# beehover/dependence_free_rl

Hardware: AMD Instinct MI355X
Metric: env-steps/sec (whole node) PPO bin-packing 64-bin (higher is better)
Workload: dtype f32 via f16-pair (layer 2, dH1) / 3-part bf16 split (dW2) MFMA, f32 accumulate

## Files before the change

### dependence_free_rl_amd/csrc/policy_kernels.hip

```cpp
#include "spec8_e0_layout.h"
#include "xh_device.h"
#include "xh_kernels.h"
#include "xh_logit_table.h"
#include "xh_split.h"

#include <cstdlib>

#ifndef XH_DIAG_ABLATE
#define XH_DIAG_ABLATE 0
#endif
#define XH_ABL(a, k) (XH_DIAG_ABLATE && ((a).ablate & (k)))
#ifndef XH_DIAG_TRACE
#define XH_DIAG_TRACE 0
#endif
#if XH_DIAG_TRACE
#define XH_STAMP(a, gi, w, lane, slot)                                        \
  do {                                                                        \
    if ((a).trace && blockIdx.x < kTraceBlocks && (gi) < kTraceGroups &&      \
        (lane) == 0)                                                          \
      (a).trace[((blockIdx.x * kTraceGroups + (gi)) * 8 + (w)) * kTraceSlots + \
                (slot)] = clock64();                                          \
  } while (0)
#else
#define XH_STAMP(a, gi, w, lane, slot) \
  do {                                 \
  } while (0)
#endif
#define XH_STAMP4(a, gi, w, lane, slot) XH_STAMP(a, gi, w, lane, slot)
#if XH_DIAG_TRACE
#define XH_SPAN(a, which)                                                     \
  do {                                                                        \
    if ((a).trace && threadIdx.x == 0) {                                      \
      unsigned long long *sp = reinterpret_cast<unsigned long long *>(        \
          (a).trace + kTraceBlocks * kTraceGroups * 8 * kTraceSlots);         \
      const unsigned long long tnow = (unsigned long long)wall_clock64();     \
      if ((which) == 0)                                                       \
        atomicMin(sp, tnow);                                                  \
      else if ((which) == 3)                                                  \
        atomicMax(sp + 1, tnow);                                              \
      if (blockIdx.x < 512) sp[2 + 4 * blockIdx.x + (which)] = tnow;          \
      if ((which) == 0 && blockIdx.x < 512) {                                 \
        unsigned hw, xc;                                                      \
        asm volatile("s_getreg_b32 %0, hwreg(HW_REG_HW_ID)" : "=s"(hw));      \
        asm volatile("s_getreg_b32 %0, hwreg(HW_REG_XCC_ID)" : "=s"(xc));     \
        sp[2 + 2048 + 2 * blockIdx.x] = hw;                                   \
        sp[2 + 2048 + 2 * blockIdx.x + 1] = xc;                               \
      }                                                                       \
    }                                                                         \
  } while (0)
#else
#define XH_SPAN(a, which) \
  do {                    \
  } while (0)
#endif

namespace xh {
int diag_build() { return XH_DIAG_ABLATE || XH_DIAG_TRACE; }
}

namespace xh {

template <int B_, int D_, int H1_, int H2_>
struct PShape {
  static constexpr int B = B_, D = D_, H1 = H1_, H2 = H2_;
  static constexpr int F0 = 2 * D;
  static constexpr int S1 = (F0 + 1) / 2;
  static constexpr int NIT = H1 / 32, NOT = H2 / 32;
  static constexpr int G = B <= 64 ? 64 / B : 1;
  static constexpr int HG = B <= 64 ? 1 : B / 64;
  static constexpr int R = 64 * HG;
  static constexpr int BD = B * D;
  static constexpr int W2S = H1 + 4;
  static constexpr int HS = H1 + 1;
  static constexpr int AS = H2 + 1;
  static constexpr int FJ = NOT >= 4 ? 2 : 1;
  static constexpr int JW = (NOT * NIT + 3) / 4;
  static constexpr int JH = (2 * NIT + 3) / 4;
  static constexpr int TOCC = (H1 <= 64 && H2 <= 64 && D == 1) ? 2 : 1;
  static_assert(B == 8 || B == 16 || B == 32 || B == 64 || B == 128, "B");
  static_assert(NIT == 1 || NIT == 2 || NIT == 4, "H1 in {32,64,128}");
  static_assert(NOT == 1 || NOT == 2 || NOT == 4, "H2 in {32,64,128}");
  static_assert(D >= 1 && D <= 3, "D");
  static constexpr int r4(int x) { return (x + 3) & ~3; }
  static constexpr int L_W2 = 0;
  static constexpr int L_W1 = L_W2 + H2 * W2S;
  static constexpr int L_B1 = L_W1 + r4(H1 * F0);
  static constexpr int L_B2 = L_B1 + H1;
  static constexpr int L_W3 = L_B2 + H2;
  static constexpr int L_B3 = L_W3 + H2;
  static constexpr int L_Z = L_B3 + 4;
  static constexpr int L_ROLLOUT_END = L_Z + NOT * R;
  static constexpr int L_H1 = L_ROLLOUT_END;
  static constexpr int L_DA2 = L_H1 + r4(64 * HS);
  static constexpr int L_TRAIN_END = L_DA2 + r4(64 * AS);
  static constexpr int TS = 68;
  static constexpr int L_H1T = L_ROLLOUT_END;
  static constexpr int L_DAT = L_H1T + H1 * TS;
  static constexpr int L_B1F = L_DAT + H2 * TS;
  static constexpr int L_TRAIN8_END = L_B1F + 2 * H1;
  static constexpr int RED = H1 * F0 + H1 + 2 * H2 + 1;
  static_assert(4 * RED <= 64 * HS + 64 * AS, "scratch fits");
};

template <class S>
__device__ __forceinline__ void stage_params(const float *__restrict__ P,
                                             float *lds) {
  const PolicyLayout L{S::F0, S::H1, S::H2};
  const int tid = threadIdx.x;
  for (int i = tid; i < S::H2 * S::H1; i += blockDim.x) {
    const int o = i / S::H1, k = i - o * S::H1;
    lds[S::L_W2 + o * S::W2S + k] = P[L.oW2() + i];
  }
  for (int i = tid; i < S::H1 * S::F0; i += blockDim.x)
    lds[S::L_W1 + i] = P[L.oW1() + i];
  for (int i = tid; i < S::H1; i += blockDim.x) lds[S::L_B1 + i] = P[L.ob1() + i];
  for (int i = tid; i < S::H2; i += blockDim.x) {
    lds[S::L_B2 + i] = P[L.ob2() + i];
    lds[S::L_W3 + i] = P[L.ow3() + i];
  }
  if (tid == 0) lds[S::L_B3] = P[L.ob3()];
}

template <class S>
struct RowRaw {
  int bv[2][S::D];
  int iv[2][S::D];
};

template <class S>
__device__ __forceinline__ void fetch_rows(const Batch &b, int slot, int e0,
                                           RowRaw<S> &rr) {
  const int lr = threadIdx.x & 31;
#pragma unroll
  for (int rt = 0; rt < 2; ++rt) {
    const int r = rt * 32 + lr;
    const size_t env = (size_t)slot * b.N + e0 + r / S::B;
    const int8_t *bp = b.bins + env * S::BD + (r % S::B) * S::D;
    const int8_t *ip = b.items + env * 4;
#pragma unroll
    for (int d = 0; d < S::D; ++d) {
      rr.bv[rt][d] = bp[d];
      rr.iv[rt][d] = ip[d];
    }
  }
}

template <class S>
__device__ __forceinline__ float row_feature(const RowRaw<S> &rr, int rt,
                                             int f) {
  int v = 0;
#pragma unroll
  for (int d = 0; d < S::D; ++d) {
    if (f == d) v = rr.bv[rt][d];
    if (f == S::D + d) v = rr.iv[rt][d];
  }
  return f < S::F0 ? (float)v / (float)kCapacity : 0.0f;
}

__device__ __forceinline__ float4 lds4(const float *p) {
  return *reinterpret_cast<const float4 *>(p);
}

template <class S>
__device__ __forceinline__ void layer1(const RowRaw<S> &rr, const float *lds,
                                       f32x16 (&h1)[S::NIT][2]) {
  const int lane = threadIdx.x & 63, lr = lane & 31, h = lane >> 5;
  float xb[2][S::S1];
#pragma unroll
  for (int rt = 0; rt < 2; ++rt)
#pragma unroll
    for (int s = 0; s < S::S1; ++s) xb[rt][s] = row_feature<S>(rr, rt, 2 * s + h);
#pragma unroll
  for (int it = 0; it < S::NIT; ++it) {
    float wa[S::S1];
#pragma unroll
    for (int s = 0; s < S::S1; ++s) {
      const int k = 2 * s + h;
      wa[s] = k < S::F0 ? lds[S::L_W1 + (it * 32 + lr) * S::F0 + k] : 0.0f;
    }
    f32x16 acc0 = zero16(), acc1 = zero16();
#pragma unroll
    for (int s = 0; s < S::S1; ++s) {
      acc0 = mfma32(wa[s], xb[0][s], acc0);
      acc1 = mfma32(wa[s], xb[1][s], acc1);
    }
#pragma unroll
    for (int q = 0; q < 4; ++q) {
      const float4 bb = lds4(lds + S::L_B1 + it * 32 + 8 * q + 4 * h);
      const float bq[4] = {bb.x, bb.y, bb.z, bb.w};
#pragma unroll
      for (int u = 0; u < 4; ++u) {
        const float v0 = acc0[4 * q + u] + bq[u];
        const float v1 = acc1[4 * q + u] + bq[u];
        acc0[4 * q + u] = relu(v0);
        acc1[4 * q + u] = relu(v1);
      }
    }
    h1[it][0] = acc0;
    h1[it][1] = acc1;
  }
}

template <class S, int NR>
__device__ __forceinline__ void layer2(const float *lds,
                                       const f32x16 (&h1)[S::NIT][2], int o2t,
                                       int rt0, f32x16 (&acc)[NR]) {
  const int lane = threadIdx.x & 63, lr = lane & 31, h = lane >> 5;
  const float *wrow = lds + S::L_W2 + (o2t * 32 + lr) * S::W2S + 4 * h;
#pragma unroll
  for (int r = 0; r < NR; ++r) acc[r] = zero16();
#pragma unroll
  for (int it = 0; it < S::NIT; ++it) {
    f32x16 hb[NR];
#pragma unroll
    for (int r = 0; r < NR; ++r)
      hb[r] = NR == 2 ? h1[it][r] : (rt0 == 0 ? h1[it][0] : h1[it][1]);
#pragma unroll
    for (int q = 0; q < 4; ++q) {
      const float4 a4 = lds4(wrow + it * 32 + 8 * q);
      const float av[4] = {a4.x, a4.y, a4.z, a4.w};
#pragma unroll
      for (int u = 0; u < 4; ++u)
#pragma unroll
        for (int r = 0; r < NR; ++r) acc[r] = mfma32(av[u], hb[r][4 * q + u], acc[r]);
    }
  }
#pragma unroll
  for (int q = 0; q < 4; ++q) {
    const float4 bb = lds4(lds + S::L_B2 + o2t * 32 + 8 * q + 4 * h);
    const float bq[4] = {bb.x, bb.y, bb.z, bb.w};
#pragma unroll
    for (int u = 0; u < 4; ++u)
#pragma unroll
      for (int r = 0; r < NR; ++r) acc[r][4 * q + u] += bq[u];
  }
}

template <class S, bool kSwap = false>
__device__ __forceinline__ float logit_part(const float *lds, const f32x16 &pre,
                                            int o2t) {
  const int h = (threadIdx.x & 63) >> 5;
  float zp = 0.0f;
#pragma unroll
  for (int q = 0; q < 4; ++q) {
    const float4 ww = lds4(lds + S::L_W3 + o2t * 32 + 8 * q + 4 * h);
    const float wq[4] = {ww.x, ww.y, ww.z, ww.w};
#pragma unroll
    for (int u = 0; u < 4; ++u) {
      const float v = relu(pre[4 * q + u]);
      zp += v * wq[u];
    }
  }
  return zp + (kSwap ? half_swap(zp) : __shfl_xor(zp, 32, kWave));
}

template <class S>
__device__ __forceinline__ void sample_step_x(const RolloutArgs &a, int t, bool last,
                                              float z, int env, int seg0, int bin,
                                              const RowRaw<S> &cur, uint32_t &x,
                                              int (&nbv)[S::D], bool &first) {
  constexpr int B = S::B;
  const int lane = threadIdx.x & 63, h = lane >> 5;
  const int N = a.b.N;
  const float ex = expf(z);
  const float sum = seg_sum<B>(ex);
  const float p = ex / sum;
  if (last && a.logits_out) a.logits_out[(size_t)env * B + bin] = z;
  if (last && a.probs_out) a.probs_out[(size_t)env * B + bin] = p;
  if (a.qold_out) a.qold_out[((size_t)t * N + env) * B + bin] = p;

  int choice;
  if (a.forced) {
    choice = a.forced[(size_t)t * N + env];
    (void)canonical(x);
  } else {
    choice = sample_discrete<B>(p, lane, canonical(x));
  }
  const float pold = wave_shfl(p, seg0 + choice);

  int nb[S::D];
  int neg = 0;
#pragma unroll
  for (int d = 0; d < S::D; ++d) {
    const int bv = h ? cur.bv[1][d] : cur.bv[0][d];
    const int iv = h ? cur.iv[1][d] : cur.iv[0][d];
    nb[d] = bin == choice ? bv - iv : bv;
    neg |= nb[d] < 0;
  }
  const int done = __shfl(neg, seg0 + choice, kWave);
  first = canonical(x) < a.env.p_a;
  int8_t *ob = a.b.bins + ((size_t)(t + 1) * N + env) * S::BD + bin * S::D;
#pragma unroll
  for (int d = 0; d < S::D; ++d) {
    nbv[d] = done ? kCapacity : nb[d];
    ob[d] = (int8_t)nbv[d];
  }
  if (bin == 0) {
    int8_t *oi = a.b.items + ((size_t)(t + 1) * N + env) * 4;
#pragma unroll
    for (int d = 0; d < 4; ++d)
      oi[d] = d < S::D ? (int8_t)(first ? a.env.item_a[d] : a.env.item_b[d]) : 0;
    a.b.action[(size_t)t * N + env] = choice;
    a.b.pold[(size_t)t * N + env] = pold;
    a.b.done[(size_t)t * N + env] = (uint8_t)done;
  }
}

template <class S>
__device__ __forceinline__ void sample_step(const RolloutArgs &a, float z,
                                            int env, int seg0, int bin,
                                            const RowRaw<S> &cur) {
  uint32_t x = a.b.rng[env];
  int nbv[S::D];
  bool first;
  sample_step_x<S>(a, a.t, true, z, env, seg0, bin, cur, x, nbv, first);
  if (bin == 0) a.b.rng[env] = (a.t == a.b.T - 1) ? mstd_mulmod(x, a.jump_mul) : x;
}

template <class S>
__global__ __launch_bounds__(256, 2) void rollout_step_kernel(RolloutArgs a) {
  extern __shared__ __attribute__((aligned(16))) float lds[];
  stage_params<S>(a.params, lds);
  __syncthreads();
  const int lane = threadIdx.x & 63, w = threadIdx.x >> 6, lr = lane & 31;
  const int N = a.b.N, t = a.t;
  const int ngroups = N / S::G;
  const int o2t = w % S::NOT;
  const int rt0 = S::NOT >= 4 ? 0 : w / S::NOT;
  const bool fwd_active = (w / S::NOT) * S::FJ < 2;

  RowRaw<S> cur, nxt;
  if ((int)blockIdx.x < ngroups) fetch_rows<S>(a.b, t, blockIdx.x * S::G, cur);
  for (int g = blockIdx.x; g < ngroups; g += gridDim.x) {
    const int e0 = g * S::G;
    const int gn = g + gridDim.x;
    if (gn < ngroups) fetch_rows<S>(a.b, t, gn * S::G, nxt);
    {
      f32x16 h1[S::NIT][2];
      layer1<S>(cur, lds, h1);
      if (fwd_active) {
        f32x16 pre[S::FJ];
        layer2<S, S::FJ>(lds, h1, o2t, rt0, pre);
#pragma unroll
        for (int q = 0; q < S::FJ; ++q) {
          const float zp = logit_part<S>(lds, pre[q], o2t);
          if (lane < 32) lds[S::L_Z + o2t * 64 + (rt0 + q) * 32 + lr] = zp;
        }
      }
    }
    __syncthreads();
    if (w == 0) {
      constexpr int B = S::B;
      const int e = lane / B, bin = lane % B, env = e0 + e, seg0 = e * B;
      float zs = 0.0f;
#pragma unroll
      for (int o = 0; o < S::NOT; ++o) zs += lds[S::L_Z + o * 64 + lane];
      const float z = zs + lds[S::L_B3];
      sample_step<S>(a, z, env, seg0, bin, cur);
    }
    __syncthreads();
    cur = nxt;
  }
}

#ifndef XH_V_RPASS
#define XH_V_RPASS 1
#endif
#ifndef XH_V_RTILES64
#define XH_V_RTILES64 4
#endif
#ifndef XH_V_RTILES128
#define XH_V_RTILES128 2
#endif
constexpr int roll_waves(int tiles) { return XH_V_RPASS && tiles == 4 ? 12 : 8; }
constexpr int roll_occ(int waves) { return waves == 8 ? 4 : (waves == 12 ? 3 : 2); }
constexpr int kRollWaves64 = roll_waves(XH_V_RTILES64);
constexpr int kRollWaves128 = roll_waves(XH_V_RTILES128);
#ifndef XH_V_RSB
#define XH_V_RSB 1
#endif
template <class S, int OT>
__device__ __forceinline__ void wave_logits_rpass(const float *lds,
                                                  const RowRaw<S> &cur,
                                                  float (&zl)[2]) {
  const int lane = threadIdx.x & 63, lr = lane & 31, h = lane >> 5;
#pragma unroll
  for (int rt = 0; rt < 2; ++rt) {
    float xb[S::S1];
#pragma unroll
    for (int s = 0; s < S::S1; ++s) xb[s] = row_feature<S>(cur, rt, 2 * s + h);
    float z = 0.0f;
#pragma unroll 1
    for (int op = 0; op < 4 / OT; ++op) {
    f32x16 pre[OT];
#pragma unroll
    for (int o = 0; o < OT; ++o) pre[o] = zero16();
#pragma unroll 1
    for (int it = 0; it < 4; ++it) {
      f32x16 t1 = zero16();
#pragma unroll
      for (int s = 0; s < S::S1; ++s) {
        const int k = 2 * s + h;
        const float wa = k < S::F0 ? lds[S::L_W1 + (it * 32 + lr) * S::F0 + k] : 0.0f;
        t1 = mfma32(wa, xb[s], t1);
      }
#pragma unroll
      for (int q = 0; q < 4; ++q) {
        const float4 bb = lds4(lds + S::L_B1 + it * 32 + 8 * q + 4 * h);
        const float bq[4] = {bb.x, bb.y, bb.z, bb.w};
#pragma unroll
        for (int u = 0; u < 4; ++u) t1[4 * q + u] = relu(t1[4 * q + u] + bq[u]);
      }
#pragma unroll
      for (int oo = 0; oo < OT; ++oo) {
        const int o = op * OT + oo;
        const float *wrow = lds + S::L_W2 + (o * 32 + lr) * S::W2S + 4 * h;
#pragma unroll
        for (int q = 0; q < 4; ++q) {
          const float4 a4 = lds4(wrow + it * 32 + 8 * q);
          const float av[4] = {a4.x, a4.y, a4.z, a4.w};
#pragma unroll
          for (int u = 0; u < 4; ++u) pre[oo] = mfma32(av[u], t1[4 * q + u], pre[oo]);
        }
        if (XH_V_RSB) __builtin_amdgcn_sched_barrier(0);
      }
    }
#pragma unroll
    for (int oo = 0; oo < OT; ++oo) {
      const int o = op * OT + oo;
#pragma unroll
      for (int q = 0; q < 4; ++q) {
        const float4 bb = lds4(lds + S::L_B2 + o * 32 + 8 * q + 4 * h);
        const float bq[4] = {bb.x, bb.y, bb.z, bb.w};
#pragma unroll
        for (int u = 0; u < 4; ++u) pre[oo][4 * q + u] += bq[u];
      }
      z += logit_part<S>(lds, pre[oo], o);
    }
    }
    if (rt == 0)
      zl[0] = z;
    else
      zl[1] = z;
  }
}

template <class S>
__global__ __launch_bounds__(64 * kRollWaves64, roll_occ(kRollWaves64)) void rollout_wave_kernel(RolloutArgs a) {
  static_assert(S::B == 64 && S::NIT == 4 && S::NOT == 4, "wave rollout: B=64, [128,128]");
  extern __shared__ __attribute__((aligned(16))) float lds[];
  stage_params<S>(a.params, lds);
  __syncthreads();
  const int lane = threadIdx.x & 63, w = threadIdx.x >> 6, lr = lane & 31,
            h = lane >> 5;
  const int wpb = blockDim.x >> 6;
  for (int env = blockIdx.x * wpb + w; env < a.b.N; env += gridDim.x * wpb) {
    RowRaw<S> cur;
    fetch_rows<S>(a.b, a.t, env, cur);
    float xb[2][S::S1];
#pragma unroll
    for (int rt = 0; rt < 2; ++rt)
#pragma unroll
      for (int s = 0; s < S::S1; ++s) xb[rt][s] = row_feature<S>(cur, rt, 2 * s + h);
    float zl[2] = {0.0f, 0.0f};
    if (XH_V_RPASS) wave_logits_rpass<S, XH_V_RTILES64>(lds, cur, zl);
#pragma unroll 1
    for (int o2t = 0; o2t < (XH_V_RPASS ? 0 : 4); ++o2t) {
      const float *wrow = lds + S::L_W2 + (o2t * 32 + lr) * S::W2S + 4 * h;
      f32x16 pre[2];
      pre[0] = zero16();
      pre[1] = zero16();
#pragma unroll 1
      for (int it = 0; it < 4; ++it) {
        f32x16 t1[2];
        t1[0] = zero16();
        t1[1] = zero16();
#pragma unroll
        for (int s = 0; s < S::S1; ++s) {
          const int k = 2 * s + h;
          const float wa = k < S::F0 ? lds[S::L_W1 + (it * 32 + lr) * S::F0 + k] : 0.0f;
          t1[0] = mfma32(wa, xb[0][s], t1[0]);
          t1[1] = mfma32(wa, xb[1][s], t1[1]);
        }
#pragma unroll
        for (int q = 0; q < 4; ++q) {
          const float4 bb = lds4(lds + S::L_B1 + it * 32 + 8 * q + 4 * h);
          const float bq[4] = {bb.x, bb.y, bb.z, bb.w};
#pragma unroll
          for (int u = 0; u < 4; ++u) {
            t1[0][4 * q + u] = relu(t1[0][4 * q + u] + bq[u]);
            t1[1][4 * q + u] = relu(t1[1][4 * q + u] + bq[u]);
          }
        }
#pragma unroll
        for (int q = 0; q < 4; ++q) {
          const float4 a4 = lds4(wrow + it * 32 + 8 * q);
          const float av[4] = {a4.x, a4.y, a4.z, a4.w};
#pragma unroll
          for (int u = 0; u < 4; ++u) {
            pre[0] = mfma32(av[u], t1[0][4 * q + u], pre[0]);
            pre[1] = mfma32(av[u], t1[1][4 * q + u], pre[1]);
          }
        }
      }
#pragma unroll
      for (int q = 0; q < 4; ++q) {
        const float4 bb = lds4(lds + S::L_B2 + o2t * 32 + 8 * q + 4 * h);
        const float bq[4] = {bb.x, bb.y, bb.z, bb.w};
#pragma unroll
        for (int u = 0; u < 4; ++u) {
          pre[0][4 * q + u] += bq[u];
          pre[1][4 * q + u] += bq[u];
        }
      }
      zl[0] += logit_part<S>(lds, pre[0], o2t);
      zl[1] += logit_part<S>(lds, pre[1], o2t);
    }
    const float z = (h ? zl[1] : zl[0]) + lds[S::L_B3];
    sample_step<S>(a, z, env, 0, lane, cur);
  }
}

template <class S>
struct RollSplitLds {
  static constexpr int W2 = 0;
  static constexpr int F = 2 * S::H2 * kImgRow;
  static constexpr int W1 = 0, B1 = S::H1 * S::F0, B2 = B1 + S::H1, W3 = B2 + S::H2,
                       B3 = W3 + S::H2, SH = B3 + 1, SC = B3 + 4, B1F = SC + 2 * 16;
  static constexpr int S1F = (S::D + 1) / 2;
  static constexpr size_t bytes = F + sizeof(float) * (B1F + 2 * S::H1);
};

template <class S>
__device__ __forceinline__ void stage_split_rollout(const float *__restrict__ P,
                                                    const EnvDesc &env, char *lds) {
  using L = RollSplitLds<S>;
  float *lf = reinterpret_cast<float *>(lds + L::F);
  const PolicyLayout PL{S::F0, S::H1, S::H2};
  float mw = 0.0f, mh = 0.0f;
  for (int e = threadIdx.x; e < S::H2 * S::H1; e += blockDim.x)
    mw = fmaxf(mw, fabsf(P[PL.oW2() + e]));
  for (int i = threadIdx.x; i < S::H1; i += blockDim.x) {
    float v = fabsf(P[PL.ob1() + i]);
    for (int k = 0; k < S::F0; ++k) v += fabsf(P[PL.oW1() + i * S::F0 + k]);
    mh = fmaxf(mh, v);
  }
#pragma unroll
  for (int o = 1; o < 64; o <<= 1) {
    mw = fmaxf(mw, __shfl_xor(mw, o, kWave));
    mh = fmaxf(mh, __shfl_xor(mh, o, kWave));
  }
  const int nw = blockDim.x >> 6, wv = threadIdx.x >> 6;
  if ((threadIdx.x & 63) == 0) {
    lf[L::SC + wv] = mw;
    lf[L::SC + 16 + wv] = mh;
  }
  __syncthreads();
  float MW = 0.0f, MH = 0.0f;
  for (int v = 0; v < nw; ++v) {
    MW = fmaxf(MW, lf[L::SC + v]);
    MH = fmaxf(MH, lf[L::SC + 16 + v]);
  }
  const float SW = f16_scale_for(MW), SH = f16_scale_for(MH), S2 = SW * SH;
  for (int e = threadIdx.x; e < S::H2 * S::H1; e += blockDim.x) {
    const int o = e / S::H1, i = e % S::H1;
    const int c = (i & ~12) | ((i & 4) << 1) | ((i & 8) >> 1);
    _Float16 x0, x1;
    split2h(P[PL.oW2() + e] * SW, x0, x1);
    const int off = img_off(o, c >> 3) + 2 * (c & 7);
    *reinterpret_cast<_Float16 *>(lds + L::W2 + off) = x0;
    *reinterpret_cast<_Float16 *>(lds + L::W2 + S::H2 * kImgRow + off) = x1;
  }
  for (int i = threadIdx.x; i < S::H1 * S::F0; i += blockDim.x)
    lf[L::W1 + i] = P[PL.oW1() + i] * SH;
  for (int i = threadIdx.x; i < S::H1; i += blockDim.x) {
    lf[L::B1 + i] = P[PL.ob1() + i] * SH;
    lf[L::B2 + i] = P[PL.ob2() + i] * S2;
    lf[L::W3 + i] = P[PL.ow3() + i] * (1.0f / S2);
    float ba = P[PL.ob1() + i], bb = ba;
#pragma unroll
    for (int d = 0; d < S::D; ++d) {
      const float wv = P[PL.oW1() + i * S::F0 + S::D + d];
      ba += wv * ((float)env.item_a[d] / (float)kCapacity);
      bb += wv * ((float)env.item_b[d] / (float)kCapacity);
    }
    lf[L::B1F + i] = ba * SH;
    lf[L::B1F + S::H1 + i] = bb * SH;
  }
  if (threadIdx.x == 0) {
    lf[L::B3] = P[PL.ob3()];
    lf[L::SH] = SH;
  }
}

template <class S, bool E0 = false>
__device__ __forceinline__ void wave_logits_split(const char *lds,
                                                  const RowRaw<S> &cur,
                                                  const float *const (&b1r)[2],
                                                  float (&zl)[2],
                                                  unsigned *mbits = nullptr) {
  using L = RollSplitLds<S>;
  const float *lf = reinterpret_cast<const float *>(lds + L::F);
  const int lane = threadIdx.x & 63, lr = lane & 31, h = lane >> 5;
  const char *w2i[2] = {lds + L::W2, lds + L::W2 + S::H2 * kImgRow};
#pragma unroll
  for (int rt = 0; rt < 2; ++rt) {
    float xb[L::S1F];
#pragma unroll
    for (int s1 = 0; s1 < L::S1F; ++s1) {
      const int f = 2 * s1 + h;
      xb[s1] = f < S::D ? row_feature<S>(cur, rt, f) : 0.0f;
    }
    f32x16s pre[S::NOT];
#pragma unroll
    for (int ot = 0; ot < S::NOT; ++ot)
#pragma unroll
      for (int q = 0; q < 4; ++q) {
        const float4 bb = *reinterpret_cast<const float4 *>(lf + L::B2 + ot * 32 + 8 * q + 4 * h);
        pre[ot][4 * q + 0] = bb.x;
        pre[ot][4 * q + 1] = bb.y;
        pre[ot][4 * q + 2] = bb.z;
        pre[ot][4 * q + 3] = bb.w;
      }
#pragma unroll
    for (int it = 0; it < S::NIT; ++it) {
      f32x16 t1;
#pragma unroll
      for (int q = 0; q < 4; ++q) {
        const float4 bb = *reinterpret_cast<const float4 *>(b1r[rt] + it * 32 + 8 * q + 4 * h);
        t1[4 * q + 0] = bb.x;
        t1[4 * q + 1] = bb.y;
        t1[4 * q + 2] = bb.z;
        t1[4 * q + 3] = bb.w;
      }
#pragma unroll
      for (int s1 = 0; s1 < L::S1F; ++s1) {
        const int k = 2 * s1 + h;
        const float wa = k < S::D ? lf[L::W1 + (it * 32 + lr) * S::F0 + k] : 0.0f;
        t1 = mfma32(wa, xb[s1], t1);
      }
      f16x8 bfr[2][2];
      {
        typedef unsigned u32x4_t __attribute__((ext_vector_type(4)));
        u32x4_t hb[2], lb[2];
#pragma unroll
        for (int jj = 0; jj < 8; ++jj) {
          unsigned h2, l2;
          split2h_x2(relu(t1[2 * jj]), relu(t1[2 * jj + 1]), h2, l2);
          hb[jj >> 2][jj & 3] = h2;
          lb[jj >> 2][jj & 3] = l2;
        }
#pragma unroll
        for (int s = 0; s < 2; ++s) {
          bfr[s][0] = __builtin_bit_cast(f16x8, hb[s]);
          bfr[s][1] = __builtin_bit_cast(f16x8, lb[s]);
        }
      }
#pragma unroll
      for (int ot = 0; ot < S::NOT; ++ot) {
        const int rb = row_base(ot * 32 + lr, h);
#pragma unroll
        for (int s = 0; s < 2; ++s) {
          f16x8 af[2];
#pragma unroll
          for (int p = 0; p < 2; ++p)
            af[p] = __builtin_bit_cast(f16x8, ld_row(w2i[p], rb, 2 * it + s));
          pre[ot] = mfma_f16(af[1], bfr[s][0], pre[ot]);
          pre[ot] = mfma_f16(af[0], bfr[s][1], pre[ot]);
          pre[ot] = mfma_f16(af[0], bfr[s][0], pre[ot]);
        }
        __builtin_amdgcn_sched_barrier(0);
      }
    }
    float z = 0.0f;
#pragma unroll
    for (int ot = 0; ot < S::NOT; ++ot) {
      float zp = 0.0f;
#pragma unroll
      for (int q = 0; q < 4; ++q) {
        const float4 ww = *reinterpret_cast<const float4 *>(lf + L::W3 + ot * 32 + 8 * q + 4 * h);
        const float wq[4] = {ww.x, ww.y, ww.z, ww.w};
#pragma unroll
        for (int u = 0; u < 4; ++u) zp = fmaf(relu(pre[ot][4 * q + u]), wq[u], zp);
      }
      z += zp + __shfl_xor(zp, 32, kWave);
    }
    zl[rt] = z;
    if constexpr (E0) {
#pragma unroll
      for (int ot = 0; ot < S::NOT; ++ot) {
        unsigned wd = rt == 0 ? 0u : mbits[ot];
#pragma unroll
        for (int e = 0; e < 16; ++e) {
          int m;
          asm("v_med3_i32 %0, %1, 0, 1" : "=v"(m) : "v"(__float_as_int(pre[ot][e])));
          wd |= (unsigned)m << sp8::e0_bit(rt, e);
        }
        mbits[ot] = wd;
      }
    }
  }
}

template <class S>
constexpr int roll_split_waves() { return S::B == 64 ? kRollWaves64 : 4; }
template <class S>
constexpr int roll_split_occ() { return S::B == 64 ? roll_occ(kRollWaves64) : 2; }

template <class S>
__device__ __forceinline__ void build_logit_table(const char *lds, float *out) {
  static_assert(S::B == 64 && S::D == 2 && S::G == 1 && lt::kCap == kCapacity,
                "the logit table: 64 bins, 2-D");
  const float *lfr = reinterpret_cast<const float *>(lds + RollSplitLds<S>::F);
  const float *const b1r[2] = {lfr + RollSplitLds<S>::B1F,
                               lfr + RollSplitLds<S>::B1F + S::H1};
  const int lane = threadIdx.x & 63, w = threadIdx.x >> 6, lr = lane & 31;
  const int nw = blockDim.x >> 6;
#pragma unroll 1
  for (int c = w; c < lt::kCalls; c += nw) {
    const int sn = lt::enum_state(c, lr);
    const int s = sn < lt::kStates ? sn : lt::kStates - 1;
    int b0, b1;
    lt::state_bins(s, b0, b1);
    RowRaw<S> cur;
#pragma unroll
    for (int rt = 0; rt < 2; ++rt) {
      cur.bv[rt][0] = b0;
      cur.bv[rt][1] = b1;
      cur.iv[rt][0] = cur.iv[rt][1] = 0;
    }
    float zl[2];
    wave_logits_split<S>(lds, cur, b1r, zl);
    if (lane < 32 && sn < lt::kStates) {
      out[lt::entry(0, b0, b1)] = zl[0];
      out[lt::entry(1, b0, b1)] = zl[1];
    }
  }
}

template <class S, bool TAB>
constexpr size_t roll_split_lds() {
  return RollSplitLds<S>::bytes + (TAB ? sizeof(float) * lt::kEntries : 0);
}

template <class S, bool E0 = false, bool TAB = false>
__global__ __launch_bounds__(64 * roll_split_waves<S>(), roll_split_occ<S>()) void rollout_split_kernel(RolloutArgs a) {
  static_assert((S::B == 64 && S::NIT == 4 && S::NOT == 4) ||
                    (S::B == 32 && S::NIT == 2 && S::NOT == 2),
                "split rollout: B=64 [128,128] or B=32 [64,64]");
  static_assert(!E0 || (S::B == 64 && S::G == 1 && S::H2 == sp8::kE0Outs),
                "the epoch-0 records: one env of 64 bins per wave");
  static_assert(!TAB || !E0, "the table carries no relu masks");
  extern __shared__ __attribute__((aligned(16))) float ldsf[];
  char *lds = reinterpret_cast<char *>(ldsf);
  stage_split_rollout<S>(a.params, a.env, lds);
  __syncthreads();
  const float *lfr = reinterpret_cast<const float *>(lds + RollSplitLds<S>::F);
  const float b3 = lfr[RollSplitLds<S>::B3];
  const float *tab = reinterpret_cast<const float *>(lds + RollSplitLds<S>::bytes);
  if constexpr (TAB) {
    build_logit_table<S>(lds, reinterpret_cast<float *>(lds + RollSplitLds<S>::bytes));
    __syncthreads();
  }
  const float *b1fa = lfr + RollSplitLds<S>::B1F, *b1fb = b1fa + S::H1;
  const int lane = threadIdx.x & 63, w = threadIdx.x >> 6, h = lane >> 5, lr = lane & 31;
  const int wpb = blockDim.x >> 6;
  const int ngroups = a.b.N / S::G;
  const int t_last = a.t + (a.nsteps > 1 ? a.nsteps : 1) - 1;
  const int eoff = S::G == 2 ? h : 0, seg0 = S::G == 2 ? 32 * h : 0;
  const int bin = S::G == 2 ? lr : lane;
  const int per = (ngroups + (int)gridDim.x - 1) / (int)gridDim.x;
  const int g_end = min(ngroups, ((int)blockIdx.x + 1) * per);
  for (int g = (int)blockIdx.x * per + w; g < g_end; g += wpb) {
    const int e0 = g * S::G, env = e0 + eoff;
    RowRaw<S> cur;
    fetch_rows<S>(a.b, a.src_slot > 0 ? a.src_slot : a.t, e0, cur);
    if (a.src_slot > 0) {
      int8_t *ob = a.b.bins + (size_t)env * S::BD + bin * S::D;
#pragma unroll
      for (int d = 0; d < S::D; ++d) ob[d] = (int8_t)(h ? cur.bv[1][d] : cur.bv[0][d]);
      if (bin == 0) {
        int8_t *oi = a.b.items + (size_t)env * 4;
#pragma unroll
        for (int d = 0; d < 4; ++d)
          oi[d] = d < S::D ? (int8_t)(h ? cur.iv[1][d] : cur.iv[0][d]) : 0;
      }
    }
    uint32_t x = a.b.rng[env];
    for (int t = a.t; t <= t_last; ++t) {
      const float *b1r[2];
      bool iar[2];
#pragma unroll
      for (int rt = 0; rt < 2; ++rt) {
        bool ia = true;
#pragma unroll
        for (int d = 0; d < S::D; ++d) ia &= cur.iv[rt][d] == a.env.item_a[d];
        iar[rt] = ia;
        b1r[rt] = ia ? b1fa : b1fb;
      }
      float zl[2];
      if constexpr (TAB) {
        const int e = lt::entry((h ? iar[1] : iar[0]) ? 0 : 1,
                                h ? cur.bv[1][0] : cur.bv[0][0],
                                h ? cur.bv[1][1] : cur.bv[0][1]);
        zl[0] = zl[1] = tab[min((unsigned)e, (unsigned)lt::kEntries - 1u)];
      } else if constexpr (E0) {
        unsigned mbits[4];
        wave_logits_split<S, true>(lds, cur, b1r, zl, mbits);
        uint32_t *rec = a.e0_mask + ((size_t)t * a.b.N + env) * sp8::kE0Words;
#pragma unroll
        for (int ot = 0; ot < 4; ++ot) rec[sp8::e0_word(ot, lane)] = mbits[ot];
      } else {
        wave_logits_split<S>(lds, cur, b1r, zl);
      }
      const float z = (h ? zl[1] : zl[0]) + b3;
      int nbv[S::D];
      bool first;
      sample_step_x<S>(a, t, t == t_last, z, env, seg0, bin, cur, x, nbv, first);
      if (t < t_last) {
#pragma unroll
        for (int d = 0; d < S::D; ++d) {
          const int own = nbv[d], oth = __shfl_xor(own, 32, kWave);
          const int ito = first ? a.env.item_a[d] : a.env.item_b[d];
          const int itp = S::G == 2 ? __shfl_xor(ito, 32, kWave) : ito;
          cur.bv[0][d] = h ? oth : own;
          cur.bv[1][d] = h ? own : oth;
          cur.iv[0][d] = h ? itp : ito;
          cur.iv[1][d] = h ? ito : itp;
        }
      }
    }
    if (bin == 0) a.b.rng[env] = (t_last == a.b.T - 1) ? mstd_mulmod(x, a.jump_mul) : x;
  }
}

template <class S>
__device__ __forceinline__ void sample_step128_x(const RolloutArgs &a, int t, bool last,
                                                 int env, const float (&z)[2],
                                                 uint32_t &x, int (&nbv)[2][S::D],
                                                 const int (&iv)[S::D], bool &first) {
  const int lane = threadIdx.x & 63;
  const int N = a.b.N;
  float p[2];
  float se = 0.0f;
#pragma unroll
  for (int k = 0; k < 2; ++k) {
    p[k] = expf(z[k]);
    se += p[k];
  }
  se = seg_sum<64>(se);
  p[0] = p[0] / se;
  p[1] = p[1] / se;
  if (last && a.logits_out) {
    a.logits_out[(size_t)env * 128 + lane] = z[0];
    a.logits_out[(size_t)env * 128 + 64 + lane] = z[1];
  }
  if (last && a.probs_out) {
    a.probs_out[(size_t)env * 128 + lane] = p[0];
    a.probs_out[(size_t)env * 128 + 64 + lane] = p[1];
  }
  if (a.qold_out) {
    a.qold_out[((size_t)t * N + env) * 128 + lane] = p[0];
    a.qold_out[((size_t)t * N + env) * 128 + 64 + lane] = p[1];
  }
  int choice;
  if (a.forced) {
    choice = a.forced[(size_t)t * N + env];
    (void)canonical(x);
  } else {
    const double pd0 = (double)p[0], pd1 = (double)p[1];
    const double sd = seg_sum_d<64>(pd0 + pd1);
    const double c0 = seg_scan_d<64>(pd0 / sd, lane);
    const double tot0 = wave_shfl_d(c0, 63);
    double c1 = tot0 + seg_scan_d<64>(pd1 / sd, lane);
    if (lane == 63) c1 = 1.0;
    const double u = canonical(x);
    choice = __popcll(__ballot(c0 < u)) + __popcll(__ballot(c1 < u));
    const float gap = (float)fmin(fabs(c0 - u), fabs(c1 - u));
    if (seg_min<64>(gap) < 1e-9f) {
      double s2 = 0.0;
      for (int k = 0; k < 128; ++k)
        s2 += (double)wave_shfl(p[k >> 6], k & 63);
      double acc = 0.0;
      int c2 = 127;
      for (int k = 0; k < 128; ++k) {
        const double qk = (double)wave_shfl(p[k >> 6], k & 63) / s2;
        acc = k == 0 ? qk : acc + qk;
        const double cpk = k == 127 ? 1.0 : acc;
        if (!(cpk < u) && k < c2) c2 = k;
      }
      choice = c2;
    }
  }
  const float pold = choice < 64 ? wave_shfl(p[0], choice)
                                 : wave_shfl(p[1], choice - 64);
  int nb[2][S::D];
  int neg[2] = {0, 0};
#pragma unroll
  for (int k = 0; k < 2; ++k) {
    const int bin = k * 64 + lane;
#pragma unroll
    for (int d = 0; d < S::D; ++d) {
      nb[k][d] = bin == choice ? nbv[k][d] - iv[d] : nbv[k][d];
      neg[k] |= nb[k][d] < 0;
    }
  }
  const int done = __shfl(choice < 64 ? neg[0] : neg[1], choice & 63, kWave);
  first = canonical(x) < a.env.p_a;
  const size_t o = (size_t)(t + 1) * N + env;
#pragma unroll
  for (int k = 0; k < 2; ++k) {
    int8_t *ob = a.b.bins + o * S::BD + (k * 64 + lane) * S::D;
#pragma unroll
    for (int d = 0; d < S::D; ++d) {
      nbv[k][d] = done ? kCapacity : nb[k][d];
      ob[d] = (int8_t)nbv[k][d];
    }
  }
  if (lane == 0) {
    int8_t *oi = a.b.items + o * 4;
#pragma unroll
    for (int d = 0; d < 4; ++d)
      oi[d] = d < S::D ? (int8_t)(first ? a.env.item_a[d] : a.env.item_b[d]) : 0;
    a.b.action[(size_t)t * N + env] = choice;
    a.b.pold[(size_t)t * N + env] = pold;
    a.b.done[(size_t)t * N + env] = (uint8_t)done;
  }
}

template <class S>
__device__ __forceinline__ void sample_step128(const RolloutArgs &a, int env,
                                               const float (&z)[2]) {
  const int lane = threadIdx.x & 63;
  uint32_t x = a.b.rng[env];
  const size_t e = (size_t)a.t * a.b.N + env;
  int nbv[2][S::D], iv[S::D];
#pragma unroll
  for (int k = 0; k < 2; ++k)
#pragma unroll
    for (int d = 0; d < S::D; ++d) nbv[k][d] = a.b.bins[e * S::BD + (k * 64 + lane) * S::D + d];
#pragma unroll
  for (int d = 0; d < S::D; ++d) iv[d] = a.b.items[e * 4 + d];
  bool first;
  sample_step128_x<S>(a, a.t, true, env, z, x, nbv, iv, first);
  if (lane == 0) a.b.rng[env] = (a.t == a.b.T - 1) ? mstd_mulmod(x, a.jump_mul) : x;
}

template <class S>
__global__ __launch_bounds__(256, 2) void rollout_step128_kernel(RolloutArgs a) {
  static_assert(S::B == 128 && S::HG == 2, "128-bin rollout");
  extern __shared__ __attribute__((aligned(16))) float lds[];
  stage_params<S>(a.params, lds);
  __syncthreads();
  constexpr int R = S::R;
  const int lane = threadIdx.x & 63, w = threadIdx.x >> 6, lr = lane & 31;
  const int N = a.b.N, t = a.t;
  const int o2t = w % S::NOT;
  const int rt0 = S::NOT >= 4 ? 0 : w / S::NOT;
  const bool fwd_active = (w / S::NOT) * S::FJ < 2;
  for (int env = blockIdx.x; env < N; env += gridDim.x) {
#pragma unroll
    for (int hg = 0; hg < 2; ++hg) {
      RowRaw<S> rr;
#pragma unroll
      for (int k = 0; k < 2; ++k) {
        const int bin = hg * 64 + k * 32 + lr;
        const size_t e = (size_t)t * N + env;
        const int8_t *bp = a.b.bins + e * S::BD + bin * S::D;
        const int8_t *ip = a.b.items + e * 4;
#pragma unroll
        for (int d = 0; d < S::D; ++d) {
          rr.bv[k][d] = bp[d];
          rr.iv[k][d] = ip[d];
        }
      }
      f32x16 h1[S::NIT][2];
      layer1<S>(rr, lds, h1);
      if (fwd_active) {
        f32x16 pre[S::FJ];
        layer2<S, S::FJ>(lds, h1, o2t, rt0, pre);
#pragma unroll
        for (int q = 0; q < S::FJ; ++q) {
          const float zp = logit_part<S>(lds, pre[q], o2t);
          if (lane < 32) lds[S::L_Z + o2t * R + hg * 64 + (rt0 + q) * 32 + lr] = zp;
        }
      }
    }
    __syncthreads();
    if (w == 0) {
      float z[2];
#pragma unroll
      for (int k = 0; k < 2; ++k) {
        float zs = 0.0f;
#pragma unroll
        for (int o = 0; o < S::NOT; ++o) zs += lds[S::L_Z + o * R + k * 64 + lane];
        z[k] = zs + lds[S::L_B3];
      }
      sample_step128<S>(a, env, z);
    }
    __syncthreads();
  }
}

template <class S>
__global__ __launch_bounds__(64 * kRollWaves128, roll_occ(kRollWaves128)) void rollout_wave128_kernel(RolloutArgs a) {
  static_assert(S::B == 128 && S::NIT == 4 && S::NOT == 4,
                "wave rollout: B=128, [128,128]");
  extern __shared__ __attribute__((aligned(16))) float lds[];
  stage_params<S>(a.params, lds);
  __syncthreads();
  const int lane = threadIdx.x & 63, w = threadIdx.x >> 6, lr = lane & 31,
            h = lane >> 5;
  const int wpb = blockDim.x >> 6;
  const int N = a.b.N, t = a.t;
  for (int env = blockIdx.x * wpb + w; env < N; env += gridDim.x * wpb) {
    float z0 = 0.0f, z1 = 0.0f;
#pragma unroll 1
    for (int hg = 0; hg < 2; ++hg) {
      RowRaw<S> cur;
      const size_t e = (size_t)t * N + env;
#pragma unroll
      for (int rt = 0; rt < 2; ++rt) {
        const int bin = hg * 64 + rt * 32 + lr;
        const int8_t *bp = a.b.bins + e * S::BD + bin * S::D;
        const int8_t *ip = a.b.items + e * 4;
#pragma unroll
        for (int d = 0; d < S::D; ++d) {
          cur.bv[rt][d] = bp[d];
          cur.iv[rt][d] = ip[d];
        }
      }
      float xb[2][S::S1];
#pragma unroll
      for (int rt = 0; rt < 2; ++rt)
#pragma unroll
        for (int s = 0; s < S::S1; ++s) xb[rt][s] = row_feature<S>(cur, rt, 2 * s + h);
      float zl[2] = {0.0f, 0.0f};
      if (XH_V_RPASS) wave_logits_rpass<S, XH_V_RTILES128>(lds, cur, zl);
#pragma unroll 1
      for (int o2t = 0; o2t < (XH_V_RPASS ? 0 : 4); ++o2t) {
        const float *wrow = lds + S::L_W2 + (o2t * 32 + lr) * S::W2S + 4 * h;
        f32x16 pre[2];
        pre[0] = zero16();
        pre[1] = zero16();
#pragma unroll 1
        for (int it = 0; it < 4; ++it) {
          f32x16 t1[2];
          t1[0] = zero16();
          t1[1] = zero16();
#pragma unroll
          for (int s = 0; s < S::S1; ++s) {
            const int k = 2 * s + h;
            const float wa = k < S::F0 ? lds[S::L_W1 + (it * 32 + lr) * S::F0 + k] : 0.0f;
            t1[0] = mfma32(wa, xb[0][s], t1[0]);
            t1[1] = mfma32(wa, xb[1][s], t1[1]);
          }
#pragma unroll
          for (int q = 0; q < 4; ++q) {
            const float4 bb = lds4(lds + S::L_B1 + it * 32 + 8 * q + 4 * h);
            const float bq[4] = {bb.x, bb.y, bb.z, bb.w};
#pragma unroll
            for (int u = 0; u < 4; ++u) {
              t1[0][4 * q + u] = relu(t1[0][4 * q + u] + bq[u]);
              t1[1][4 * q + u] = relu(t1[1][4 * q + u] + bq[u]);
            }
          }
#pragma unroll
          for (int q = 0; q < 4; ++q) {
            const float4 a4 = lds4(wrow + it * 32 + 8 * q);
            const float av[4] = {a4.x, a4.y, a4.z, a4.w};
#pragma unroll
            for (int u = 0; u < 4; ++u) {
              pre[0] = mfma32(av[u], t1[0][4 * q + u], pre[0]);
              pre[1] = mfma32(av[u], t1[1][4 * q + u], pre[1]);
            }
          }
        }
#pragma unroll
        for (int q = 0; q < 4; ++q) {
          const float4 bb = lds4(lds + S::L_B2 + o2t * 32 + 8 * q + 4 * h);
          const float bq[4] = {bb.x, bb.y, bb.z, bb.w};
#pragma unroll
          for (int u = 0; u < 4; ++u) {
            pre[0][4 * q + u] += bq[u];
            pre[1][4 * q + u] += bq[u];
          }
        }
        zl[0] += logit_part<S>(lds, pre[0], o2t);
        zl[1] += logit_part<S>(lds, pre[1], o2t);
      }
      const float zh = (h ? zl[1] : zl[0]) + lds[S::L_B3];
      if (hg == 0)
        z0 = zh;
      else
        z1 = zh;
    }
    const float z[2] = {z0, z1};
    sample_step128<S>(a, env, z);
  }
}

constexpr int kRollWavesS128 = 12;
template <class S>
__global__ __launch_bounds__(64 * kRollWavesS128, 3) void rollout_split128_kernel(RolloutArgs a) {
  static_assert(S::B == 128 && S::NIT == 4 && S::NOT == 4,
                "split rollout: B=128, [128,128]");
  extern __shared__ __attribute__((aligned(16))) float ldsf[];
  char *lds = reinterpret_cast<char *>(ldsf);
  stage_split_rollout<S>(a.params, a.env, lds);
  __syncthreads();
  const float *lfr = reinterpret_cast<const float *>(lds + RollSplitLds<S>::F);
  const float b3 = lfr[RollSplitLds<S>::B3];
  const float *b1fa = lfr + RollSplitLds<S>::B1F, *b1fb = b1fa + S::H1;
  const int lane = threadIdx.x & 63, w = threadIdx.x >> 6, h = lane >> 5;
  const int wpb = blockDim.x >> 6;
  const int N = a.b.N;
  const int t_last = a.t + (a.nsteps > 1 ? a.nsteps : 1) - 1;
  const int per = (N + (int)gridDim.x - 1) / (int)gridDim.x;
  const int env_end = min(N, ((int)blockIdx.x + 1) * per);
  for (int env = (int)blockIdx.x * per + w; env < env_end; env += wpb) {
    int own[2][S::D], it[S::D];
    {
      const size_t e = (size_t)(a.src_slot > 0 ? a.src_slot : a.t) * N + env;
#pragma unroll
      for (int k = 0; k < 2; ++k)
#pragma unroll
        for (int d = 0; d < S::D; ++d) own[k][d] = a.b.bins[e * S::BD + (k * 64 + lane) * S::D + d];
#pragma unroll
      for (int d = 0; d < S::D; ++d) it[d] = a.b.items[e * 4 + d];
      if (a.src_slot > 0) {
#pragma unroll
        for (int k = 0; k < 2; ++k)
#pragma unroll
          for (int d = 0; d < S::D; ++d)
            a.b.bins[(size_t)env * S::BD + (k * 64 + lane) * S::D + d] = (int8_t)own[k][d];
        if (lane == 0)
#pragma unroll
          for (int d = 0; d < 4; ++d) a.b.items[(size_t)env * 4 + d] = d < S::D ? (int8_t)it[d] : 0;
      }
    }
    uint32_t x = a.b.rng[env];
    for (int t = a.t; t <= t_last; ++t) {
      bool ia = true;
#pragma unroll
      for (int d = 0; d < S::D; ++d) ia &= it[d] == a.env.item_a[d];
      const float *b1r[2] = {ia ? b1fa : b1fb, ia ? b1fa : b1fb};
      float z[2];
#pragma unroll 1
      for (int hg = 0; hg < 2; ++hg) {
        RowRaw<S> cur;
#pragma unroll
        for (int d = 0; d < S::D; ++d) {
          const int v = hg ? own[1][d] : own[0][d];
          const int o = __shfl_xor(v, 32, kWave);
          cur.bv[0][d] = h ? o : v;
          cur.bv[1][d] = h ? v : o;
          cur.iv[0][d] = it[d];
          cur.iv[1][d] = it[d];
        }
        float zl[2];
        wave_logits_split<S>(lds, cur, b1r, zl);
        const float zh = (h ? zl[1] : zl[0]) + b3;
        if (hg == 0)
          z[0] = zh;
        else
          z[1] = zh;
      }
      bool first;
      sample_step128_x<S>(a, t, t == t_last, env, z, x, own, it, first);
#pragma unroll
      for (int d = 0; d < S::D; ++d) it[d] = first ? a.env.item_a[d] : a.env.item_b[d];
    }
    if (lane == 0) a.b.rng[env] = (t_last == a.b.T - 1) ? mstd_mulmod(x, a.jump_mul) : x;
  }
}


template <class S>
__global__ __launch_bounds__(256, 1) void eval_argmax_kernel(EvalArgs a) {
  static_assert(S::HG == 1, "groups of whole envs");
  extern __shared__ __attribute__((aligned(16))) float lds[];
  stage_params<S>(a.params, lds);
  constexpr int B = S::B, G = S::G, D = S::D;
  int *sbins = reinterpret_cast<int *>(lds + S::L_ROLLOUT_END);
  int *sitem = sbins + G * S::BD;
  uint32_t *srng = reinterpret_cast<uint32_t *>(sitem + G * 4);
  int *sleft = reinterpret_cast<int *>(srng + G);
  int *sflag = sleft + G;
  const int lane = threadIdx.x & 63, w = threadIdx.x >> 6, lr = lane & 31;
  const int o2t = w % S::NOT;
  const int rt0 = S::NOT >= 4 ? 0 : w / S::NOT;
  const bool fwd_active = (w / S::NOT) * S::FJ < 2;
  const int ngroups = a.n_envs / G;
  for (int g = blockIdx.x; g < ngroups; g += gridDim.x) {
    __syncthreads();
    if (w == 0) {
      const int e = lane / B, bin = lane % B, env = g * G + e;
      uint32_t x = mstd_jump(a.x0, (uint64_t)env * a.stream_stride);
      bool first = false;
      if (!a.init_items) first = canonical(x) < a.env.p_a;
      for (int d = 0; d < D; ++d) sbins[e * S::BD + bin * D + d] = kCapacity;
      if (bin == 0) {
        for (int d = 0; d < 4; ++d)
          sitem[e * 4 + d] =
              d >= D ? 0
              : a.init_items ? a.init_items[env * D + d]
              : (first ? a.env.item_a[d] : a.env.item_b[d]);
        srng[e] = x;
        sleft[e] = a.episodes;
        a.total[env] = 0.0;
        a.steps[env] = 0;
      }
    }
    __syncthreads();
    double reward = 0.0;
    long nsteps = 0;
    for (long it = 0; it < a.max_steps; ++it) {
      RowRaw<S> rr;
#pragma unroll
      for (int rt = 0; rt < 2; ++rt) {
        const int r = rt * 32 + lr, e = r / B, bin = r % B;
#pragma unroll
        for (int d = 0; d < D; ++d) {
          rr.bv[rt][d] = sbins[e * S::BD + bin * D + d];
          rr.iv[rt][d] = sitem[e * 4 + d];
        }
      }
      {
        f32x16 h1[S::NIT][2];
        layer1<S>(rr, lds, h1);
        if (fwd_active) {
          f32x16 pre[S::FJ];
          layer2<S, S::FJ>(lds, h1, o2t, rt0, pre);
#pragma unroll
          for (int q = 0; q < S::FJ; ++q) {
            const float zp = logit_part<S>(lds, pre[q], o2t);
            if (lane < 32) lds[S::L_Z + o2t * 64 + (rt0 + q) * 32 + lr] = zp;
          }
        }
      }
      __syncthreads();
      if (w == 0) {
        const int e = lane / B, bin = lane % B, seg0 = e * B;
        float zs = 0.0f;
#pragma unroll
        for (int o = 0; o < S::NOT; ++o) zs += lds[S::L_Z + o * 64 + lane];
        float v = zs + lds[S::L_B3];
        if (a.argmax_probs) {
          const float ex = expf(v);
          v = ex / seg_sum<B>(ex);
        }
        const int choice = seg_argmax_first<B>(v, bin);
        const bool active = sleft[e] > 0;
        int nb[D];
        int neg = 0;
#pragma unroll
        for (int d = 0; d < D; ++d) {
          const int b0 = sbins[e * S::BD + bin * D + d];
          nb[d] = bin == choice ? b0 - sitem[e * 4 + d] : b0;
          neg |= nb[d] < 0;
        }
        const int done = __shfl(neg, seg0 + choice, kWave);
        if (active) {
          uint32_t x = srng[e];
          const bool first = canonical(x) < a.env.p_a;
#pragma unroll
          for (int d = 0; d < D; ++d)
            sbins[e * S::BD + bin * D + d] = done ? kCapacity : nb[d];
          __builtin_amdgcn_wave_barrier();
          if (bin == 0) {
            for (int d = 0; d < D; ++d)
              sitem[e * 4 + d] = first ? a.env.item_a[d] : a.env.item_b[d];
            srng[e] = x;
            if (done) sleft[e] -= 1;
            reward += done ? 0.0 : 1.0;
            if (a.trace && g == 0 && e == 0 && nsteps < a.trace_cap)
              a.trace[nsteps] = choice;
            ++nsteps;
          }
        }
        const int any = __any(sleft[e] > 0);
        if (lane == 0) *sflag = any;
      }
      __syncthreads();
      if (*sflag == 0) break;
    }
    if (w == 0 && lane % B == 0) {
      const int env = g * G + lane / B;
      a.total[env] = reward;
      a.steps[env] = nsteps;
      a.rng_out[env] = srng[lane / B];
      for (int d = 0; d < D; ++d)
        a.final_items[env * D + d] = sitem[(lane / B) * 4 + d];
    }
  }
}

#ifndef XH_V4_UNROLL
#define XH_V4_UNROLL 3
#endif
#ifndef XH_V4_L3
#define XH_V4_L3 1
#endif


template <class S, bool KL>
__global__ __launch_bounds__(256, S::TOCC) void policy_train_kernel(PolicyTrainArgs a) {
  extern __shared__ __attribute__((aligned(16))) float lds[];
  XH_SPAN(a, 0);
  XH_STAMP4(a, kTraceGroups - 1, threadIdx.x >> 6, threadIdx.x & 63, 0);
  stage_params<S>(a.params, lds);
  __syncthreads();
  XH_STAMP4(a, kTraceGroups - 1, threadIdx.x >> 6, threadIdx.x & 63, 1);
  XH_SPAN(a, 1);
  constexpr int B = S::B, NIT = S::NIT, NOT = S::NOT;
  const int lane = threadIdx.x & 63, w = threadIdx.x >> 6, lr = lane & 31,
            h = lane >> 5;
  const int N = a.b.N, T = a.b.T;
  const int gpt = N / S::G;
  const int gmain = T * gpt;
  const int n_end = KL ? *a.n_end : 0;
  const int ngroups = KL ? gmain + gpt + (n_end + S::G - 1) / S::G : gmain;
  const float beta = KL ? *a.beta : 0.0f;
  double kl_acc = 0.0;
  float *H1img = lds + S::L_H1;
  float *DAimg = lds + S::L_DA2;

  const int o2t = w % NOT;
  const int rt0 = NOT >= 4 ? 0 : w / NOT;
  const bool fwd_active = (w / NOT) * S::FJ < 2;
  const int it_own = w % NIT;
  const int hrt0 = NIT >= 4 ? 0 : w / NIT;
  constexpr int HSTEP = 4 / NIT;

  f32x16 accW2[S::JW];
#pragma unroll
  for (int q = 0; q < S::JW; ++q) accW2[q] = zero16();
  float accW1[16][S::F0], accB1[16], accW3[16], accB2[16], accB3 = 0.0f;
#pragma unroll
  for (int j = 0; j < 16; ++j) {
    accB1[j] = accW3[j] = accB2[j] = 0.0f;
#pragma unroll
    for (int f = 0; f < S::F0; ++f) accW1[j][f] = 0.0f;
  }

  RowRaw<S> cur, nxt;
  int c_cur = 0, c_nxt = 0, v_cur = 1, v_nxt = 1;
  float po_cur = 1.0f, po_nxt = 1.0f, A_cur = 0.0f, A_nxt = 0.0f;
  float q_cur = 1.0f, q_nxt = 1.0f;
  auto fetch = [&](int g, RowRaw<S> &rr, int &c, float &po, float &A, float &q,
                   int &valid) {
    if constexpr (!KL) {
      const int t = g / gpt, e0 = (g - t * gpt) * S::G;
      fetch_rows<S>(a.b, t, e0, rr);
      const size_t ti = (size_t)t * N + e0 + lane / B;
      c = a.b.action[ti];
      po = a.b.pold[ti];
      A = a.adv[ti];
    } else {
#pragma unroll
      for (int rt = 0; rt < 2; ++rt) {
        const int r = rt * 32 + lr, el = r / B, bin = r % B;
        int t, e, kind, ok = 1;
        if (g < gmain) {
          t = g / gpt;
          e = (g - t * gpt) * S::G + el;
          kind = 0;
        } else if (g < gmain + gpt) {
          t = T;
          e = (g - gmain) * S::G + el;
          kind = 1;
          ok = a.b.done[(size_t)(T - 1) * N + e] == 0;
        } else {
          const int j = (g - gmain - gpt) * S::G + el;
          kind = 2;
          ok = j < n_end;
          const int te = ok ? a.end_list[j] : 0;
          t = te / N;
          e = te - t * N;
        }
        const size_t env = (size_t)t * N + e;
        const int8_t *bp = a.b.bins + env * S::BD + bin * S::D;
        const int8_t *ip = a.b.items + env * 4;
        const bool sub = kind == 2 && a.b.action[env] == bin;
#pragma unroll
        for (int d = 0; d < S::D; ++d) {
          rr.iv[rt][d] = ip[d];
          rr.bv[rt][d] = bp[d] - (sub ? ip[d] : 0);
        }
        if (rt == h) {
          c = kind == 0 ? a.b.action[env] : 0;
          A = kind == 0 ? a.adv[env] : 0.0f;
          po = 1.0f;
          const size_t qrow = kind == 1 ? (size_t)(T - 1) * N + e : env;
          q = a.qold[qrow * B + bin];
          valid = ok;
        }
      }
    }
  };
  if ((int)blockIdx.x < ngroups)
    fetch(blockIdx.x, cur, c_cur, po_cur, A_cur, q_cur, v_cur);

  for (int g = blockIdx.x; g < ngroups; g += gridDim.x) {
    const int gi = (g - (int)blockIdx.x) / (int)gridDim.x;
    (void)gi;
    XH_STAMP4(a, gi, w, lane, 0);
    const int gn = g + gridDim.x;
    if (gn < ngroups) fetch(gn, nxt, c_nxt, po_nxt, A_nxt, q_nxt, v_nxt);
    f32x16 pre[S::FJ];
    f32x16 h1own[2];
    {
      f32x16 h1[NIT][2];
      layer1<S>(cur, lds, h1);
      if (w < NIT) {
#pragma unroll
        for (int it = 0; it < NIT; ++it)
          if (it == w) {
#pragma unroll
            for (int rt = 0; rt < 2; ++rt)
#pragma unroll
              for (int j = 0; j < 16; ++j)
                H1img[(rt * 32 + lr) * S::HS + it * 32 + acc_row(j, h)] =
                    h1[it][rt][j];
          }
      }
#pragma unroll
      for (int it = 0; it < NIT; ++it)
        if (it == it_own) {
          h1own[0] = h1[it][0];
          h1own[1] = h1[it][1];
        }
      if (fwd_active) {
        if (!XH_ABL(a, 4)) {
          layer2<S, S::FJ>(lds, h1, o2t, rt0, pre);
        } else {
#pragma unroll
          for (int q = 0; q < S::FJ; ++q) pre[q] = h1[0][q & 1];
        }
#pragma unroll
        for (int q = 0; q < S::FJ; ++q) {
          const float zp = logit_part<S>(lds, pre[q], o2t);
          if (lane < 32) lds[S::L_Z + o2t * 64 + (rt0 + q) * 32 + lr] = zp;
        }
      }
    }
    XH_STAMP4(a, gi, w, lane, 1);
    __syncthreads();
    XH_STAMP4(a, gi, w, lane, 2);

    constexpr bool kOne = S::JW == 1 && S::JH == 1 && !KL;
    constexpr int kU4 = kOne ? XH_V4_UNROLL : 0;
    constexpr bool kL34 = kOne && XH_V4_L3;
    float4 w3v[4];
    if (kL34) {
#pragma unroll
      for (int qq = 0; qq < 4; ++qq)
        w3v[qq] = lds4(lds + S::L_W3 + o2t * 32 + 8 * qq + 4 * h);
    }

    float gz;
    {
      const int bin = lane % B, seg0 = (lane / B) * B;
      float zs = 0.0f;
#pragma unroll
      for (int o = 0; o < NOT; ++o) zs += lds[S::L_Z + o * 64 + lane];
      const float z = zs + lds[S::L_B3];
      const float ex = expf(z);
      const float p = ex / seg_sum<B>(ex);
      const int c = c_cur;
      const float A = A_cur;
      if constexpr (KL) {
        float gp = p * A + beta * (p - q_cur);
        if (bin == c) gp -= A;
        const float sg = seg_sum<B>(p * gp);
        gz = v_cur ? p * (gp - sg) : 0.0f;
        if (w == 0 && v_cur)
          kl_acc += (double)q_cur * log((double)q_cur / (double)p);
      } else if (XH_ABL(a, 8)) {
        gz = z * 1e-3f;
      } else if (a.algo == kPPO) {
        const float pc = wave_shfl(p, seg0 + c);
        const float ratio = pc / po_cur;
        float clipped = ratio;
        if (ratio > 1.0f + a.clip_eps)
          clipped = 1.0f + a.clip_eps;
        else if (ratio < 1.0f - a.clip_eps)
          clipped = 1.0f - a.clip_eps;
        const float ig = fminf(clipped * A, ratio * A) * -1.0f;
        const float gc = ig / pc;
        const float lin = bin == c ? p : 0.0f;
        gz = (lin - p * pc) * gc;
      } else {
        gz = p * A;
        if (bin == c) gz -= A;
      }
      if (w == 0) accB3 += gz;
    }
    XH_STAMP4(a, gi, w, lane, 3);

    if (fwd_active) {
#pragma unroll
      for (int q = 0; q < S::FJ; ++q) {
        const int rt = rt0 + q;
        const float gr = wave_shfl(gz, rt * 32 + lr);
#pragma unroll
        for (int qq = 0; qq < 4; ++qq) {
          const float4 ww =
              kL34 ? w3v[qq] : lds4(lds + S::L_W3 + o2t * 32 + 8 * qq + 4 * h);
          const float wq[4] = {ww.x, ww.y, ww.z, ww.w};
#pragma unroll
          for (int u = 0; u < 4; ++u) {
            const int j = 4 * qq + u;
            const float v = pre[q][j];
            const float h2 = relu(v);
            accW3[j] += gr * h2;
            const float d = v > 0.0f ? gr * wq[u] : 0.0f;
            accB2[j] += d;
            DAimg[(rt * 32 + lr) * S::AS + o2t * 32 + acc_row(j, h)] = d;
          }
        }
      }
    }
    XH_STAMP4(a, gi, w, lane, 4);
    __syncthreads();
    XH_STAMP4(a, gi, w, lane, 5);

    auto dw2_step = [&](int s) {
      const int r = 2 * s + h;
      const float av = DAimg[r * S::AS + o2t * 32 + lr];
#pragma unroll
      for (int q = 0; q < S::JW; ++q) {
        const int it = NOT >= 4 ? q : w / NOT + q * (4 / NOT);
        if (NOT >= 4 || it < NIT)
          accW2[q] = mfma32(av, H1img[r * S::HS + it * 32 + lr], accW2[q]);
      }
    };
    if constexpr (kU4 & 1) {
#pragma unroll
      for (int s = 0; s < 32; ++s) dw2_step(s);
    } else {
#pragma unroll 4
      for (int s = 0; s < (XH_ABL(a, 1) ? 0 : 32); ++s) dw2_step(s);
    }
    XH_STAMP4(a, gi, w, lane, 6);

    {
      f32x16 dh[S::JH];
#pragma unroll
      for (int q = 0; q < S::JH; ++q) dh[q] = zero16();
      auto dh1_step = [&](int s) {
        const int k = 2 * s + h;
        const float av = lds[S::L_W2 + k * S::W2S + it_own * 32 + lr];
#pragma unroll
        for (int q = 0; q < S::JH; ++q) {
          const int rt = NIT >= 4 ? q : hrt0 + q * HSTEP;
          if (NIT >= 4 || rt < 2)
            dh[q] = mfma32(av, DAimg[(rt * 32 + lr) * S::AS + k], dh[q]);
        }
      };
      if constexpr (kU4 & 2) {
#pragma unroll
        for (int s = 0; s < S::H2 / 2; ++s) dh1_step(s);
      } else {
#pragma unroll 4
        for (int s = 0; s < (XH_ABL(a, 2) ? 0 : S::H2 / 2); ++s) dh1_step(s);
      }
#pragma unroll
      for (int q = 0; q < S::JH; ++q) {
        const int rt = NIT >= 4 ? q : hrt0 + q * HSTEP;
        if (NIT >= 4 || rt < 2) {
          float xf[S::F0];
#pragma unroll
          for (int f = 0; f < S::F0; ++f)
            xf[f] = rt == 0 ? row_feature<S>(cur, 0, f) : row_feature<S>(cur, 1, f);
          const f32x16 hv = (rt == 0) ? h1own[0] : h1own[1];
#pragma unroll
          for (int j = 0; j < 16; ++j) {
            const float d = hv[j] > 0.0f ? dh[q][j] : 0.0f;
            accB1[j] += d;
#pragma unroll
            for (int f = 0; f < S::F0; ++f) accW1[j][f] += d * xf[f];
          }
        }
      }
    }
    XH_STAMP4(a, gi, w, lane, 7);
    __syncthreads();
    cur = nxt;
    c_cur = c_nxt;
    po_cur = po_nxt;
    A_cur = A_nxt;
    q_cur = q_nxt;
    v_cur = v_nxt;
  }
  XH_STAMP4(a, kTraceGroups - 1, w, lane, 2);
  XH_SPAN(a, 2);
  if constexpr (KL) {
    if (w == 0) {
#pragma unroll
      for (int o = 1; o < 64; o <<= 1) kl_acc += __shfl_xor(kl_acc, o, kWave);
      if (lane == 0) a.kl_part[blockIdx.x] = kl_acc;
    }
  }

  const PolicyLayout L{S::F0, S::H1, S::H2};
  float *slab = a.slab + (size_t)blockIdx.x * a.slab_stride;
#pragma unroll
  for (int q = 0; q < S::JW; ++q) {
    const int it = w / NOT + q * (4 / NOT);
    if (it < NIT) {
#pragma unroll
      for (int j = 0; j < 16; ++j) {
        const int o2 = o2t * 32 + acc_row(j, h);
        slab[L.oW2() + o2 * S::H1 + it * 32 + lr] = accW2[q][j];
      }
    }
  }
  float *scr = lds + S::L_H1;
  for (int i = threadIdx.x; i < 4 * S::RED; i += blockDim.x) scr[i] = 0.0f;
  __syncthreads();
  float *my = scr + w * S::RED;
  const bool h_active = hrt0 < 2;
#pragma unroll
  for (int j = 0; j < 16; ++j) {
    const float vb1 = half_sum32(accB1[j]), vw3 = half_sum32(accW3[j]),
                vb2 = half_sum32(accB2[j]);
    float vw1[S::F0];
#pragma unroll
    for (int f = 0; f < S::F0; ++f) vw1[f] = half_sum32(accW1[j][f]);
    if (lr == 31) {
      const int i = it_own * 32 + acc_row(j, h);
      const int o2 = o2t * 32 + acc_row(j, h);
      if (h_active) {
#pragma unroll
        for (int f = 0; f < S::F0; ++f) my[i * S::F0 + f] = vw1[f];
        my[S::H1 * S::F0 + i] = vb1;
      }
      if (fwd_active) {
        my[S::H1 * S::F0 + S::H1 + o2] = vw3;
        my[S::H1 * S::F0 + S::H1 + S::H2 + o2] = vb2;
      }
    }
  }
  {
    float v = accB3;
#pragma unroll
    for (int o = 1; o < 64; o <<= 1) v += __shfl_xor(v, o, kWave);
    if (w == 0 && lane == 0) my[S::RED - 1] = v;
  }
  __syncthreads();
  for (int i = threadIdx.x; i < S::RED; i += blockDim.x) {
    const float v = ((scr[i] + scr[S::RED + i]) + scr[2 * S::RED + i]) +
                    scr[3 * S::RED + i];
    int dst;
    if (i < S::H1 * S::F0)
      dst = L.oW1() + i;
    else if (i < S::H1 * S::F0 + S::H1)
      dst = L.ob1() + (i - S::H1 * S::F0);
    else if (i < S::H1 * S::F0 + S::H1 + S::H2)
      dst = L.ow3() + (i - S::H1 * S::F0 - S::H1);
    else if (i < S::RED - 1)
      dst = L.ob2() + (i - S::H1 * S::F0 - S::H1 - S::H2);
    else
      dst = L.ob3();
    slab[dst] = v;
  }
  XH_STAMP4(a, kTraceGroups - 1, w, lane, 3);
  XH_SPAN(a, 3);
}

#ifndef XH_V_DH1
#define XH_V_DH1 1
#endif
#ifndef XH_V_DH1W
#define XH_V_DH1W 16
#endif
#ifndef XH_V_W2U
#define XH_V_W2U 8
#endif
#ifndef XH_V_L3
#define XH_V_L3 1
#endif
#ifndef XH_V_L3W
#define XH_V_L3W 1
#endif
#ifndef XH_V_FOLDW
#define XH_V_FOLDW 1
#endif
#ifndef XH_V_FOLD
#define XH_V_FOLD 1
#endif

template <class S>
__global__ __launch_bounds__(512, 2) void policy_train8_kernel(PolicyTrainArgs a) {
  static_assert(S::NIT == 4 && S::NOT == 4, "8-wave kernel is for 128x128");
  static_assert(8 * S::RED <= (S::H1 + S::H2) * S::TS, "scratch fits");
  extern __shared__ __attribute__((aligned(16))) float lds[];
  stage_params<S>(a.params, lds);
  constexpr bool kFold = XH_V_FOLD && S::G == 1 && (S::HG > 1 ? XH_V_FOLDW : 1);
  constexpr int kS1 = kFold ? (S::D + 1) / 2 : S::S1;
  if (kFold) {
    __syncthreads();
    for (int i = threadIdx.x; i < 2 * S::H1; i += blockDim.x) {
      const int e = i / S::H1, u = i - e * S::H1;
      const int *it = e == 0 ? a.env.item_a : a.env.item_b;
      float v = lds[S::L_B1 + u];
#pragma unroll
      for (int d = 0; d < S::D; ++d)
        v += lds[S::L_W1 + u * S::F0 + S::D + d] * ((float)it[d] / (float)kCapacity);
      lds[S::L_B1F + i] = v;
    }
  }
  __syncthreads();
  constexpr int B = S::B, HG = S::HG, R = S::R;
  const int lane = threadIdx.x & 63, w = threadIdx.x >> 6, lr = lane & 31,
            h = lane >> 5;
  const int q = w & 3, rt = w >> 2;
  const int N = a.b.N, T = a.b.T;
  const int gpt = N / S::G;
  const int ngroups = T * gpt;
  float *H1T = lds + S::L_H1T;
  float *DAT = lds + S::L_DAT;

  f32x16 accW2[2];
  accW2[0] = zero16();
  accW2[1] = zero16();
  constexpr bool kB2Late = S::HG > 1;
  constexpr bool kMW1 = S::HG > 1;
  typedef float f32x4 __attribute__((ext_vector_type(4)));
  f32x4 accW1m = {0.0f, 0.0f, 0.0f, 0.0f};
  float b2s = 0.0f;
  float accW1[16][S::D], sA[16], sB[16], accW3[16], accB2[16], accB3 = 0.0f;
#pragma unroll
  for (int j = 0; j < 16; ++j) {
    sA[j] = sB[j] = accW3[j] = accB2[j] = 0.0f;
#pragma unroll
    for (int f = 0; f < S::D; ++f) accW1[j][f] = 0.0f;
  }

  int bv_c[S::D], iv_c[S::D], bv_n[S::D], iv_n[S::D];
  auto fetch_row = [&](int g, int hg, int (&bv)[S::D], int (&iv)[S::D]) {
    const int t = g / gpt, e0 = (g - t * gpt) * S::G;
    const int r = hg * 64 + rt * 32 + lr;
    const size_t env = (size_t)t * N + e0 + r / B;
    const int8_t *bp = a.b.bins + env * S::BD + (r % B) * S::D;
    const int8_t *ip = a.b.items + env * 4;
#pragma unroll
    for (int d = 0; d < S::D; ++d) {
      bv[d] = bp[d];
      iv[d] = ip[d];
    }
  };
  auto feat = [&](int f) {
    int v = 0;
#pragma unroll
    for (int d = 0; d < S::D; ++d) {
      if (f == d) v = bv_c[d];
      if (f == S::D + d) v = iv_c[d];
    }
    return f < S::F0 ? (float)v / (float)kCapacity : 0.0f;
  };
  auto fold_feat = [&](int f) { return (kFold && f >= S::D) ? 0.0f : feat(f); };
  bool item_b_grp = false;
  auto forward = [&](bool write_h1) {
    f32x16 pre;
#pragma unroll
    for (int qq = 0; qq < 4; ++qq) {
      const float4 bb = lds4(lds + S::L_B2 + q * 32 + 8 * qq + 4 * h);
      pre[4 * qq + 0] = bb.x;
      pre[4 * qq + 1] = bb.y;
      pre[4 * qq + 2] = bb.z;
      pre[4 * qq + 3] = bb.w;
    }
    float xb[S::S1];
#pragma unroll
    for (int s = 0; s < S::S1; ++s) xb[s] = fold_feat(2 * s + h);
    const float *wrow = lds + S::L_W2 + (q * 32 + lr) * S::W2S + 4 * h;
    auto l1 = [&](int it) {
      f32x16 t;
      const float *bsrc = kFold ? lds + S::L_B1F + (item_b_grp ? S::H1 : 0)
                                : lds + S::L_B1;
#pragma unroll
      for (int qq = 0; qq < 4; ++qq) {
        const float4 bb = lds4(bsrc + it * 32 + 8 * qq + 4 * h);
        t[4 * qq + 0] = bb.x;
        t[4 * qq + 1] = bb.y;
        t[4 * qq + 2] = bb.z;
        t[4 * qq + 3] = bb.w;
      }
#pragma unroll
      for (int s = 0; s < kS1; ++s) {
        const int k = 2 * s + h;
        const float wa = k < S::F0 ? lds[S::L_W1 + (it * 32 + lr) * S::F0 + k] : 0.0f;
        t = mfma32(wa, xb[s], t);
      }
      return t;
    };
#pragma unroll
    for (int it = 0; it < 4; ++it) {
      f32x16 t1 = l1(it);
#pragma unroll
      for (int j = 0; j < 16; ++j) t1[j] = relu(t1[j]);
      if (write_h1 && it == q) {
#pragma unroll
        for (int j = 0; j < 16; ++j)
          H1T[(it * 32 + acc_row(j, h)) * S::TS + rt * 32 + lr] = t1[j];
      }
      if (XH_ABL(a, 4)) continue;
#pragma unroll
      for (int qq = 0; qq < 4; ++qq) {
        const float4 a4 = lds4(wrow + it * 32 + 8 * qq);
        pre = mfma32(a4.x, t1[4 * qq + 0], pre);
        pre = mfma32(a4.y, t1[4 * qq + 1], pre);
        pre = mfma32(a4.z, t1[4 * qq + 2], pre);
        pre = mfma32(a4.w, t1[4 * qq + 3], pre);
      }
    }
    return pre;
  };
  auto write_h1_tile = [&]() {
    float xb[S::S1];
#pragma unroll
    for (int s = 0; s < S::S1; ++s) xb[s] = fold_feat(2 * s + h);
    f32x16 t1;
    const float *bsrc = kFold ? lds + S::L_B1F + (item_b_grp ? S::H1 : 0)
                              : lds + S::L_B1;
#pragma unroll
    for (int qq = 0; qq < 4; ++qq) {
      const float4 bb = lds4(bsrc + q * 32 + 8 * qq + 4 * h);
      t1[4 * qq + 0] = bb.x;
      t1[4 * qq + 1] = bb.y;
      t1[4 * qq + 2] = bb.z;
      t1[4 * qq + 3] = bb.w;
    }
#pragma unroll
    for (int s = 0; s < kS1; ++s) {
      const int k = 2 * s + h;
      const float wa = k < S::F0 ? lds[S::L_W1 + (q * 32 + lr) * S::F0 + k] : 0.0f;
      t1 = mfma32(wa, xb[s], t1);
    }
#pragma unroll
    for (int j = 0; j < 16; ++j)
      H1T[(q * 32 + acc_row(j, h)) * S::TS + rt * 32 + lr] = relu(t1[j]);
  };

  if (HG == 1 && (int)blockIdx.x < ngroups) fetch_row(blockIdx.x, 0, bv_c, iv_c);
  constexpr int kDH1 = HG == 1 ? XH_V_DH1 : 0;
  constexpr bool kL3 = HG == 1 ? XH_V_L3 : XH_V_L3W;

  for (int g = blockIdx.x; g < ngroups; g += gridDim.x) {
    const int gi = (g - (int)blockIdx.x) / (int)gridDim.x;
    (void)gi;
    XH_STAMP(a, gi, w, lane, 0);
    const int gn = g + gridDim.x;
    if (HG == 1 && gn < ngroups) fetch_row(gn, 0, bv_n, iv_n);
    int c_cur;
    float po_cur, A_cur;
    {
      const int t = g / gpt, e0 = (g - t * gpt) * S::G;
      const size_t ti = (size_t)t * N + e0 + lane / (B <= 64 ? B : 64);
      c_cur = a.b.action[ti];
      po_cur = a.b.pold[ti];
      A_cur = a.adv[ti];
    }

    if (kFold && HG == 1) {
      bool is_a = true;
#pragma unroll
      for (int d = 0; d < S::D; ++d) is_a &= iv_c[d] == a.env.item_a[d];
      item_b_grp = !is_a;
    }
    f32x16 pre, pre0 = zero16();
#pragma unroll
    for (int hg = 0; hg < HG; ++hg) {
      if (HG > 1) {
        fetch_row(g, hg, bv_c, iv_c);
        if (kFold && hg == 0) {
          bool is_a = true;
#pragma unroll
          for (int d = 0; d < S::D; ++d) is_a &= iv_c[d] == a.env.item_a[d];
          item_b_grp = !is_a;
        }
      }
      pre = forward(hg == HG - 1);
      if (HG > 1 && hg == 0) pre0 = pre;
      const float zp = logit_part<S, true>(lds, pre, q);
      if (lane < 32) lds[S::L_Z + q * R + hg * 64 + rt * 32 + lr] = zp;
    }
    XH_STAMP(a, gi, w, lane, 1);
    __syncthreads();
    XH_STAMP(a, gi, w, lane, 2);
    float4 w3v[4];
    if (kL3) {
#pragma unroll
      for (int qq = 0; qq < 4; ++qq)
        w3v[qq] = lds4(lds + S::L_W3 + q * 32 + 8 * qq + 4 * h);
    }

    float gzk[HG];
    {
      constexpr int SEG = B <= 64 ? B : 64;
      float z[HG], ex[HG], p[HG];
      float se = 0.0f;
#pragma unroll
      for (int k = 0; k < HG; ++k) {
        const int r = k * 64 + lane;
        const float zs = ((lds[S::L_Z + r] + lds[S::L_Z + R + r]) +
                          lds[S::L_Z + 2 * R + r]) + lds[S::L_Z + 3 * R + r];
        z[k] = zs + lds[S::L_B3];
        ex[k] = __expf(z[k]);
        se += ex[k];
      }
      se = seg_sum<SEG>(se);
      const float rse = __builtin_amdgcn_rcpf(se);
#pragma unroll
      for (int k = 0; k < HG; ++k) p[k] = ex[k] * rse;
      const int c = c_cur;
      const float A = A_cur;
      const int seg0 = (lane / SEG) * SEG;
      float pc = 0.0f;
      if constexpr (B == 64) {
        const int cu = __builtin_amdgcn_readfirstlane(c);
        pc = __int_as_float(__builtin_amdgcn_readlane(__float_as_int(p[0]), cu));
      } else {
#pragma unroll
        for (int k = 0; k < HG; ++k) {
          const float v = wave_shfl(p[k], seg0 + (c % SEG));
          if (HG == 1 || c / 64 == k) pc = v;
        }
      }
#pragma unroll
      for (int k = 0; k < HG; ++k) {
        const int bin = (k * 64 + lane) % B;
        float gz;
        if (XH_ABL(a, 8)) {
          gz = z[k] * 1e-3f;
        } else if (a.algo == kPPO) {
          const float ratio = pc * __builtin_amdgcn_rcpf(po_cur);
          float clipped = ratio;
          if (ratio > 1.0f + a.clip_eps)
            clipped = 1.0f + a.clip_eps;
          else if (ratio < 1.0f - a.clip_eps)
            clipped = 1.0f - a.clip_eps;
          const float ig = fminf(clipped * A, ratio * A) * -1.0f;
          const float gc = ig * __builtin_amdgcn_rcpf(pc);
          const float lin = bin == c ? p[k] : 0.0f;
          gz = (lin - p[k] * pc) * gc;
        } else {
          gz = p[k] * A;
          if (bin == c) gz -= A;
        }
        gzk[k] = gz;
        if (w == 0) accB3 += gz;
      }
    }
    XH_STAMP(a, gi, w, lane, 3);

#pragma unroll
    for (int hb = 0; hb < HG; ++hb) {
      const int hg = HG - 1 - hb;
      if (hb > 0) {
        __syncthreads();
        fetch_row(g, hg, bv_c, iv_c);
        write_h1_tile();
        pre = pre0;
      }
      {
        const float sw = half_swap(gzk[hg]);
        const float gr = h == rt ? gzk[hg] : sw;
#pragma unroll
        for (int qq = 0; qq < 4; ++qq) {
          const float4 ww =
              kL3 ? w3v[qq] : lds4(lds + S::L_W3 + q * 32 + 8 * qq + 4 * h);
          const float wq[4] = {ww.x, ww.y, ww.z, ww.w};
#pragma unroll
          for (int u = 0; u < 4; ++u) {
            const int j = 4 * qq + u;
            const float v = pre[j];
            accW3[j] += gr * relu(v);
            const float d = v > 0.0f ? gr * wq[u] : 0.0f;
            if (!kB2Late) accB2[j] += d;
            DAT[(q * 32 + acc_row(j, h)) * S::TS + rt * 32 + lr] = d;
          }
        }
      }
      XH_STAMP(a, gi, w, lane, 4);
      __syncthreads();
      XH_STAMP(a, gi, w, lane, 5);

      f32x16 dh = zero16();
      auto dh1_step = [&](int s) {
        const int k = (kDH1 & 2) ? s + (S::H2 / 2) * h : 2 * s + h;
        dh = mfma32(lds[S::L_W2 + k * S::W2S + q * 32 + lr],
                    DAT[k * S::TS + rt * 32 + lr], dh);
      };
      if constexpr (kDH1 & 1) {
#pragma unroll
        for (int s = 0; s < S::H2 / 2; ++s) {
          if (XH_ABL(a, 16)) break;
          dh1_step(s);
        }
      } else {
        constexpr int kU = XH_V_DH1W;
#pragma unroll kU
        for (int s = 0; s < S::H2 / 2; ++s) {
          if (XH_ABL(a, 16)) break;
          dh1_step(s);
        }
      }
      XH_STAMP(a, gi, w, lane, 6);
      float xf[S::D];
#pragma unroll
      for (int f = 0; f < S::D; ++f) xf[f] = feat(f);
      bool item_is_a = true;
#pragma unroll
      for (int d = 0; d < S::D; ++d) item_is_a &= iv_c[d] == a.env.item_a[d];
      const float fa = item_is_a ? 1.0f : 0.0f, fb = 1.0f - fa;
      const float *hcol = H1T + (q * 32) * S::TS + rt * 32 + lr;
      constexpr int kUnrollW2 = S::HG > 1 ? XH_V_W2U : 8;
      const float *pa = DAT + (q * 32 + lr) * S::TS + 32 * h;
      const float *pb0 = H1T + ((2 * rt) * 32 + lr) * S::TS + 32 * h;
      const float *pb1 = H1T + ((2 * rt + 1) * 32 + lr) * S::TS + 32 * h;
#pragma unroll kUnrollW2
      for (int s4 = 0; s4 < 8; ++s4) {
        if (XH_ABL(a, 32)) break;
        const float4 av = lds4(pa + 4 * s4);
        const float4 b0 = lds4(pb0 + 4 * s4);
        const float4 b1 = lds4(pb1 + 4 * s4);
        if (kB2Late && (s4 >> 2) == rt) b2s += (av.x + av.y) + (av.z + av.w);
        accW2[0] = mfma32(av.x, b0.x, accW2[0]);
        accW2[1] = mfma32(av.x, b1.x, accW2[1]);
        accW2[0] = mfma32(av.y, b0.y, accW2[0]);
        accW2[1] = mfma32(av.y, b1.y, accW2[1]);
        accW2[0] = mfma32(av.z, b0.z, accW2[0]);
        accW2[1] = mfma32(av.z, b1.z, accW2[1]);
        accW2[0] = mfma32(av.w, b0.w, accW2[0]);
        accW2[1] = mfma32(av.w, b1.w, accW2[1]);
#pragma unroll
        for (int jj = 0; jj < 2; ++jj) {
          const int j = 2 * s4 + jj;
          const float d = hcol[acc_row(j, h) * S::TS] > 0.0f ? dh[j] : 0.0f;
          if constexpr (kMW1) {
            dh[j] = d;
          } else {
            sA[j] = fmaf(d, fa, sA[j]);
            sB[j] = fmaf(d, fb, sB[j]);
#pragma unroll
            for (int f = 0; f < S::D; ++f) accW1[j][f] += d * xf[f];
          }
        }
      }
      XH_STAMP(a, gi, w, lane, 7);
      if constexpr (kMW1) {
        __syncthreads();
        float *A1T = H1T;
        float *XT = DAT;
#pragma unroll
        for (int j = 0; j < 16; ++j)
          A1T[(q * 32 + acc_row(j, h)) * S::TS + rt * 32 + lr] = dh[j];
        if (q == 0) {
#pragma unroll
          for (int f = 0; f < S::F0; ++f) XT[f * S::TS + rt * 32 + lr] = feat(f);
          XT[S::F0 * S::TS + rt * 32 + lr] = 1.0f;
        }
        __syncthreads();
        const int fi = lane & 15, kq = lane >> 4;
        const float *xa = XT + fi * S::TS + kq;
        const float *ab = A1T + (w * 16 + fi) * S::TS + kq;
#pragma unroll
        for (int s = 0; s < 16; ++s) {
          const float av = fi <= S::F0 ? xa[4 * s] : 0.0f;
          accW1m = __builtin_amdgcn_mfma_f32_16x16x4f32(av, ab[4 * s], accW1m,
                                                       0, 0, 0);
        }
      }
    }
    __syncthreads();
    if (HG == 1) {
#pragma unroll
      for (int d = 0; d < S::D; ++d) {
        bv_c[d] = bv_n[d];
        iv_c[d] = iv_n[d];
      }
    }
  }

  const PolicyLayout L{S::F0, S::H1, S::H2};
  float *slab = a.slab + (size_t)blockIdx.x * a.slab_stride;
#pragma unroll
  for (int k = 0; k < 2; ++k) {
    const int it = 2 * rt + k;
#pragma unroll
    for (int j = 0; j < 16; ++j) {
      const int o2 = q * 32 + acc_row(j, h);
      slab[L.oW2() + o2 * S::H1 + it * 32 + lr] = accW2[k][j];
    }
  }
  float *scr = lds + S::L_H1T;
  for (int i = threadIdx.x; i < 8 * S::RED; i += blockDim.x) scr[i] = 0.0f;
  __syncthreads();
  float *my = scr + w * S::RED;
#pragma unroll
  for (int j = 0; j < 16; ++j) {
    const float va = half_sum32(sA[j]), vb = half_sum32(sB[j]),
                vw3 = half_sum32(accW3[j]), vb2 = half_sum32(accB2[j]);
    float vw1[S::D];
#pragma unroll
    for (int f = 0; f < S::D; ++f) vw1[f] = half_sum32(accW1[j][f]);
    if (lr == 31) {
      const int i = q * 32 + acc_row(j, h);
      if constexpr (!kMW1) {
#pragma unroll
        for (int f = 0; f < S::D; ++f) my[i * S::F0 + f] = vw1[f];
#pragma unroll
        for (int d = 0; d < S::D; ++d)
          my[i * S::F0 + S::D + d] =
              va * ((float)a.env.item_a[d] / (float)kCapacity) +
              vb * ((float)a.env.item_b[d] / (float)kCapacity);
        my[S::H1 * S::F0 + i] = va + vb;
      }
      my[S::H1 * S::F0 + S::H1 + i] = vw3;
      if (!kB2Late) my[S::H1 * S::F0 + S::H1 + S::H2 + i] = vb2;
    }
  }
  if (kB2Late) {
    const float v = b2s + __shfl_xor(b2s, 32, kWave);
    if (h == 0) my[S::H1 * S::F0 + S::H1 + S::H2 + q * 32 + lr] = v;
  }
  {
    float v = accB3;
#pragma unroll
    for (int o = 1; o < 64; o <<= 1) v += __shfl_xor(v, o, kWave);
    if (lane == 0) my[S::RED - 1] = w == 0 ? v : 0.0f;
  }
  __syncthreads();
  if constexpr (kMW1) {
    const int fi = lane & 15, kq = lane >> 4, i = w * 16 + fi;
#pragma unroll
    for (int r = 0; r < 4; ++r) {
      const int f = 4 * kq + r;
      if (f < S::F0)
        slab[L.oW1() + i * S::F0 + f] = accW1m[r];
      else if (f == S::F0)
        slab[L.ob1() + i] = accW1m[r];
    }
  }
  for (int i = threadIdx.x; i < S::RED; i += blockDim.x) {
    if (kMW1 && i < S::H1 * S::F0 + S::H1) continue;
    float v = 0.0f;
#pragma unroll
    for (int k = 0; k < 8; ++k) v += scr[k * S::RED + i];
    int dst;
    if (i < S::H1 * S::F0)
      dst = L.oW1() + i;
    else if (i < S::H1 * S::F0 + S::H1)
      dst = L.ob1() + (i - S::H1 * S::F0);
    else if (i < S::H1 * S::F0 + S::H1 + S::H2)
      dst = L.ow3() + (i - S::H1 * S::F0 - S::H1);
    else if (i < S::RED - 1)
      dst = L.ob2() + (i - S::H1 * S::F0 - S::H1 - S::H2);
    else
      dst = L.ob3();
    slab[dst] = v;
  }
}

#define XH_POLICY_SHAPES(X) \
  X(8, 2, 128, 64)          \
  X(8, 2, 64, 32)           \
  X(16, 2, 64, 64)          \
  X(32, 1, 64, 64)          \
  X(64, 2, 128, 128)        \
  X(128, 3, 128, 128)

#ifndef XH_TRAIN4
#define XH_TRAIN4 0
#endif

template <class S>
constexpr size_t rollout_lds() {
  return sizeof(float) * S::L_ROLLOUT_END;
}
template <class S>
constexpr size_t train_lds() {
  return sizeof(float) *
         (S::L_TRAIN_END > S::L_TRAIN8_END ? S::L_TRAIN_END : S::L_TRAIN8_END);
}

static bool rollout4() {
  const char *e = std::getenv("XH_ROLLOUT_KERNEL");
  return e && std::atoi(e) == 4;
}
static bool rollout_split() {
  const char *e = std::getenv("XH_ROLLOUT_KERNEL");
  return !(e && (e[0] == 'f' || std::atoi(e) == 4));
}

bool policy_shape_supported(int B, int D, int H1, int H2) {
#define X(XB, XD, XH1, XH2) \
  if (B == XB && D == XD && H1 == XH1 && H2 == XH2) return true;
  XH_POLICY_SHAPES(X)
#undef X
  return false;
}

static int cu_count() {
  static int n = 0;
  if (!n) {
    int dev = 0;
    (void)hipGetDevice(&dev);
    if (hipDeviceGetAttribute(&n, hipDeviceAttributeMultiprocessorCount, dev) !=
            hipSuccess ||
        n <= 0)
      n = 256;
  }
  return n;
}

int rollout_grid(int B, int D, int H1, int H2) {
  (void)B; (void)D; (void)H1; (void)H2;
  return 2 * cu_count();
}
int policy_train_grid(int B, int D, int H1, int H2, int kl) {
  if (train_spec4_default(B, D, H1, H2, kl)) return cu_count();
#define X(XB, XD, XH1, XH2)                                     \
  if (B == XB && D == XD && H1 == XH1 && H2 == XH2) {          \
    using S = PShape<XB, XD, XH1, XH2>;                         \
    (void)kl;                                                   \
    return (S::NIT == 4 && S::NOT == 4) ? cu_count()            \
                                        : S::TOCC * cu_count(); \
  }
  XH_POLICY_SHAPES(X)
#undef X
  return cu_count();
}

static bool rollout_fetch_shifts(const RolloutArgs &a, int H1, int H2) {
  if (!rollout_split() || a.wide) return false;
  const int B = a.env.B;
  return (B == 64 && H1 == 128 && H2 == 128) || (B == 32 && H1 == 64 && H2 == 64) ||
         (B == 128 && H1 == 128 && H2 == 128);
}

static bool rollout_table() {
  const char *e = std::getenv("XH_ROLLOUT_TABLE");
  return !(e && *e && std::atoi(e) == 0);
}

static hipError_t launch_rollout_one(const RolloutArgs &a, int H1, int H2,
                                     int grid, hipStream_t s, KernelInfo *info,
                                     bool &multi) {
  const int B = a.env.B, D = a.env.D;
  multi = false;
  info->math = kMathF32Mfma;
#define X(XB, XD, XH1, XH2)                                                  \
  if (B == XB && D == XD && H1 == XH1 && H2 == XH2) {                        \
    using S = PShape<XB, XD, XH1, XH2>;                                      \
    static bool attr = false;                                                \
    if (!attr) {                                                             \
      if constexpr (S::HG == 1)                                              \
        (void)hipFuncSetAttribute((const void *)rollout_step_kernel<S>,      \
                                  hipFuncAttributeMaxDynamicSharedMemorySize,\
                                  (int)rollout_lds<S>());                    \
      else                                                                   \
        (void)hipFuncSetAttribute((const void *)rollout_step128_kernel<S>,   \
                                  hipFuncAttributeMaxDynamicSharedMemorySize,\
                                  (int)rollout_lds<S>());                    \
      attr = true;                                                           \
    }                                                                        \
    const int ng = a.b.N / S::G;                                             \
    if constexpr (S::B == 128 && S::NIT == 4 && S::NOT == 4) {               \
      if (rollout_split() && !a.wide) {                                      \
        static bool sattr = false;                                           \
        if (!sattr) {                                                        \
          (void)hipFuncSetAttribute((const void *)rollout_split128_kernel<S>,\
                                    hipFuncAttributeMaxDynamicSharedMemorySize,\
                                    (int)RollSplitLds<S>::bytes);            \
          sattr = true;                                                      \
        }                                                                    \
        constexpr int kRW = kRollWavesS128;                                  \
        const int wg = (a.b.N + kRW - 1) / kRW;                              \
        const int wgr = cu_count();                                          \
        info->name = "rollout_split128_kernel";                              \
        info->math = kMathSplitRollout;                                      \
        multi = true;                                                        \
        hipLaunchKernelGGL(rollout_split128_kernel<S>,                       \
                           dim3(wgr < wg ? wgr : wg), dim3(64 * kRW),        \
                           RollSplitLds<S>::bytes, s, a);                    \
        return hipGetLastError();                                            \
      }                                                                      \
    }                                                                        \
    if constexpr (S::B == 128 && S::NIT == 4 && S::NOT == 4) {               \
      if (!rollout4()) {                                                     \
        static bool wattr = false;                                           \
        if (!wattr) {                                                        \
          (void)hipFuncSetAttribute((const void *)rollout_wave128_kernel<S>, \
                                    hipFuncAttributeMaxDynamicSharedMemorySize,\
                                    (int)rollout_lds<S>());                  \
          wattr = true;                                                      \
        }                                                                    \
        constexpr int kRW = kRollWaves128;                                   \
        const int wg = (a.b.N + kRW - 1) / kRW;                              \
        const int wgr = kRW == 8 ? grid : cu_count();                        \
        info->name = "rollout_wave128_kernel";                               \
        hipLaunchKernelGGL(rollout_wave128_kernel<S>,                        \
                           dim3(wgr < wg ? wgr : wg), dim3(64 * kRW),        \
                           rollout_lds<S>(), s, a);                          \
        return hipGetLastError();                                            \
      }                                                                      \
    }                                                                        \
    if constexpr ((S::B == 64 && S::NIT == 4 && S::NOT == 4) ||             \
                  (S::B == 32 && S::NIT == 2 && S::NOT == 2)) {              \
      if (rollout_split() && !a.wide) {                                      \
        static bool sattr = false;                                           \
        if (!sattr) {                                                        \
          (void)hipFuncSetAttribute((const void *)rollout_split_kernel<S>,   \
                                    hipFuncAttributeMaxDynamicSharedMemorySize,\
                                    (int)RollSplitLds<S>::bytes);               \
          sattr = true;                                                      \
        }                                                                    \
        constexpr int kRW = roll_split_waves<S>();                           \
        const int wg = (ng + kRW - 1) / kRW;                                 \
         \
         \
        const int wgr = S::B == 64 ? (kRW == 8 ? grid : cu_count()) : wg;    \
        info->name = "rollout_split_kernel";                                 \
        info->math = kMathSplitRollout;                                      \
        multi = true;                                                        \
        if constexpr (S::B == 64) {                                          \
          if (a.e0_mask) {                                                   \
            static bool eattr = false;                                       \
            if (!eattr) {                                                    \
              (void)hipFuncSetAttribute(                                     \
                  (const void *)rollout_split_kernel<S, true>,               \
                  hipFuncAttributeMaxDynamicSharedMemorySize,                \
                  (int)RollSplitLds<S>::bytes);                              \
              eattr = true;                                                  \
            }                                                                \
            hipLaunchKernelGGL((rollout_split_kernel<S, true>),              \
                               dim3(wgr < wg ? wgr : wg), dim3(64 * kRW),    \
                               RollSplitLds<S>::bytes, s, a);                \
            return hipGetLastError();                                        \
          }                                                                  \
          if constexpr (S::D == 2) {                                         \
             \
             \
            if (rollout_table() && !a.wide_seen) {                           \
              static bool tattr = false;                                     \
              if (!tattr) {                                                  \
                (void)hipFuncSetAttribute(                                   \
                    (const void *)rollout_split_kernel<S, false, true>,      \
                    hipFuncAttributeMaxDynamicSharedMemorySize,              \
                    (int)roll_split_lds<S, true>());                         \
                tattr = true;                                                \
              }                                                              \
              info->logit_table = true;                                      \
              hipLaunchKernelGGL((rollout_split_kernel<S, false, true>),     \
                                 dim3(wgr < wg ? wgr : wg), dim3(64 * kRW),  \
                                 (roll_split_lds<S, true>()), s, a);         \
              return hipGetLastError();                                      \
            }                                                                \
          }                                                                  \
        }                                                                    \
        hipLaunchKernelGGL(rollout_split_kernel<S>,                          \
                           dim3(wgr < wg ? wgr : wg), dim3(64 * kRW),        \
                           RollSplitLds<S>::bytes, s, a);                       \
        return hipGetLastError();                                            \
      }                                                                      \
    }                                                                        \
    if constexpr (S::B == 64 && S::NIT == 4 && S::NOT == 4) {                \
      if (!rollout4()) {                                                     \
        static bool wattr = false;                                           \
        if (!wattr) {                                                        \
          (void)hipFuncSetAttribute((const void *)rollout_wave_kernel<S>,    \
                                    hipFuncAttributeMaxDynamicSharedMemorySize,\
                                    (int)rollout_lds<S>());                  \
          wattr = true;                                                      \
        }                                                                    \
        constexpr int kRW = kRollWaves64;                                    \
        const int wg = (ng + kRW - 1) / kRW;                                 \
        const int wgr = kRW == 8 ? grid : cu_count();                        \
        info->name = "rollout_wave_kernel";                                  \
        hipLaunchKernelGGL(rollout_wave_kernel<S>,                           \
                           dim3(wgr < wg ? wgr : wg), dim3(64 * kRW),        \
                           rollout_lds<S>(), s, a);                          \
        return hipGetLastError();                                            \
      }                                                                      \
    }                                                                        \
    info->name = S::HG == 1 ? "rollout_step_kernel" : "rollout_step128_kernel";\
    if constexpr (S::HG == 1)                                                \
      hipLaunchKernelGGL(rollout_step_kernel<S>, dim3(grid < ng ? grid : ng),\
                         dim3(256), rollout_lds<S>(), s, a);                 \
    else                                                                     \
      hipLaunchKernelGGL(rollout_step128_kernel<S>,                          \
                         dim3(grid < ng ? grid : ng), dim3(256),             \
                         rollout_lds<S>(), s, a);                            \
    return hipGetLastError();                                                \
  }
  XH_POLICY_SHAPES(X)
#undef X
  return hipErrorInvalidValue;
}

hipError_t launch_rollout_step(const RolloutArgs &a, int H1, int H2, int grid,
                               hipStream_t s, KernelInfo *info) {
  KernelInfo dummy;
  if (!info) info = &dummy;
  info->logit_table = false;
  const int n = a.nsteps > 1 ? a.nsteps : 1;
  bool multi = false;
  if (a.src_slot > 0 && !rollout_fetch_shifts(a, H1, H2)) {
    const size_t N = (size_t)a.b.N, BD = (size_t)a.env.B * a.env.D;
    hipError_t e = hipMemcpyAsync(a.b.bins, a.b.bins + (size_t)a.src_slot * N * BD,
                                  N * BD, hipMemcpyDeviceToDevice, s);
    if (e == hipSuccess)
      e = hipMemcpyAsync(a.b.items, a.b.items + (size_t)a.src_slot * N * 4, N * 4,
                         hipMemcpyDeviceToDevice, s);
    if (e != hipSuccess) return e;
    RolloutArgs a0 = a;
    a0.src_slot = -1;
    return launch_rollout_step(a0, H1, H2, grid, s, info);
  }
  if (a.e0_p && !a.qold_out) {
    RolloutArgs ap = a;
    ap.qold_out = a.e0_p;
    ap.e0_p = nullptr;
    return launch_rollout_step(ap, H1, H2, grid, s, info);
  }
  hipError_t e = launch_rollout_one(a, H1, H2, grid, s, info, multi);
  for (int k = 1; e == hipSuccess && !multi && k < n; ++k) {
    RolloutArgs ak = a;
    ak.t = a.t + k;
    ak.nsteps = n - k;
    ak.wide = 0;
    ak.src_slot = -1;
    e = launch_rollout_one(ak, H1, H2, grid, s, info, multi);
  }
  return e;
}

hipError_t launch_eval_argmax(const EvalArgs &a, int H1, int H2,
                              hipStream_t s) {
  const int B = a.env.B, D = a.env.D;
#define X(XB, XD, XH1, XH2)                                                  \
  if (B == XB && D == XD && H1 == XH1 && H2 == XH2) {                        \
    using S = PShape<XB, XD, XH1, XH2>;                                      \
    if constexpr (S::HG == 1) {                                              \
      constexpr size_t bytes =                                               \
          rollout_lds<S>() + sizeof(int) * (S::G * (S::BD + 4 + 2) + 4);     \
      static bool attr = false;                                              \
      if (!attr) {                                                           \
        (void)hipFuncSetAttribute((const void *)eval_argmax_kernel<S>,       \
                                  hipFuncAttributeMaxDynamicSharedMemorySize,\
                                  (int)bytes);                               \
        attr = true;                                                         \
      }                                                                      \
      const int ng = a.n_envs / S::G;                                        \
      hipLaunchKernelGGL(eval_argmax_kernel<S>,                              \
                         dim3(ng < 1024 ? ng : 1024), dim3(256), bytes, s, a);\
      return hipGetLastError();                                              \
    }                                                                        \
  }
  XH_POLICY_SHAPES(X)
#undef X
  return hipErrorInvalidValue;
}

hipError_t launch_policy_train(const PolicyTrainArgs &a, int H1, int H2,
                               int grid, hipStream_t s, KernelInfo *info) {
  const int B = a.env.B, D = a.env.D;
  KernelInfo dummy;
  if (!info) info = &dummy;
  info->math = kMathF32Mfma;
  if (policy_train_split_supported(a, H1, H2) && train_split_enabled() &&
      !a.wide)
    return launch_policy_train_split(a, grid, s, info);
#define X(XB, XD, XH1, XH2)                                                  \
  if (B == XB && D == XD && H1 == XH1 && H2 == XH2) {                        \
    using S = PShape<XB, XD, XH1, XH2>;                                      \
    static bool attr = false;                                                \
    if (!attr) {                                                             \
      if constexpr (S::HG == 1) {                                            \
        (void)hipFuncSetAttribute((const void *)policy_train_kernel<S, false>,\
                                  hipFuncAttributeMaxDynamicSharedMemorySize,\
                                  (int)train_lds<S>());                      \
        (void)hipFuncSetAttribute((const void *)policy_train_kernel<S, true>,\
                                  hipFuncAttributeMaxDynamicSharedMemorySize,\
                                  (int)train_lds<S>());                      \
      }                                                                      \
      if constexpr (S::NIT == 4 && S::NOT == 4)                              \
        (void)hipFuncSetAttribute((const void *)policy_train8_kernel<S>,     \
                                  hipFuncAttributeMaxDynamicSharedMemorySize,\
                                  (int)train_lds<S>());                      \
      attr = true;                                                           \
    }                                                                        \
    if (a.algo == kKLPPO) {                                                  \
      info->name = "policy_train_kernel<kl>";                                \
      if constexpr (S::HG == 1)                                              \
        hipLaunchKernelGGL((policy_train_kernel<S, true>), dim3(grid),       \
                           dim3(256), train_lds<S>(), s, a);                 \
      else                                                                   \
        return hipErrorInvalidValue;                                         \
      return hipGetLastError();                                              \
    }                                                                        \
    info->name = (S::NIT == 4 && S::NOT == 4 && (!XH_TRAIN4 || S::HG > 1))   \
                     ? "policy_train8_kernel" : "policy_train_kernel";       \
    if constexpr (S::NIT == 4 && S::NOT == 4 && (!XH_TRAIN4 || S::HG > 1))  \
      hipLaunchKernelGGL(policy_train8_kernel<S>, dim3(grid), dim3(512),     \
                         train_lds<S>(), s, a);                              \
    else if constexpr (S::HG == 1)                                           \
      hipLaunchKernelGGL((policy_train_kernel<S, false>), dim3(grid),        \
                         dim3(256), train_lds<S>(), s, a);                   \
    return hipGetLastError();                                                \
  }
  XH_POLICY_SHAPES(X)
#undef X
  return hipErrorInvalidValue;
}

template <int B>
__device__ __forceinline__ void diag_record(const DiagArgs &a, size_t row,
                                            double hterm, double kterm,
                                            float pa, bool writer) {
#pragma clang fp contract(off)
  const double hs = seg_sum_d<(B < 64 ? B : 64)>(hterm);
  const double ks = seg_sum_d<(B < 64 ? B : 64)>(kterm);
  if (writer) {
    a.p_new[row] = pa;
    a.ent[row] = -hs;
    a.kl[row] = a.q ? ks : __builtin_nan("");
  }
}

__device__ __forceinline__ void diag_bin_terms(float p, const float *q,
                                               double &hterm, double &kterm) {
#pragma clang fp contract(off)
  const double pd = (double)p, lp = log(pd);
  hterm += p == 0.0f ? 0.0 : pd * lp;
  if (q) {
    const float qf = *q;
    const double qd = (double)qf;
    kterm += qf == 0.0f ? 0.0 : qd * (log(qd) - lp);
  }
}

template <class S>
__device__ __forceinline__ void diag_step(const DiagArgs &a, int t, float z,
                                          int env, int seg0, int bin) {
  constexpr int B = S::B;
  const float ex = expf(z);
  const float sum = seg_sum<B>(ex);
  const float p = ex / sum;
  const size_t row = (size_t)t * a.b.N + env;
  const float pa = wave_shfl(p, seg0 + a.b.action[row]);
  double hterm = 0.0, kterm = 0.0;
  diag_bin_terms(p, a.q ? a.q + row * B + bin : nullptr, hterm, kterm);
  diag_record<B>(a, row, hterm, kterm, pa, bin == 0);
}

template <class S>
__device__ __forceinline__ void diag_step128(const DiagArgs &a, int t, int env,
                                             const float (&z)[2]) {
  const int lane = threadIdx.x & 63;
  float p[2];
  float se = 0.0f;
#pragma unroll
  for (int k = 0; k < 2; ++k) {
    p[k] = expf(z[k]);
    se += p[k];
  }
  se = seg_sum<64>(se);
  p[0] = p[0] / se;
  p[1] = p[1] / se;
  const size_t row = (size_t)t * a.b.N + env;
  const int act = a.b.action[row];
  const float pa = act < 64 ? wave_shfl(p[0], act) : wave_shfl(p[1], act - 64);
  double hterm = 0.0, kterm = 0.0;
#pragma unroll
  for (int k = 0; k < 2; ++k)
    diag_bin_terms(p[k], a.q ? a.q + row * 128 + k * 64 + lane : nullptr, hterm,
                   kterm);
  diag_record<128>(a, row, hterm, kterm, pa, lane == 0);
}

template <class S>
__global__ __launch_bounds__(256, 2) void policy_diag_kernel(DiagArgs a) {
  extern __shared__ __attribute__((aligned(16))) float lds[];
  stage_params<S>(a.params, lds);
  __syncthreads();
  const int lane = threadIdx.x & 63, w = threadIdx.x >> 6, lr = lane & 31;
  const int N = a.b.N;
  const int o2t = w % S::NOT;
  const int rt0 = S::NOT >= 4 ? 0 : w / S::NOT;
  const bool fwd_active = (w / S::NOT) * S::FJ < 2;
  if constexpr (S::HG == 1) {
    const int ngroups = N / S::G;
    const int njobs = a.b.T * ngroups;
    RowRaw<S> cur, nxt;
    if ((int)blockIdx.x < njobs)
      fetch_rows<S>(a.b, blockIdx.x / ngroups, (blockIdx.x % ngroups) * S::G, cur);
    for (int j = blockIdx.x; j < njobs; j += gridDim.x) {
      const int t = j / ngroups, e0 = (j - t * ngroups) * S::G;
      const int jn = j + gridDim.x;
      if (jn < njobs) fetch_rows<S>(a.b, jn / ngroups, (jn % ngroups) * S::G, nxt);
      {
        f32x16 h1[S::NIT][2];
        layer1<S>(cur, lds, h1);
        if (fwd_active) {
          f32x16 pre[S::FJ];
          layer2<S, S::FJ>(lds, h1, o2t, rt0, pre);
#pragma unroll
          for (int q = 0; q < S::FJ; ++q) {
            const float zp = logit_part<S>(lds, pre[q], o2t);
            if (lane < 32) lds[S::L_Z + o2t * 64 + (rt0 + q) * 32 + lr] = zp;
          }
        }
      }
      __syncthreads();
      if (w == 0) {
        constexpr int B = S::B;
        const int e = lane / B, bin = lane % B, env = e0 + e, seg0 = e * B;
        float zs = 0.0f;
#pragma unroll
        for (int o = 0; o < S::NOT; ++o) zs += lds[S::L_Z + o * 64 + lane];
        const float z = zs + lds[S::L_B3];
        diag_step<S>(a, t, z, env, seg0, bin);
      }
      __syncthreads();
      cur = nxt;
    }
  } else {
    static_assert(S::B == 128 && S::HG == 2, "128-bin form");
    constexpr int R = S::R;
    const int njobs = a.b.T * N;
    for (int j = blockIdx.x; j < njobs; j += gridDim.x) {
      const int t = j / N, env = j - t * N;
#pragma unroll
      for (int hg = 0; hg < 2; ++hg) {
        RowRaw<S> rr;
#pragma unroll
        for (int k = 0; k < 2; ++k) {
          const int bin = hg * 64 + k * 32 + lr;
          const size_t e = (size_t)t * N + env;
          const int8_t *bp = a.b.bins + e * S::BD + bin * S::D;
          const int8_t *ip = a.b.items + e * 4;
#pragma unroll
          for (int d = 0; d < S::D; ++d) {
            rr.bv[k][d] = bp[d];
            rr.iv[k][d] = ip[d];
          }
        }
        f32x16 h1[S::NIT][2];
        layer1<S>(rr, lds, h1);
        if (fwd_active) {
          f32x16 pre[S::FJ];
          layer2<S, S::FJ>(lds, h1, o2t, rt0, pre);
#pragma unroll
          for (int q = 0; q < S::FJ; ++q) {
            const float zp = logit_part<S>(lds, pre[q], o2t);
            if (lane < 32) lds[S::L_Z + o2t * R + hg * 64 + (rt0 + q) * 32 + lr] = zp;
          }
        }
      }
      __syncthreads();
      if (w == 0) {
        float z[2];
#pragma unroll
        for (int k = 0; k < 2; ++k) {
          float zs = 0.0f;
#pragma unroll
          for (int o = 0; o < S::NOT; ++o) zs += lds[S::L_Z + o * R + k * 64 + lane];
          z[k] = zs + lds[S::L_B3];
        }
        diag_step128<S>(a, t, env, z);
      }
      __syncthreads();
    }
  }
}

template <class S>
__global__ __launch_bounds__(64 * roll_split_waves<S>(), roll_split_occ<S>()) void policy_diag_split_kernel(DiagArgs a) {
  static_assert((S::B == 64 && S::NIT == 4 && S::NOT == 4) ||
                    (S::B == 32 && S::NIT == 2 && S::NOT == 2),
                "split form: B=64 [128,128] or B=32 [64,64]");
  extern __shared__ __attribute__((aligned(16))) float ldsf[];
  char *lds = reinterpret_cast<char *>(ldsf);
  stage_split_rollout<S>(a.params, a.env, lds);
  __syncthreads();
  const float *lfr = reinterpret_cast<const float *>(lds + RollSplitLds<S>::F);
  const float b3 = lfr[RollSplitLds<S>::B3];
  const float *b1fa = lfr + RollSplitLds<S>::B1F, *b1fb = b1fa + S::H1;
  const int lane = threadIdx.x & 63, w = threadIdx.x >> 6, h = lane >> 5, lr = lane & 31;
  const int wpb = blockDim.x >> 6;
  const int ngroups = a.b.N / S::G;
  const int eoff = S::G == 2 ? h : 0, seg0 = S::G == 2 ? 32 * h : 0;
  const int bin = S::G == 2 ? lr : lane;
  const int per = (ngroups + (int)gridDim.x - 1) / (int)gridDim.x;
  const int g_end = min(ngroups, ((int)blockIdx.x + 1) * per);
  for (int g = (int)blockIdx.x * per + w; g < g_end; g += wpb) {
    const int e0 = g * S::G, env = e0 + eoff;
    for (int t = 0; t < a.b.T; ++t) {
      RowRaw<S> cur;
      fetch_rows<S>(a.b, t, e0, cur);
      const float *b1r[2];
#pragma unroll
      for (int rt = 0; rt < 2; ++rt) {
        bool ia = true;
#pragma unroll
        for (int d = 0; d < S::D; ++d) ia &= cur.iv[rt][d] == a.env.item_a[d];
        b1r[rt] = ia ? b1fa : b1fb;
      }
      float zl[2];
      wave_logits_split<S>(lds, cur, b1r, zl);
      const float z = (h ? zl[1] : zl[0]) + b3;
      diag_step<S>(a, t, z, env, seg0, bin);
    }
  }
}

hipError_t launch_policy_diag(const DiagArgs &a, int H1, int H2, int wide,
                              int grid, hipStream_t s, KernelInfo *info) {
  const int B = a.env.B, D = a.env.D;
  KernelInfo dummy;
  if (!info) info = &dummy;
  info->math = kMathF32Mfma;
#define X(XB, XD, XH1, XH2)                                                  \
  if (B == XB && D == XD && H1 == XH1 && H2 == XH2) {                        \
    using S = PShape<XB, XD, XH1, XH2>;                                      \
    const int ng = a.b.N / S::G;                                             \
    if constexpr ((S::B == 64 && S::NIT == 4 && S::NOT == 4) ||             \
                  (S::B == 32 && S::NIT == 2 && S::NOT == 2)) {              \
      if (rollout_split() && !wide) {                                        \
        static bool sattr = false;                                           \
        if (!sattr) {                                                        \
          (void)hipFuncSetAttribute(                                         \
              (const void *)policy_diag_split_kernel<S>,                     \
              hipFuncAttributeMaxDynamicSharedMemorySize,                    \
              (int)RollSplitLds<S>::bytes);                                  \
          sattr = true;                                                      \
        }                                                                    \
        constexpr int kRW = roll_split_waves<S>();                           \
        const int wg = (ng + kRW - 1) / kRW;                                 \
        const int wgr = S::B == 64 ? (kRW == 8 ? grid : cu_count()) : wg;    \
        info->name = "policy_diag_split_kernel";                             \
        info->math = kMathSplitRollout;                                      \
        hipLaunchKernelGGL(policy_diag_split_kernel<S>,                      \
                           dim3(wgr < wg ? wgr : wg), dim3(64 * kRW),        \
                           RollSplitLds<S>::bytes, s, a);                    \
        return hipGetLastError();                                            \
      }                                                                      \
    }                                                                        \
    static bool attr = false;                                                \
    if (!attr) {                                                             \
      (void)hipFuncSetAttribute((const void *)policy_diag_kernel<S>,         \
                                hipFuncAttributeMaxDynamicSharedMemorySize,  \
                                (int)rollout_lds<S>());                      \
      attr = true;                                                           \
    }                                                                        \
    const long jobs = (long)a.b.T * ng;                                      \
    info->name = "policy_diag_kernel";                                       \
    hipLaunchKernelGGL(policy_diag_kernel<S>,                                \
                       dim3((unsigned)(grid < jobs ? grid : jobs)),          \
                       dim3(256), rollout_lds<S>(), s, a);                   \
    return hipGetLastError();                                                \
  }
  XH_POLICY_SHAPES(X)
#undef X
  return hipErrorInvalidValue;
}

}
```

### dependence_free_rl_amd/csrc/trainer_diag.cpp

```cpp
#include <hip/hip_runtime.h>

#include <cmath>
#include <cstdio>
#include <cstdlib>
#include <cstring>
#include <string>

#include "../../include/xylo_hip.h"
#include "spec8_pack_layout.h"
#include "spec8_table_layout.h"
#include "xh_host.h"
#include "xh_kernels.h"
#include "xh_trainer.h"

namespace xh {
namespace host {

void stats_free(xh_trainer *t) {
  auto &st = t->stats;
  if (st.ring.dev) (void)hipFree(st.ring.dev);
  if (st.part) (void)hipFree(st.part);
  if (st.norms) (void)hipFree(st.norms);
  if (st.ep_len) (void)hipFree(st.ep_len);
  st = xh_trainer::stats_state{};
}

int stats_rollout(xh_trainer *t) {
  auto &st = t->stats;
  hipStream_t s = t->ctx->stream;
  const int N = (int)t->N(), T = (int)t->T();
  double *row = ring_row(st.ring, st.ring.rows);
  CHK(timed(t, "stats", [&]() {
    return xh::launch_episode_stats(t->done, t->pold, N, T, st.ep_len, st.part,
                                    s);
  }));
  CHK(timed(t, "stats", [&]() {
    return xh::launch_episode_row(st.part, xh::gae_grid(N),
                                  (double)st.ring.rows,
                                  (double)T * t->cfg.num_envs_global,
                                  (double)T * N, row, s);
  }));
  CHK(allreduce_d(t, row + XH_STAT_EPISODES, xh::kStatEpisodeSummed));
  ++st.ring.rows;
  st.open = true;
  return XH_OK;
}

int stats_learn(xh_trainer *t) {
  auto &st = t->stats;
  if (!st.open) return XH_OK;
  hipStream_t s = t->ctx->stream;
  const int N = (int)t->N(), T = (int)t->T();
  double *row = ring_row(st.ring, st.ring.rows - 1);
  CHK(timed(t, "stats", [&]() {
    return xh::launch_learner_stats(t->v_state0, t->targets, t->adv, N, T,
                                    st.part, s);
  }));
  CHK(timed(t, "stats", [&]() {
    return xh::launch_grad_norms(
        t->pgrads, t->pgrads + (size_t)(t->cfg.epochs - 1) * t->np, t->np,
        t->vgrad, t->nv, st.norms, s);
  }));
  CHK(timed(t, "stats", [&]() {
    return xh::launch_learner_row(
        st.part, xh::gae_grid(N), st.norms,
        t->kl_log ? t->kl_log + 3 * (size_t)(t->cfg.epochs - 1) : nullptr,
        t->clip[XH_POLICY].log, t->cfg.epochs, t->clip[XH_VALUE].log, row, s);
  }));
  CHK(allreduce_d(t, row + XH_STAT_VERR_SUM, xh::kStatLearnerSums));
  st.open = false;
  return XH_OK;
}

void upd_free(xh_trainer *t) {
  if (t->upd.ring.dev) (void)hipFree(t->upd.ring.dev);
  t->upd = xh_trainer::upd_state{};
}

int upd_learn(xh_trainer *t, bool e0_at_entry) {
  auto &u = t->upd;
  const long learn = u.learns++;
  if (learn % u.every) return XH_OK;
  hipStream_t s = t->ctx->stream;
  const int N = (int)t->N(), T = (int)t->T();
  xh::DiagArgs a{};
  a.env = t->env;
  a.b = t->batch();
  a.params = t->pp;
  a.q = t->qold ? t->qold : (e0_at_entry && t->e0_p ? t->e0_p : nullptr);
  u.kl_source = t->qold ? "qold" : (a.q ? "e0_p" : nullptr);
  a.p_new = u.p_new;
  a.ent = u.ent;
  a.kl = u.kl;
  const int wide = batch_wide(t);
  double *row = ring_row(u.ring, u.ring.rows);
  CHK(timed(t, "probe", [&]() {
    return xh::launch_policy_diag(a, t->cfg.policy_h1, t->cfg.policy_h2, wide,
                                  t->rgrid, s, &u.info);
  }));
  CHK(timed(t, "probe", [&]() {
    return xh::launch_update_diag_sum(u.p_new, t->pold, t->adv, u.ent, u.kl, N,
                                      T, t->cfg.clip_eps, u.part, s);
  }));
  CHK(timed(t, "probe", [&]() {
    return xh::launch_update_diag_row(u.part, xh::gae_grid(N), (double)learn,
                                      (double)T * t->cfg.num_envs_global, row,
                                      s);
  }));
  CHK(allreduce_d(t, row + XH_UPD_LOGR_SUM, xh::kUpdSums));
  ++u.ring.rows;
  return XH_OK;
}

void clip_free(xh_trainer *t, int which) {
  auto &c = t->clip[which];
  if (c.part) (void)hipFree(c.part);
  c = xh_trainer::clip_state{};
}

namespace {

constexpr int kMaxStatsRows = 1 << 20;
constexpr int kMaxUpdRows = 1 << 20;

int upd_ready(const xh_trainer *t, const char *who, bool probed) {
  if (!t->upd.ring.history)
    return fail(XH_ERR_STATE, "%s: the diagnostics are off "
                "(xh_trainer_set_update_diag)", who);
  if (probed && !t->upd.ring.rows)
    return fail(XH_ERR_STATE, "%s: no probed learn() since "
                "xh_trainer_set_update_diag", who);
  return XH_OK;
}

int clip_log_rows(const xh_trainer *t, int which) {
  return which == XH_POLICY && t->cfg.algo != XH_PG ? t->cfg.epochs : 1;
}

constexpr double kBf16DensePeakTflops = 2500.0;
constexpr double kF32MfmaPeakTflops = 157.3;

std::string kernel_json(const xh::KernelInfo &k) {
  char buf[640];
  if (!k.name) return "{\"kernel\": null}";
  const double prod = k.math == xh::kMathSplitTrain      ? 4.0
                      : k.math == xh::kMathSplitRollout  ? 3.0
                      : k.math == xh::kMathSplitTrainF16 ||
                                k.math == xh::kMathSplitTrainF16Pair
                          ? 8.0 / 3.0
                          : 0.0;
  const bool bf16 = k.math == xh::kMathSplitTrain;
  const char *math = prod == 0.0                         ? "f32_mfma"
                     : bf16                              ? "bf16_split"
                     : k.math == xh::kMathSplitRollout   ? "f16_pair"
                                                         : "f16_pair_bf16_split";
  char products[32] = "null";
  if (prod > 0) std::snprintf(products, sizeof products, "%.6g", prod);
  int n = std::snprintf(buf, sizeof buf,
                        "{\"kernel\": \"%s\", \"math\": \"%s\", "
                        "\"bf16_products_per_f32_product\": %s, "
                        "\"products_per_f32_product\": %s, \"peak_tflops\": %.6g",
                        k.name, math, bf16 ? products : "null", products,
                        prod > 0 ? kBf16DensePeakTflops / prod
                                 : kF32MfmaPeakTflops);
  if (k.math == xh::kMathSplitTrainF16Pair) {
    const double issued = 7.0 / 3.0;
    std::snprintf(buf + n, sizeof buf - n,
                  ", \"dw2_math\": \"f16_pair_per_feature_scale\", "
                  "\"issued_math\": \"f16_pair_train\", "
                  "\"issued_products_per_f32_product\": %.6g, "
                  "\"issued_peak_tflops\": %.6g",
                  issued, kBf16DensePeakTflops / issued);
  }
  return std::string(buf) + "}";
}

std::string env_json(const char *name) {
  const char *v = std::getenv(name);
  if (!v) return std::string("\"") + name + "\": null";
  std::string out = std::string("\"") + name + "\": \"";
  for (const char *p = v; *p; ++p)
    if (*p != '"' && *p != '\\' && (unsigned char)*p >= 32) out += *p;
  return out + "\"";
}

}
}
}

using namespace xh::host;

extern "C" {

int xh_trainer_set_stats(xh_trainer *t, int history_rows) {
  return guard([&]() -> int {
    if (!t) return fail(XH_ERR_INVALID, "null trainer");
    if (t->cfg.algo == XH_PG)
      return fail(XH_ERR_INVALID, "set_stats: not for XH_PG trainers (REINFORCE "
                  "plays whole episodes: XH_BUF_LEN)");
    if (history_rows < 0 || history_rows > kMaxStatsRows)
      return fail(XH_ERR_INVALID, "set_stats: history_rows %d not in [0, %d]",
                  history_rows, kMaxStatsRows);
    HIPCHK(hipSetDevice(t->ctx->device));
    hipStream_t s = t->ctx->stream;
    HIPCHK(hipStreamSynchronize(s));
    stats_free(t);
    if (history_rows == 0) return XH_OK;
    auto &st = t->stats;
    const size_t ring = (size_t)history_rows * XH_STAT_COUNT * 8,
                 part = (size_t)xh::gae_grid((int)t->N()) *
                        xh::kStatLearnerSums * 8;
    hipError_t e = hipMalloc((void **)&st.ring.dev, ring);
    if (e == hipSuccess) e = hipMalloc((void **)&st.part, part);
    if (e == hipSuccess) e = hipMalloc((void **)&st.norms, 3 * 8);
    if (e == hipSuccess) e = hipMalloc((void **)&st.ep_len, t->N() * 4);
    if (e == hipSuccess) e = hipMemsetAsync(st.ring.dev, 0xFF, ring, s);
    if (e == hipSuccess) e = hipMemsetAsync(st.ep_len, 0, t->N() * 4, s);
    if (e == hipSuccess) e = hipStreamSynchronize(s);
    if (e != hipSuccess) {
      stats_free(t);
      return fail(XH_ERR_HIP, "set_stats(%d): %s", history_rows,
                  hipGetErrorString(e));
    }
    st.ring.history = history_rows;
    return XH_OK;
  });
}

int xh_trainer_stats_count(xh_trainer *t, long *total_rows) {
  return guard([&]() -> int {
    if (!t || !total_rows) return fail(XH_ERR_INVALID, "null arg");
    if (!t->stats.ring.history)
      return fail(XH_ERR_STATE, "stats_count: statistics are off "
                  "(xh_trainer_set_stats)");
    *total_rows = t->stats.ring.rows;
    return XH_OK;
  });
}

int xh_trainer_get_stats(xh_trainer *t, long first, int count, double *out) {
  return guard([&]() -> int {
    if (!t || (count > 0 && !out)) return fail(XH_ERR_INVALID, "null arg");
    if (!t->stats.ring.history)
      return fail(XH_ERR_STATE, "get_stats: statistics are off "
                  "(xh_trainer_set_stats)");
    return ring_read(t->stats.ring, t->ctx, first, count, out, "get_stats");
  });
}

int xh_trainer_set_update_diag(xh_trainer *t, int history_rows, int every) {
  return guard([&]() -> int {
    if (!t) return fail(XH_ERR_INVALID, "null trainer");
    if (t->cfg.algo == XH_PG)
      return fail(XH_ERR_INVALID, "set_update_diag: not for XH_PG trainers "
                  "(REINFORCE has no old policy to compare with)");
    if (history_rows < 0 || history_rows > kMaxUpdRows)
      return fail(XH_ERR_INVALID, "set_update_diag: history_rows %d not in "
                  "[0, %d]", history_rows, kMaxUpdRows);
    if (history_rows > 0 && every < 1)
      return fail(XH_ERR_INVALID, "set_update_diag: every %d (>= 1)", every);
    HIPCHK(hipSetDevice(t->ctx->device));
    hipStream_t s = t->ctx->stream;
    HIPCHK(hipStreamSynchronize(s));
    upd_free(t);
    if (history_rows == 0) return XH_OK;
    auto &u = t->upd;
    const size_t rows = t->T() * t->N();
    const size_t ring = (size_t)history_rows * XH_UPD_COUNT,
                 part = (size_t)xh::gae_grid((int)t->N()) * xh::kUpdSums;
    const size_t bytes = (ring + part + 2 * rows) * 8 + rows * 4;
    hipError_t e = hipMalloc((void **)&u.ring.dev, bytes);
    if (e == hipSuccess) e = hipMemsetAsync(u.ring.dev, 0xFF, bytes, s);
    if (e == hipSuccess) e = hipStreamSynchronize(s);
    if (e != hipSuccess) {
      upd_free(t);
      return fail(XH_ERR_HIP, "set_update_diag(%d, %d): %s", history_rows, every,
                  hipGetErrorString(e));
    }
    u.part = u.ring.dev + ring;
    u.ent = u.part + part;
    u.kl = u.ent + rows;
    u.p_new = reinterpret_cast<float *>(u.kl + rows);
    u.ring.history = history_rows;
    u.every = every;
    return XH_OK;
  });
}

int xh_trainer_update_diag_count(xh_trainer *t, long *total_rows) {
  return guard([&]() -> int {
    if (!t || !total_rows) return fail(XH_ERR_INVALID, "null arg");
    CHK(upd_ready(t, "update_diag_count", false));
    *total_rows = t->upd.ring.rows;
    return XH_OK;
  });
}

int xh_trainer_get_update_diag(xh_trainer *t, long first, int count, double *out) {
  return guard([&]() -> int {
    if (!t || (count > 0 && !out)) return fail(XH_ERR_INVALID, "null arg");
    CHK(upd_ready(t, "get_update_diag", true));
    return ring_read(t->upd.ring, t->ctx, first, count, out, "get_update_diag");
  });
}

int xh_trainer_get_update_diag_rows(xh_trainer *t, float *p_new, double *entropy,
                                    double *kl, size_t n) {
  return guard([&]() -> int {
    if (!t) return fail(XH_ERR_INVALID, "null trainer");
    const auto &u = t->upd;
    CHK(upd_ready(t, "get_update_diag_rows", true));
    const size_t rows = t->T() * t->N();
    if (n != rows)
      return fail(XH_ERR_INVALID, "get_update_diag_rows: n %zu, the batch has "
                  "%zu transitions", n, rows);
    HIPCHK(hipSetDevice(t->ctx->device));
    hipStream_t s = t->ctx->stream;
    HIPCHK(hipStreamSynchronize(s));
    if (p_new) HIPCHK(copy_to_host(p_new, u.p_new, rows * 4, s));
    if (entropy) HIPCHK(copy_to_host(entropy, u.ent, rows * 8, s));
    if (kl) HIPCHK(copy_to_host(kl, u.kl, rows * 8, s));
    return XH_OK;
  });
}

int xh_trainer_update_diag_info(xh_trainer *t, char *buf, size_t cap) {
  return guard([&]() -> int {
    if (!t || !buf || cap == 0) return fail(XH_ERR_INVALID, "null arg");
    const auto &u = t->upd;
    CHK(upd_ready(t, "update_diag_info", false));
    auto quoted = [](const char *v) {
      return v ? "\"" + std::string(v) + "\"" : std::string("null");
    };
    const std::string js =
        "{\"kernel\": " + quoted(u.info.name) + ", \"math\": " +
        quoted(u.info.math == xh::kMathSplitRollout ? "f16_pair" : "f32_mfma") +
        ", \"kl_source\": " + quoted(u.kl_source) + ", \"history_rows\": " +
        std::to_string(u.ring.history) + ", \"every\": " +
        std::to_string(u.every) + "}";
    if (js.size() + 1 > cap)
      return fail(XH_ERR_INVALID, "update_diag_info: %zu bytes needed",
                  js.size() + 1);
    std::memcpy(buf, js.c_str(), js.size() + 1);
    return XH_OK;
  });
}

int xh_trainer_set_grad_clip(xh_trainer *t, int which, float max_norm) {
  return guard([&]() -> int {
    if (!t) return fail(XH_ERR_INVALID, "null trainer");
    if (which != XH_POLICY && which != XH_VALUE)
      return fail(XH_ERR_INVALID, "grad clip: which %d", which);
    if (which == XH_VALUE && t->cfg.algo == XH_PG)
      return fail(XH_ERR_INVALID, "grad clip: REINFORCE has no value net");
    if (!(max_norm >= 0.0f) || std::isinf(max_norm))
      return fail(XH_ERR_INVALID, "grad clip: max_norm %g (a finite norm > 0, "
                  "or 0 for off)", (double)max_norm);
    HIPCHK(hipSetDevice(t->ctx->device));
    hipStream_t s = t->ctx->stream;
    HIPCHK(hipStreamSynchronize(s));
    auto &c = t->clip[which];
    if (max_norm == 0.0f) {
      clip_free(t, which);
      return XH_OK;
    }
    if (!c.part) {
      const size_t bytes =
          ((size_t)xh::kClipMaxParts + 2 * (size_t)clip_log_rows(t, which)) * 8;
      hipError_t e = hipMalloc((void **)&c.part, bytes);
      if (e == hipSuccess) e = hipMemsetAsync(c.part, 0, bytes, s);
      if (e == hipSuccess) e = hipStreamSynchronize(s);
      if (e != hipSuccess) {
        clip_free(t, which);
        return fail(XH_ERR_HIP, "grad clip: %s", hipGetErrorString(e));
      }
      c.log = c.part + xh::kClipMaxParts;
    }
    c.max_norm = max_norm;
    c.learned = false;
    return XH_OK;
  });
}

int xh_trainer_get_grad_clip_log(xh_trainer *t, int which, double *out,
                                 int cap_rows, int *rows) {
  return guard([&]() -> int {
    if (!t || !out || !rows) return fail(XH_ERR_INVALID, "null arg");
    if (which != XH_POLICY && which != XH_VALUE)
      return fail(XH_ERR_INVALID, "grad clip log: which %d", which);
    const auto &c = t->clip[which];
    if (!c.part)
      return fail(XH_ERR_STATE, "grad clip log: clipping is off for net %d "
                  "(xh_trainer_set_grad_clip)", which);
    if (!c.learned)
      return fail(XH_ERR_STATE, "grad clip log: no learn() since "
                  "xh_trainer_set_grad_clip");
    const int n = clip_log_rows(t, which);
    if (cap_rows < n)
      return fail(XH_ERR_INVALID, "grad clip log: room for %d rows, the log has "
                  "%d", cap_rows, n);
    HIPCHK(hipSetDevice(t->ctx->device));
    HIPCHK(copy_to_host(out, c.log, (size_t)n * 16, t->ctx->stream));
    *rows = n;
    return XH_OK;
  });
}

int xh_trainer_set_timing(xh_trainer *t, int on) {
  if (!t) return fail(XH_ERR_INVALID, "null trainer");
  if (on < 0 || on > XH_TIMING_TRAIN)
    return fail(XH_ERR_INVALID, "set_timing: mode %d (0, 1 or XH_TIMING_TRAIN)", on);
  t->timing = on;
  return XH_OK;
}

int xh_trainer_reset_timing(xh_trainer *t) {
  return guard([&]() -> int {
    if (!t) return fail(XH_ERR_INVALID, "null trainer");
    HIPCHK(hipStreamSynchronize(t->ctx->stream));
    for (auto &ev : t->events) {
      t->event_pool.push_back(ev.start);
      t->event_pool.push_back(ev.stop);
    }
    t->events.clear();
    return XH_OK;
  });
}

int xh_trainer_kernel_info(xh_trainer *t, char *buf, size_t cap) {
  return guard([&]() -> int {
    if (!t || !buf || cap == 0) return fail(XH_ERR_INVALID, "null arg");
    std::string roll = kernel_json(t->last_rollout);
    roll.insert(roll.size() - 1, std::string(", \"logit_table\": ") +
                                     (t->last_rollout.logit_table ? "true" : "false"));
    const std::string js = "{\"rollout_step\": " + roll +
                           ", \"policy_train\": " + kernel_json(t->last_train) +
                           ", \"value\": \"" +
                           std::string(t->cfg.algo != XH_PG
                                           ? xh::value_kernel_name(value_mlp(t, 0, nullptr))
                                           : "gemm") +
                           "\", \"train_grid\": " + std::to_string(t->pslab_n) +
                           ", \"train_grid_cap\": " +
                           std::to_string(t->cfg.train_grid_cap) +
                           ", \"overrides\": {" + env_json("XH_TRAIN_KERNEL") +
                           ", " + env_json("XH_ROLLOUT_KERNEL") + ", " +
                           env_json("XH_VALUE_KERNEL") + "}}";
    if (js.size() + 1 > cap)
      return fail(XH_ERR_INVALID, "kernel_info: %zu bytes needed", js.size() + 1);
    std::memcpy(buf, js.c_str(), js.size() + 1);
    return XH_OK;
  });
}

int xh_trainer_pack_stats(xh_trainer *t, long *packed, long *unpacked, long *groups) {
  return guard([&]() -> int {
    if (!t || !packed || !unpacked || !groups) return fail(XH_ERR_INVALID, "null arg");
    *packed = *unpacked = *groups = 0;
    if (!t->pk_hdr || !t->pk_learned) return XH_OK;
    int h[xh::sp8::kPkHdrInts];
    HIPCHK(hipMemcpyAsync(h, t->pk_hdr, sizeof(h), hipMemcpyDeviceToHost, t->ctx->stream));
    HIPCHK(hipStreamSynchronize(t->ctx->stream));
    *packed = (long)h[xh::sp8::kPkNA] + h[xh::sp8::kPkNB];
    *unpacked = (long)h[xh::sp8::kPkUA] + h[xh::sp8::kPkUB];
    *groups = h[xh::sp8::kPkGroups];
    return XH_OK;
  });
}

int xh_trainer_pack_read(xh_trainer *t, int *hdr, void *records, size_t cap) {
  return guard([&]() -> int {
    if (!t || !hdr) return fail(XH_ERR_INVALID, "null arg");
    if (!t->pk || !t->pk_hdr || !t->pk_learned)
      return fail(XH_ERR_STATE, "pack_read: the last learn() did not run packed");
    HIPCHK(hipMemcpyAsync(hdr, t->pk_hdr, xh::sp8::kPkHdrInts * sizeof(int),
                          hipMemcpyDeviceToHost, t->ctx->stream));
    HIPCHK(hipStreamSynchronize(t->ctx->stream));
    if (!records) return XH_OK;
    const size_t groups = (size_t)hdr[xh::sp8::kPkGroups];
    const size_t bytes = groups * xh::sp8::kPkGroupBytes;
    if (hdr[xh::sp8::kPkGroups] < 0 ||
        groups > xh::sp8::pk_max_groups((size_t)(t->T() * t->N())))
      return fail(XH_ERR_STATE, "pack_read: a header of %d groups", hdr[xh::sp8::kPkGroups]);
    if (bytes > cap) return fail(XH_ERR_INVALID, "pack_read: %zu bytes needed", bytes);
    HIPCHK(hipMemcpyAsync(records, t->pk, bytes, hipMemcpyDeviceToHost, t->ctx->stream));
    HIPCHK(hipStreamSynchronize(t->ctx->stream));
    return XH_OK;
  });
}

int xh_trainer_table_stats(xh_trainer *t, int *ran, long *out_of_domain, long *groups) {
  return guard([&]() -> int {
    if (!t || !ran || !out_of_domain || !groups) return fail(XH_ERR_INVALID, "null arg");
    *ran = 0;
    *out_of_domain = *groups = 0;
    if (!t->tab_ood || !t->tab_learned) return XH_OK;
    int ood = 0;
    HIPCHK(hipMemcpyAsync(&ood, t->tab_ood, sizeof(ood), hipMemcpyDeviceToHost, t->ctx->stream));
    HIPCHK(hipStreamSynchronize(t->ctx->stream));
    *ran = 1;
    *out_of_domain = ood;
    *groups = xh::tb::kGroups;
    return XH_OK;
  });
}

int xh_trainer_kernel_time(xh_trainer *t, const char *name, double *ms,
                           long *launches) {
  return guard([&]() -> int {
    if (!t || !name || !ms || !launches) return fail(XH_ERR_INVALID, "null arg");
    HIPCHK(hipStreamSynchronize(t->ctx->stream));
    double total = 0;
    long n = 0;
    for (auto &ev : t->events) {
      if (ev.name != name) continue;
      float e = 0;
      HIPCHK(hipEventElapsedTime(&e, ev.start, ev.stop));
      total += e;
      ++n;
    }
    *ms = total;
    *launches = n;
    return XH_OK;
  });
}

}
```

### dependence_free_rl_amd/csrc/xh_kernels.h

```cpp
#pragma once
#include <hip/hip_runtime.h>
#include <stdint.h>

namespace xh {

enum Algo { kPPO = 0, kAC = 1, kKLPPO = 2 };
enum Heuristic { kHeurRandom = 0, kHeurFirstfit = 1, kHeurBestfit = 2,
                 kHeurMinwaste = 3 };

struct PolicyLayout {
  int F0, H1, H2;
  __host__ __device__ int oW1() const { return 0; }
  __host__ __device__ int ob1() const { return H1 * F0; }
  __host__ __device__ int oW2() const { return ob1() + H1; }
  __host__ __device__ int ob2() const { return oW2() + H2 * H1; }
  __host__ __device__ int ow3() const { return ob2() + H2; }
  __host__ __device__ int ob3() const { return ow3() + H2; }
  __host__ __device__ int size() const { return ob3() + 1; }
};

struct ValueLayout {
  int Fin, V1, V2;
  __host__ __device__ int oW1() const { return 0; }
  __host__ __device__ int ob1() const { return V1 * Fin; }
  __host__ __device__ int oW2() const { return ob1() + V1; }
  __host__ __device__ int ob2() const { return oW2() + V2 * V1; }
  __host__ __device__ int ow3() const { return ob2() + V2; }
  __host__ __device__ int ob3() const { return ow3() + V2; }
  __host__ __device__ int size() const { return ob3() + 1; }
};

struct EnvDesc {
  int B, D;
  int item_a[3], item_b[3];
  double p_a;
};

struct Batch {
  int N, T;
  int8_t *bins;
  int8_t *items;
  int32_t *action;
  float *pold;
  uint8_t *done;
  uint32_t *rng;
};

struct RolloutArgs {
  EnvDesc env;
  Batch b;
  int t;
  uint32_t jump_mul;
  const float *params;
  const int32_t *forced;
  float *logits_out;
  float *probs_out;
  float *qold_out;
  int wide;
  int wide_seen;
  int src_slot;
  int nsteps;
  float *e0_p;
  uint32_t *e0_mask;
};

struct PolicyTrainE0Args {
  const float *e0_p;
  const uint32_t *e0_mask;
};

struct PolicyTrainArgs {
  EnvDesc env;
  Batch b;
  int algo;
  float clip_eps;
  const float *params;
  const float *adv;
  const float *g_bound;
  float *slab;
  int slab_stride;
  int wide;
  int ablate;
  const float *qold;
  const float *beta;
  const int *end_list;
  const int *n_end;
  double *kl_part;
  long long *trace;
  const uint8_t *pk;
  const int *pk_hdr;
};
constexpr int kTraceBlocks = 4, kTraceGroups = 32, kTraceSlots = 8;

struct EndListArgs {
  const uint8_t *done;
  int N, T;
  int *end_list;
  int *n_end;
  int *n_open;
  int *rows_out;
  int rows_base;
};
int end_list_scratch_ints(int N);
hipError_t launch_scatter_list(const int *list, const int *n, const float *src,
                               float *dst, int max_n, hipStream_t s);

struct ValueArgs {
  EnvDesc env;
  Batch b;
  float *v_state;
  float *v_term;
  float *row_g;
};

struct EvalArgs {
  EnvDesc env;
  const float *params;
  int n_envs;
  int episodes;
  int argmax_probs;
  uint32_t x0;
  uint64_t stream_stride;
  long max_steps;
  const int *init_items;
  double *total;
  long *steps;
  int *final_items;
  uint32_t *rng_out;
  int *trace;
  long trace_cap;
};

struct HeuristicArgs {
  EnvDesc env;
  int n_envs;
  int episodes;
  uint32_t x0;
  uint64_t stream_stride;
  long max_steps;
  const int *init_items;
  double *total;
  long *steps;
  int *final_items;
  uint32_t *rng_out;
  int *trace;
  long trace_cap;
};
struct MlpArgs {
  EnvDesc env;
  const int8_t *bins, *items;
  const int *list;
  int N, slot;
  const int32_t *action;
  int term_from;
  const int *term_list;
  const int *rows;
  int max_rows;
  float *w0red;
  int nlayers;
  int w[4];
  const float *params;
  float *act[3];
  float *grad[3];
  float *v_term;
  const int *term_n;
  void *w0frag;
  int act_rows;
  int w0frag_ready;
};
hipError_t mlp_forward(const MlpArgs &a, hipStream_t s);
hipError_t mlp_backward(const MlpArgs &a, float *slab, int stride, int splits,
                        hipStream_t s);
hipError_t value_backward(const MlpArgs &a, const ValueArgs &va, float gamma,
                          float *targets, float *slab, int stride, int splits,
                          hipStream_t s);
const char *value_kernel_name(const MlpArgs &a);
bool value_reduced_slab(const MlpArgs &a);
bool vnet_shape_ok(const MlpArgs &a);
size_t vnet_frag_bytes(const EnvDesc &e);
hipError_t vnet_forward(const MlpArgs &a, hipStream_t s);
hipError_t vnet_backward(const MlpArgs &a, const ValueArgs &va, float gamma,
                         float *targets, float *slab, int stride, int splits,
                         hipStream_t s);

enum LayerKind { kLayerFull = 0, kLayerConv1d = 1, kLayerRelu = 2,
                 kLayerSoftmax = 3, kLayerSoftmaxXent = 4 };
struct ModelLayer {
  int kind, in, out;
};
hipError_t model_forward(const ModelLayer *layers, int nl, const float *params,
                         const float *x, int rows, int cols, float *a, float *b,
                         const float **out, int *out_cols, hipStream_t s);
hipError_t layer_forward(const ModelLayer &L, const float *W, const float *x,
                         int rows, int cols, float *y, hipStream_t s);
hipError_t layer_backward(const ModelLayer &L, const float *W, const float *x,
                          int rows, int cols, const float *bp, float *out,
                          hipStream_t s);
int layer_gradient_splits(const ModelLayer &L, int rows, int cols);
hipError_t layer_gradient(const ModelLayer &L, const float *x, int rows,
                          int cols, const float *bp, float *slab, int stride,
                          float *grad, hipStream_t s);
enum LossKind { kLossGradientLog = 0, kLossSoftmaxGradientLog = 1,
                kLossClipped = 2, kLossKlRegulated = 3 };
hipError_t launch_action_loss(int kind, int rows, int range,
                              const int32_t *choice, const float *distrib,
                              const float *adv, const float *probs, float param,
                              float *out, hipStream_t s);

struct PgStepArgs {
  EnvDesc env;
  Batch b;
  int t, episodes;
  const float *logits;
  const int32_t *forced;
  int *ep_done, *len, *active;
};
struct PgLearnArgs {
  int N, B, episodes;
  float gamma;
  const int *len;
  int *row_off, *list, *nrows;
  const uint8_t *done;
  const int32_t *action;
  float *rtg;
  double *ep_part;
  double *stats;
  const float *logits;
  float *dlogits;
  float *adv_grid;
};
hipError_t launch_pg_env_init(const EnvDesc &env, Batch b, uint32_t x0,
                              int env_offset, uint64_t stride, hipStream_t s);
hipError_t launch_pg_seed(Batch b, uint32_t x, int env_offset, uint64_t stride,
                          hipStream_t s);
hipError_t launch_pg_begin(int N, int *active, int *ep_done, int *len,
                           hipStream_t s);
hipError_t launch_pg_step(const PgStepArgs &a, hipStream_t s);
hipError_t launch_pg_rows(const PgLearnArgs &a, hipStream_t s);
hipError_t launch_pg_adv(const PgLearnArgs &a, hipStream_t s);
hipError_t launch_pg_loss(const PgLearnArgs &a, int max_rows, hipStream_t s);

enum VenvOp { kVenvStep = 0, kVenvReset = 1, kVenvObserve = 2 };
struct VenvEpAcc {
  int32_t count;
  int32_t len_min, len_max;
  int32_t pad;
  int64_t len_sum;
  uint64_t len_sqsum;
};
static_assert(sizeof(VenvEpAcc) == 32, "one env's accumulators are 32 bytes");
struct VenvArgs {
  EnvDesc env;
  int N;
  int8_t *bins, *items;
  uint32_t *rng;
  const int32_t *action;
  const uint8_t *mask;
  float *reward;
  uint8_t *done;
  float *obs;
  int *err;
  int mode;
  uint32_t skip_mul;
  uint32_t jump_mul;
  int32_t *ep_running;
  int32_t *ep_first;
  VenvEpAcc *ep_acc;
};
struct VenvActArgs {
  VenvArgs v;
  const float *policy;
  int32_t *action;
  float *pchoice;
  int logits;
  int argmax;
  int32_t *rec_action;
  float *rec_pchoice;
  float *rec_reward;
  uint8_t *rec_done;
  int8_t *rec_bins;
  int8_t *rec_items;
  int slot;
  int legal;
  float *rec_distrib;
  uint32_t *rec_legal;
};
inline int venv_legal_words(int B) { return B >= 32 ? B / 32 : 1; }
constexpr int kVenvItemsMax = 16;
struct VenvItemTable {
  double thr[kVenvItemsMax];
  uint32_t shape[kVenvItemsMax];
  int32_t cap[4];
};
bool venv_shape_supported(int B, int D);
hipError_t launch_venv(const VenvArgs &a, int op, hipStream_t s,
                       const VenvItemTable *items = nullptr);
hipError_t launch_venv_act(const VenvActArgs &a, hipStream_t s,
                           const VenvItemTable *items = nullptr);
hipError_t launch_venv_gen(const VenvArgs &a, int op, hipStream_t s,
                           const VenvItemTable &items);
hipError_t launch_venv_act_gen(const VenvActArgs &a, hipStream_t s,
                               const VenvItemTable &items);
struct VenvHeurArgs {
  VenvActArgs a;
  int heur;
};
hipError_t launch_venv_heur(const VenvHeurArgs &h, hipStream_t s,
                            const VenvItemTable *items = nullptr);
hipError_t launch_venv_heur_gen(const VenvHeurArgs &h, hipStream_t s,
                                const VenvItemTable &items);
struct VenvTabDomain {
  int D, K;
  int side[4];
  int states;
  long entries;
};
hipError_t launch_venv_table_obs(const VenvTabDomain &m,
                                 const VenvItemTable &t, long total,
                                 float *obs, hipStream_t s);
struct VenvTabActArgs {
  VenvActArgs a;
  VenvTabDomain m;
  const float *table;
};
hipError_t launch_venv_act_table(const VenvTabActArgs &h, hipStream_t s,
                                 const VenvItemTable &t);
struct VenvTabRowArgs {
  int B, D, N;
  int P;
  VenvTabDomain m;
  const int8_t *rec_bins;
  const int8_t *rec_items;
  const int8_t *cur_bins;
  const int8_t *cur_items;
  const int32_t *rows;
  long first, count;
  const float *table;
  float *out;
  const float *dout;
  uint32_t *maxbits;
  unsigned long long *acc;
  int *err;
};
hipError_t launch_venv_table_gather(const VenvTabRowArgs &a, hipStream_t s,
                                    const VenvItemTable &t);
hipError_t launch_venv_table_grad(const VenvTabRowArgs &a, long total,
                                  int accumulate, float *g, hipStream_t s,
                                  const VenvItemTable &t);
hipError_t launch_venv_legal(const VenvArgs &a, uint32_t *out, hipStream_t s);
hipError_t launch_venv_init(const VenvArgs &a, uint32_t x0, int env_offset,
                            int n_global, int k, hipStream_t s,
                            const VenvItemTable *items = nullptr);
hipError_t launch_venv_init_gen(const VenvArgs &a, uint32_t x0, int env_offset,
                                int n_global, int k, hipStream_t s,
                                const VenvItemTable &items);

hipError_t launch_venv_ep_init(int N, int32_t *running, int32_t *first,
                               VenvEpAcc *acc, hipStream_t s);
constexpr int kVepSums = 7;
constexpr int kVepExts = 3;
int venv_ep_grid(int N);
hipError_t launch_venv_ep_row(int N, const int32_t *running,
                              const int32_t *first, VenvEpAcc *acc,
                              double *psum, double *pext, double row_index,
                              double calls, double *row, hipStream_t s);

struct VenvObsArgs {
  int B, D, N;
  int P;
  int next;
  const int8_t *rec_bins;
  const int8_t *rec_items;
  const int8_t *cur_bins;
  const int8_t *cur_items;
  const int32_t *rec_action;
  const uint8_t *rec_done;
  const int32_t *rows;
  long first, count;
  float *obs;
  int *err;
};
hipError_t launch_venv_record_obs(const VenvObsArgs &a, hipStream_t s,
                                  const int32_t *cap = nullptr);
struct VenvGaeArgs {
  int N, T;
  const float *values;
  const float *v_term;
  const float *reward;
  const uint8_t *done;
  float gamma, lambda;
  float *adv;
  float *td_target;
  float *lambda_return;
  double *part;
  int *end_part;
};
int venv_gae_grid(int N);
hipError_t launch_venv_gae(const VenvGaeArgs &a, hipStream_t s);
hipError_t launch_venv_adv_counts(const int *end_part, int nparts, double rows,
                                  double *stats, hipStream_t s);
constexpr int kVenvLossMaxBlocks = 4096;
struct VenvLossArgs {
  int B;
  int logits;
  int loss;
  const float *policy;
  const int32_t *rows;
  long first, count, total;
  long tiles;
  const float *adv;
  const int32_t *action;
  const float *p_old;
  float eps, scale;
  const float *values_new;
  const float *target;
  float value_scale;
  float *grad;
  float *dvalue;
  float *probs_out;
  double *part;
  int *err;
  const float *distrib;
  float beta;
  const float *beta_dev;
  double *kl_part;
  const uint32_t *legal;
  int ext;
  float ent_coef;
  const float *ent_coef_dev;
  const float *v_old;
  float vclip;
  double *ext_part;
};
int venv_loss_grid(int B, long count);
hipError_t launch_venv_policy_loss(VenvLossArgs a, hipStream_t s);
hipError_t launch_venv_loss_reduce(const double *part, int nparts,
                                   int accumulate, double *stats,
                                   hipStream_t s);
hipError_t launch_venv_kl_reduce(const double *part, int nparts, int accumulate,
                                 double *kl_stats, hipStream_t s);
hipError_t launch_venv_ext_reduce(const double *part, int nparts,
                                  int accumulate, double *ext_stats,
                                  hipStream_t s);

struct NetPolicyArgs {
  int F0, H1, H2;
  const float *params;
  const float *obs;
  long R;
  float *logits;
  const float *dout;
  float *slab;
  int slab_stride;
};
bool net_policy_shape_supported(int F0, int H1, int H2);
long net_policy_tiles(long R);
int net_policy_lds_bytes(int F0, int H1, int H2, int backward);
hipError_t launch_net_policy_fwd(const NetPolicyArgs &a, int grid, hipStream_t s);
hipError_t launch_net_policy_bwd(const NetPolicyArgs &a, int grid, hipStream_t s);

struct NetValueArgs {
  VenvObsArgs rec;
  int32_t cap[4];
  const float *params;
  float *out;
  const float *dout;
  float *slab;
  int slab_stride;
};
constexpr int kNetValueV1 = 64, kNetValueV2 = 32;
long net_value_tiles(long count);
int net_value_lds_bytes(int backward);
hipError_t launch_net_value_fwd(const NetValueArgs &a, int grid, hipStream_t s);
hipError_t launch_net_value_bwd(const NetValueArgs &a, int grid, hipStream_t s);

int diag_build();

bool heuristic_shape_supported(int B, int D);
hipError_t launch_heuristic(const HeuristicArgs &a, int kind, hipStream_t s);

bool policy_shape_supported(int B, int D, int H1, int H2);
hipError_t launch_env_init(const EnvDesc &env, Batch b, uint32_t x0,
                           int env_offset, int n_global, hipStream_t s);
hipError_t launch_env_seed(Batch b, uint32_t x, int env_offset,
                           hipStream_t s);
hipError_t launch_end_list(const EndListArgs &a, int *scratch, hipStream_t s);
hipError_t launch_kl_reduce(const double *kl_part, int nparts, const int *n_end,
                            const int *n_open, double rows_main,
                            double *kl_sum, hipStream_t s);
hipError_t launch_kl_beta_update(const double *kl_sum, float *beta,
                                 float d_targ, float *log, hipStream_t s);
enum Math {
  kMathF32Mfma = 0,
  kMathSplitTrain = 1,
  kMathSplitRollout = 2,
  kMathSplitTrainF16 = 3,
  kMathSplitTrainF16Pair = 4
};
struct KernelInfo {
  const char *name = nullptr;
  int math = kMathF32Mfma;
  bool logit_table = false;
};
hipError_t launch_rollout_step(const RolloutArgs &a, int H1, int H2, int grid,
                               hipStream_t s, KernelInfo *info = nullptr);
hipError_t launch_policy_train(const PolicyTrainArgs &a, int H1, int H2,
                               int grid, hipStream_t s,
                               KernelInfo *info = nullptr);
constexpr int kSplit128Bins = 128, kSplit128Dims = 3;
constexpr int kSplit4hBins = 32;
bool train_split_enabled();
bool policy_train_split_supported(const PolicyTrainArgs &a, int H1, int H2);
hipError_t launch_policy_train_split(const PolicyTrainArgs &a, int grid,
                                     hipStream_t s, KernelInfo *info);
hipError_t launch_policy_train_split128(const PolicyTrainArgs &a, int grid,
                                        hipStream_t s);
hipError_t launch_policy_train_split8w(const PolicyTrainArgs &a, int grid,
                                       hipStream_t s);
hipError_t launch_policy_train_split8wp(const PolicyTrainArgs &a, int grid,
                                        hipStream_t s);
hipError_t launch_policy_train_split4p(const PolicyTrainArgs &a, int grid,
                                       hipStream_t s);
hipError_t launch_policy_train_split8wh(const PolicyTrainArgs &a, int grid,
                                        hipStream_t s);
hipError_t launch_policy_train_split8wh_kl(const PolicyTrainArgs &a, int grid,
                                           hipStream_t s);
hipError_t launch_policy_train_spec8(const PolicyTrainArgs &a, int grid, hipStream_t s);
hipError_t launch_policy_train_spec8_kl(const PolicyTrainArgs &a, int grid, hipStream_t s);
hipError_t launch_policy_train_spec8_e0(const PolicyTrainArgs &a, const PolicyTrainE0Args &ea,
                                        int grid, hipStream_t s);
hipError_t launch_policy_train_spec8_pack(const PolicyTrainArgs &a, int grid, hipStream_t s);
struct PackArgs {
  EnvDesc env;
  Batch b;
  const float *adv;
  uint8_t *pk;
  int *hdr;
  uint8_t *cls;
  int *blk;
};
hipError_t launch_spec8_pack(const PackArgs &a, bool loop, hipStream_t s);
struct PolicyTrainTabArgs {
  float *logits;
  const float *G;
  int forward;
};
hipError_t launch_policy_train_spec8_tab(const PolicyTrainArgs &a, const PolicyTrainTabArgs &ta,
                                         int grid, hipStream_t s);
struct TableStreamArgs {
  const uint8_t *pk;
  const int *pk_hdr;
  const float *logits;
  int algo;
  float clip_eps;
  double *part;
  float *G;
  float *gmax;
  int *ood;
};
hipError_t launch_table_stream(const TableStreamArgs &a, int grid, hipStream_t s,
                               bool reduce = true);
struct TableFwdArgs {
  EnvDesc env;
  const float *params;
  float *logits;
  float *h2;
  int *zero_ood;
};
struct TableBwdArgs {
  EnvDesc env;
  const float *params;
  const float *h2;
  const double *part;
  int nparts;
  float *G;
  float *slab;
  int slab_stride;
};
hipError_t launch_table_fwd(const TableFwdArgs &a, hipStream_t s);
hipError_t launch_table_bwd(const TableBwdArgs &a, hipStream_t s);
hipError_t launch_policy_train_spec8_3p(const PolicyTrainArgs &a, int grid, hipStream_t s);
hipError_t launch_policy_train_spec4(const PolicyTrainArgs &a, int grid, hipStream_t s);
bool train_spec4_default(int B, int D, int H1, int H2, int kl);
hipError_t launch_policy_train_split8wg(const PolicyTrainArgs &a, int grid,
                                       hipStream_t s);
hipError_t launch_policy_train_split4h(const PolicyTrainArgs &a, int grid,
                                       hipStream_t s);
hipError_t launch_policy_train_split4h_kl(const PolicyTrainArgs &a, int grid,
                                          hipStream_t s);
hipError_t launch_policy_train_split8x(const PolicyTrainArgs &a, int grid,
                                       hipStream_t s);
hipError_t launch_policy_train_split8x_kl(const PolicyTrainArgs &a, int grid,
                                          hipStream_t s);
int policy_train_grid(int B, int D, int H1, int H2, int kl);
hipError_t launch_eval_argmax(const EvalArgs &a, int H1, int H2,
                              hipStream_t s);
int rollout_grid(int B, int D, int H1, int H2);

bool value_shape_supported(int V1, int V2);
hipError_t launch_value_targets(const ValueArgs &a, float gamma, float *targets,
                                hipStream_t s);
int gae_grid(int N);
hipError_t launch_gae(const ValueArgs &a, float gamma, float lambda, float *adv,
                      double *part, hipStream_t s);
hipError_t launch_adv_stats(const double *part, int nparts, double *stats,
                            hipStream_t s);
hipError_t launch_adv_normalize(float *adv, long n, const double *stats,
                                double count, hipStream_t s);
hipError_t launch_g_bound(const float *adv, const float *pold, long n, int ppo,
                          float clip_eps, float *out, hipStream_t s);

constexpr int kStatEpisodeSums = 4;
constexpr int kStatEpisodeSummed = 5;
constexpr int kStatLearnerSums = 6;
hipError_t launch_episode_stats(const uint8_t *done, const float *pold, int N,
                                int T, int *ep_len, double *part,
                                hipStream_t s);
hipError_t launch_episode_row(const double *part, int nparts, double iter,
                              double transitions_global,
                              double transitions_local, double *row,
                              hipStream_t s);
hipError_t launch_learner_stats(const float *v0, const float *targets,
                                const float *adv, int N, int T, double *part,
                                hipStream_t s);
hipError_t launch_grad_norms(const float *g_first, const float *g_last, int np,
                             const float *gv, int nv, double *out,
                             hipStream_t s);
hipError_t launch_learner_row(const double *part, int nparts,
                              const double *norms, const float *kl_last,
                              const double *pclip, int psteps,
                              const double *vclip, double *row, hipStream_t s);
struct DiagArgs {
  EnvDesc env;
  Batch b;
  const float *params;
  const float *q;
  float *p_new;
  double *ent;
  double *kl;
};
constexpr int kUpdSums = 7;
hipError_t launch_policy_diag(const DiagArgs &a, int H1, int H2, int wide,
                              int grid, hipStream_t s, KernelInfo *info);
hipError_t launch_update_diag_sum(const float *p_new, const float *pold,
                                  const float *adv, const double *ent,
                                  const double *kl, int N, int T, float clip_eps,
                                  double *part, hipStream_t s);
hipError_t launch_update_diag_row(const double *part, int nparts, double learn,
                                  double rows_global, double *row,
                                  hipStream_t s);

struct SlabAlias {
  int rows, in, B, D;
};
hipError_t launch_slab_reduce(const float *slab, int nslab, int stride, int n,
                              float *out, hipStream_t s,
                              SlabAlias al = SlabAlias{0, 0, 0, 0});
hipError_t launch_sgd(float *params, const float *grad, int n, float lr,
                      float wd, hipStream_t s);
struct OptStep {
  int kind;
  float lr, beta1, beta2, c1, c2;
  float wd;
};
hipError_t launch_opt(float *params, const float *grad, float *m, float *v,
                      int n, OptStep o, hipStream_t s);
hipError_t launch_slab_reduce_opt(const float *slab, int nslab, int stride,
                                  int n, float *out, float *params, float *m,
                                  float *v, OptStep o, hipStream_t s,
                                  SlabAlias al = SlabAlias{0, 0, 0, 0});

constexpr int kClipMaxParts = 256;
int clip_parts(int n);
hipError_t launch_clip_sumsq(const float *g, int n, double *part,
                             hipStream_t s);
hipError_t launch_clip_step(const double *part, double r, float max_norm,
                            const float *g, float *params, float *m, float *v,
                            int n, OptStep o, float *scaled, double *log,
                            hipStream_t s);

constexpr int kDigestMaxEntries = 10;
constexpr int kDigestBlocks = 128;
constexpr int kDigestWsWords = kDigestMaxEntries * (kDigestBlocks + 1);
struct DigestTable {
  struct {
    const void *ptr;
    unsigned long long bytes;
  } e[kDigestMaxEntries];
  int n;
};
inline unsigned long long *digest_results(unsigned long long *ws) {
  return ws + kDigestMaxEntries * kDigestBlocks;
}
hipError_t launch_digest(const DigestTable &tab, unsigned long long *ws,
                         hipStream_t s);

enum TensorMapOp {
  kTensorAdd = 0, kTensorMinus = 1, kTensorMultiply = 2, kTensorDivide = 3,
  kTensorAddS = 4, kTensorMinusS = 5, kTensorMultiplyS = 6, kTensorDivideS = 7,
  kTensorAbs = 8, kTensorSin = 9, kTensorExp = 10, kTensorLog = 11,
  kTensorSqrt = 12, kTensorFill = 13, kTensorRMinusS = 14, kTensorRDivideS = 15
};
enum TensorReduceOp {
  kTensorSum = 0, kTensorDot = 1, kTensorSqDev = 2, kTensorMax = 3,
  kTensorArgmax = 4
};
hipError_t launch_tensor_map(int op, const float *a, const float *b, float s,
                             float *out, long n, hipStream_t st);
int tensor_reduce_parts(long n);
hipError_t launch_tensor_reduce(int op, const float *a, const float *b, float s,
                                long n, void *scratch, hipStream_t st);
hipError_t launch_tensor_transpose(const float *in, float *out, int rows,
                                   int cols, hipStream_t st);
hipError_t launch_tensor_gemm(bool b_nk, const float *A, const float *B,
                              float *C, int M, int N, int K, hipStream_t st);

}
```

Baseline: 312.1 million.

## Add packed-lane rollout kernel that splits each wave across several envs

Adds a new rollout kernel for the logit-table path that packs several environments per wave, giving each env a segment of L lanes and doing the per-env reductions and scans with DPP segment operations. It becomes the default table path unless XH_ROLLOUT_TABLE=1 selects the old one-env-per-wave kernel. Shared rollout split helpers move into a new header so both kernels can use them. The aim is to stop idling most of a 64-lane wave on a 64-bin env when logits come from a table lookup; the cost is more per-lane work, since each lane handles several bins.

New measurement: 369.1 million, median of 6. 18.2% higher.

```diff
diff --git a/dependence_free_rl_amd/csrc/policy_kernels.hip b/dependence_free_rl_amd/csrc/policy_kernels.hip
--- a/dependence_free_rl_amd/csrc/policy_kernels.hip
+++ b/dependence_free_rl_amd/csrc/policy_kernels.hip
@@ -2,6 +2,7 @@
 #include "xh_device.h"
 #include "xh_kernels.h"
 #include "xh_logit_table.h"
+#include "xh_roll_split.h"
 #include "xh_split.h"
 
 #include <cstdlib>
@@ -60,103 +61,6 @@
 
 namespace xh {
 
-template <int B_, int D_, int H1_, int H2_>
-struct PShape {
-  static constexpr int B = B_, D = D_, H1 = H1_, H2 = H2_;
-  static constexpr int F0 = 2 * D;
-  static constexpr int S1 = (F0 + 1) / 2;
-  static constexpr int NIT = H1 / 32, NOT = H2 / 32;
-  static constexpr int G = B <= 64 ? 64 / B : 1;
-  static constexpr int HG = B <= 64 ? 1 : B / 64;
-  static constexpr int R = 64 * HG;
-  static constexpr int BD = B * D;
-  static constexpr int W2S = H1 + 4;
-  static constexpr int HS = H1 + 1;
-  static constexpr int AS = H2 + 1;
-  static constexpr int FJ = NOT >= 4 ? 2 : 1;
-  static constexpr int JW = (NOT * NIT + 3) / 4;
-  static constexpr int JH = (2 * NIT + 3) / 4;
-  static constexpr int TOCC = (H1 <= 64 && H2 <= 64 && D == 1) ? 2 : 1;
-  static_assert(B == 8 || B == 16 || B == 32 || B == 64 || B == 128, "B");
-  static_assert(NIT == 1 || NIT == 2 || NIT == 4, "H1 in {32,64,128}");
-  static_assert(NOT == 1 || NOT == 2 || NOT == 4, "H2 in {32,64,128}");
-  static_assert(D >= 1 && D <= 3, "D");
-  static constexpr int r4(int x) { return (x + 3) & ~3; }
-  static constexpr int L_W2 = 0;
-  static constexpr int L_W1 = L_W2 + H2 * W2S;
-  static constexpr int L_B1 = L_W1 + r4(H1 * F0);
-  static constexpr int L_B2 = L_B1 + H1;
-  static constexpr int L_W3 = L_B2 + H2;
-  static constexpr int L_B3 = L_W3 + H2;
-  static constexpr int L_Z = L_B3 + 4;
-  static constexpr int L_ROLLOUT_END = L_Z + NOT * R;
-  static constexpr int L_H1 = L_ROLLOUT_END;
-  static constexpr int L_DA2 = L_H1 + r4(64 * HS);
-  static constexpr int L_TRAIN_END = L_DA2 + r4(64 * AS);
-  static constexpr int TS = 68;
-  static constexpr int L_H1T = L_ROLLOUT_END;
-  static constexpr int L_DAT = L_H1T + H1 * TS;
-  static constexpr int L_B1F = L_DAT + H2 * TS;
-  static constexpr int L_TRAIN8_END = L_B1F + 2 * H1;
-  static constexpr int RED = H1 * F0 + H1 + 2 * H2 + 1;
-  static_assert(4 * RED <= 64 * HS + 64 * AS, "scratch fits");
-};
-
-template <class S>
-__device__ __forceinline__ void stage_params(const float *__restrict__ P,
-                                             float *lds) {
-  const PolicyLayout L{S::F0, S::H1, S::H2};
-  const int tid = threadIdx.x;
-  for (int i = tid; i < S::H2 * S::H1; i += blockDim.x) {
-    const int o = i / S::H1, k = i - o * S::H1;
-    lds[S::L_W2 + o * S::W2S + k] = P[L.oW2() + i];
-  }
-  for (int i = tid; i < S::H1 * S::F0; i += blockDim.x)
-    lds[S::L_W1 + i] = P[L.oW1() + i];
-  for (int i = tid; i < S::H1; i += blockDim.x) lds[S::L_B1 + i] = P[L.ob1() + i];
-  for (int i = tid; i < S::H2; i += blockDim.x) {
-    lds[S::L_B2 + i] = P[L.ob2() + i];
-    lds[S::L_W3 + i] = P[L.ow3() + i];
-  }
-  if (tid == 0) lds[S::L_B3] = P[L.ob3()];
-}
-
-template <class S>
-struct RowRaw {
-  int bv[2][S::D];
-  int iv[2][S::D];
-};
-
-template <class S>
-__device__ __forceinline__ void fetch_rows(const Batch &b, int slot, int e0,
-                                           RowRaw<S> &rr) {
-  const int lr = threadIdx.x & 31;
-#pragma unroll
-  for (int rt = 0; rt < 2; ++rt) {
-    const int r = rt * 32 + lr;
-    const size_t env = (size_t)slot * b.N + e0 + r / S::B;
-    const int8_t *bp = b.bins + env * S::BD + (r % S::B) * S::D;
-    const int8_t *ip = b.items + env * 4;
-#pragma unroll
-    for (int d = 0; d < S::D; ++d) {
-      rr.bv[rt][d] = bp[d];
-      rr.iv[rt][d] = ip[d];
-    }
-  }
-}
-
-template <class S>
-__device__ __forceinline__ float row_feature(const RowRaw<S> &rr, int rt,
-                                             int f) {
-  int v = 0;
-#pragma unroll
-  for (int d = 0; d < S::D; ++d) {
-    if (f == d) v = rr.bv[rt][d];
-    if (f == S::D + d) v = rr.iv[rt][d];
-  }
-  return f < S::F0 ? (float)v / (float)kCapacity : 0.0f;
-}
-
 __device__ __forceinline__ float4 lds4(const float *p) {
   return *reinterpret_cast<const float4 *>(p);
 }
@@ -522,226 +426,9 @@
 }
 
 template <class S>
-struct RollSplitLds {
-  static constexpr int W2 = 0;
-  static constexpr int F = 2 * S::H2 * kImgRow;
-  static constexpr int W1 = 0, B1 = S::H1 * S::F0, B2 = B1 + S::H1, W3 = B2 + S::H2,
-                       B3 = W3 + S::H2, SH = B3 + 1, SC = B3 + 4, B1F = SC + 2 * 16;
-  static constexpr int S1F = (S::D + 1) / 2;
-  static constexpr size_t bytes = F + sizeof(float) * (B1F + 2 * S::H1);
-};
-
-template <class S>
-__device__ __forceinline__ void stage_split_rollout(const float *__restrict__ P,
-                                                    const EnvDesc &env, char *lds) {
-  using L = RollSplitLds<S>;
-  float *lf = reinterpret_cast<float *>(lds + L::F);
-  const PolicyLayout PL{S::F0, S::H1, S::H2};
-  float mw = 0.0f, mh = 0.0f;
-  for (int e = threadIdx.x; e < S::H2 * S::H1; e += blockDim.x)
-    mw = fmaxf(mw, fabsf(P[PL.oW2() + e]));
-  for (int i = threadIdx.x; i < S::H1; i += blockDim.x) {
-    float v = fabsf(P[PL.ob1() + i]);
-    for (int k = 0; k < S::F0; ++k) v += fabsf(P[PL.oW1() + i * S::F0 + k]);
-    mh = fmaxf(mh, v);
-  }
-#pragma unroll
-  for (int o = 1; o < 64; o <<= 1) {
-    mw = fmaxf(mw, __shfl_xor(mw, o, kWave));
-    mh = fmaxf(mh, __shfl_xor(mh, o, kWave));
-  }
-  const int nw = blockDim.x >> 6, wv = threadIdx.x >> 6;
-  if ((threadIdx.x & 63) == 0) {
-    lf[L::SC + wv] = mw;
-    lf[L::SC + 16 + wv] = mh;
-  }
-  __syncthreads();
-  float MW = 0.0f, MH = 0.0f;
-  for (int v = 0; v < nw; ++v) {
-    MW = fmaxf(MW, lf[L::SC + v]);
-    MH = fmaxf(MH, lf[L::SC + 16 + v]);
-  }
-  const float SW = f16_scale_for(MW), SH = f16_scale_for(MH), S2 = SW * SH;
-  for (int e = threadIdx.x; e < S::H2 * S::H1; e += blockDim.x) {
-    const int o = e / S::H1, i = e % S::H1;
-    const int c = (i & ~12) | ((i & 4) << 1) | ((i & 8) >> 1);
-    _Float16 x0, x1;
-    split2h(P[PL.oW2() + e] * SW, x0, x1);
-    const int off = img_off(o, c >> 3) + 2 * (c & 7);
-    *reinterpret_cast<_Float16 *>(lds + L::W2 + off) = x0;
-    *reinterpret_cast<_Float16 *>(lds + L::W2 + S::H2 * kImgRow + off) = x1;
-  }
-  for (int i = threadIdx.x; i < S::H1 * S::F0; i += blockDim.x)
-    lf[L::W1 + i] = P[PL.oW1() + i] * SH;
-  for (int i = threadIdx.x; i < S::H1; i += blockDim.x) {
-    lf[L::B1 + i] = P[PL.ob1() + i] * SH;
-    lf[L::B2 + i] = P[PL.ob2() + i] * S2;
-    lf[L::W3 + i] = P[PL.ow3() + i] * (1.0f / S2);
-    float ba = P[PL.ob1() + i], bb = ba;
-#pragma unroll
-    for (int d = 0; d < S::D; ++d) {
-      const float wv = P[PL.oW1() + i * S::F0 + S::D + d];
-      ba += wv * ((float)env.item_a[d] / (float)kCapacity);
-      bb += wv * ((float)env.item_b[d] / (float)kCapacity);
-    }
-    lf[L::B1F + i] = ba * SH;
-    lf[L::B1F + S::H1 + i] = bb * SH;
-  }
-  if (threadIdx.x == 0) {
-    lf[L::B3] = P[PL.ob3()];
-    lf[L::SH] = SH;
-  }
-}
-
-template <class S, bool E0 = false>
-__device__ __forceinline__ void wave_logits_split(const char *lds,
-                                                  const RowRaw<S> &cur,
-                                                  const float *const (&b1r)[2],
-                                                  float (&zl)[2],
-                                                  unsigned *mbits = nullptr) {
-  using L = RollSplitLds<S>;
-  const float *lf = reinterpret_cast<const float *>(lds + L::F);
-  const int lane = threadIdx.x & 63, lr = lane & 31, h = lane >> 5;
-  const char *w2i[2] = {lds + L::W2, lds + L::W2 + S::H2 * kImgRow};
-#pragma unroll
-  for (int rt = 0; rt < 2; ++rt) {
-    float xb[L::S1F];
-#pragma unroll
-    for (int s1 = 0; s1 < L::S1F; ++s1) {
-      const int f = 2 * s1 + h;
-      xb[s1] = f < S::D ? row_feature<S>(cur, rt, f) : 0.0f;
-    }
-    f32x16s pre[S::NOT];
-#pragma unroll
-    for (int ot = 0; ot < S::NOT; ++ot)
-#pragma unroll
-      for (int q = 0; q < 4; ++q) {
-        const float4 bb = *reinterpret_cast<const float4 *>(lf + L::B2 + ot * 32 + 8 * q + 4 * h);
-        pre[ot][4 * q + 0] = bb.x;
-        pre[ot][4 * q + 1] = bb.y;
-        pre[ot][4 * q + 2] = bb.z;
-        pre[ot][4 * q + 3] = bb.w;
-      }
-#pragma unroll
-    for (int it = 0; it < S::NIT; ++it) {
-      f32x16 t1;
-#pragma unroll
-      for (int q = 0; q < 4; ++q) {
-        const float4 bb = *reinterpret_cast<const float4 *>(b1r[rt] + it * 32 + 8 * q + 4 * h);
-        t1[4 * q + 0] = bb.x;
-        t1[4 * q + 1] = bb.y;
-        t1[4 * q + 2] = bb.z;
-        t1[4 * q + 3] = bb.w;
-      }
-#pragma unroll
-      for (int s1 = 0; s1 < L::S1F; ++s1) {
-        const int k = 2 * s1 + h;
-        const float wa = k < S::D ? lf[L::W1 + (it * 32 + lr) * S::F0 + k] : 0.0f;
-        t1 = mfma32(wa, xb[s1], t1);
-      }
-      f16x8 bfr[2][2];
-      {
-        typedef unsigned u32x4_t __attribute__((ext_vector_type(4)));
-        u32x4_t hb[2], lb[2];
-#pragma unroll
-        for (int jj = 0; jj < 8; ++jj) {
-          unsigned h2, l2;
-          split2h_x2(relu(t1[2 * jj]), relu(t1[2 * jj + 1]), h2, l2);
-          hb[jj >> 2][jj & 3] = h2;
-          lb[jj >> 2][jj & 3] = l2;
-        }
-#pragma unroll
-        for (int s = 0; s < 2; ++s) {
-          bfr[s][0] = __builtin_bit_cast(f16x8, hb[s]);
-          bfr[s][1] = __builtin_bit_cast(f16x8, lb[s]);
-        }
-      }
-#pragma unroll
-      for (int ot = 0; ot < S::NOT; ++ot) {
-        const int rb = row_base(ot * 32 + lr, h);
-#pragma unroll
-        for (int s = 0; s < 2; ++s) {
-          f16x8 af[2];
-#pragma unroll
-          for (int p = 0; p < 2; ++p)
-            af[p] = __builtin_bit_cast(f16x8, ld_row(w2i[p], rb, 2 * it + s));
-          pre[ot] = mfma_f16(af[1], bfr[s][0], pre[ot]);
-          pre[ot] = mfma_f16(af[0], bfr[s][1], pre[ot]);
-          pre[ot] = mfma_f16(af[0], bfr[s][0], pre[ot]);
-        }
-        __builtin_amdgcn_sched_barrier(0);
-      }
-    }
-    float z = 0.0f;
-#pragma unroll
-    for (int ot = 0; ot < S::NOT; ++ot) {
-      float zp = 0.0f;
-#pragma unroll
-      for (int q = 0; q < 4; ++q) {
-        const float4 ww = *reinterpret_cast<const float4 *>(lf + L::W3 + ot * 32 + 8 * q + 4 * h);
-        const float wq[4] = {ww.x, ww.y, ww.z, ww.w};
-#pragma unroll
-        for (int u = 0; u < 4; ++u) zp = fmaf(relu(pre[ot][4 * q + u]), wq[u], zp);
-      }
-      z += zp + __shfl_xor(zp, 32, kWave);
-    }
-    zl[rt] = z;
-    if constexpr (E0) {
-#pragma unroll
-      for (int ot = 0; ot < S::NOT; ++ot) {
-        unsigned wd = rt == 0 ? 0u : mbits[ot];
-#pragma unroll
-        for (int e = 0; e < 16; ++e) {
-          int m;
-          asm("v_med3_i32 %0, %1, 0, 1" : "=v"(m) : "v"(__float_as_int(pre[ot][e])));
-          wd |= (unsigned)m << sp8::e0_bit(rt, e);
-        }
-        mbits[ot] = wd;
-      }
-    }
-  }
-}
-
-template <class S>
 constexpr int roll_split_waves() { return S::B == 64 ? kRollWaves64 : 4; }
 template <class S>
 constexpr int roll_split_occ() { return S::B == 64 ? roll_occ(kRollWaves64) : 2; }
-
-template <class S>
-__device__ __forceinline__ void build_logit_table(const char *lds, float *out) {
-  static_assert(S::B == 64 && S::D == 2 && S::G == 1 && lt::kCap == kCapacity,
-                "the logit table: 64 bins, 2-D");
-  const float *lfr = reinterpret_cast<const float *>(lds + RollSplitLds<S>::F);
-  const float *const b1r[2] = {lfr + RollSplitLds<S>::B1F,
-                               lfr + RollSplitLds<S>::B1F + S::H1};
-  const int lane = threadIdx.x & 63, w = threadIdx.x >> 6, lr = lane & 31;
-  const int nw = blockDim.x >> 6;
-#pragma unroll 1
-  for (int c = w; c < lt::kCalls; c += nw) {
-    const int sn = lt::enum_state(c, lr);
-    const int s = sn < lt::kStates ? sn : lt::kStates - 1;
-    int b0, b1;
-    lt::state_bins(s, b0, b1);
-    RowRaw<S> cur;
-#pragma unroll
-    for (int rt = 0; rt < 2; ++rt) {
-      cur.bv[rt][0] = b0;
-      cur.bv[rt][1] = b1;
-      cur.iv[rt][0] = cur.iv[rt][1] = 0;
-    }
-    float zl[2];
-    wave_logits_split<S>(lds, cur, b1r, zl);
-    if (lane < 32 && sn < lt::kStates) {
-      out[lt::entry(0, b0, b1)] = zl[0];
-      out[lt::entry(1, b0, b1)] = zl[1];
-    }
-  }
-}
-
-template <class S, bool TAB>
-constexpr size_t roll_split_lds() {
-  return RollSplitLds<S>::bytes + (TAB ? sizeof(float) * lt::kEntries : 0);
-}
 
 template <class S, bool E0 = false, bool TAB = false>
 __global__ __launch_bounds__(64 * roll_split_waves<S>(), roll_split_occ<S>()) void rollout_split_kernel(RolloutArgs a) {
@@ -2246,6 +1933,14 @@
 static bool rollout_table() {
   const char *e = std::getenv("XH_ROLLOUT_TABLE");
   return !(e && *e && std::atoi(e) == 0);
+}
+static bool rollout_table_wave() {
+  const char *e = std::getenv("XH_ROLLOUT_TABLE");
+  return e && *e && std::atoi(e) == 1;
+}
+static int rollout_pack_lanes_env() {
+  const char *e = std::getenv("XH_ROLLOUT_PACK_LANES");
+  return rollout_pack_lanes(e && *e ? std::atoi(e) : 0);
 }
 
 static hipError_t launch_rollout_one(const RolloutArgs &a, int H1, int H2,
@@ -2327,6 +2022,7 @@
         const int wgr = S::B == 64 ? (kRW == 8 ? grid : cu_count()) : wg;    \
         info->name = "rollout_split_kernel";                                 \
         info->math = kMathSplitRollout;                                      \
+        info->envs_per_wave = S::G;                                          \
         multi = true;                                                        \
         if constexpr (S::B == 64) {                                          \
           if (a.e0_mask) {                                                   \
@@ -2356,6 +2052,11 @@
                 tattr = true;                                                \
               }                                                              \
               info->logit_table = true;                                      \
+              if (!rollout_table_wave()) {                                   \
+                const int pl = rollout_pack_lanes_env();                     \
+                info->envs_per_wave = 64 / pl;                               \
+                return launch_rollout_pack(a, pl, cu_count(), s);            \
+              }                                                              \
               hipLaunchKernelGGL((rollout_split_kernel<S, false, true>),     \
                                  dim3(wgr < wg ? wgr : wg), dim3(64 * kRW),  \
                                  (roll_split_lds<S, true>()), s, a);         \
@@ -2408,6 +2109,7 @@
   KernelInfo dummy;
   if (!info) info = &dummy;
   info->logit_table = false;
+  info->envs_per_wave = 0;
   const int n = a.nsteps > 1 ? a.nsteps : 1;
   bool multi = false;
   if (a.src_slot > 0 && !rollout_fetch_shifts(a, H1, H2)) {
diff --git a/dependence_free_rl_amd/csrc/rollout_pack_kernels.hip b/dependence_free_rl_amd/csrc/rollout_pack_kernels.hip
--- /dev/null
+++ b/dependence_free_rl_amd/csrc/rollout_pack_kernels.hip
@@ -0,0 +1,273 @@
+#include "rollout_pack_layout.h"
+#include "xh_roll_split.h"
+
+namespace xh {
+namespace {
+
+#ifndef XH_PACK_WAVES
+#define XH_PACK_WAVES 12
+#endif
+constexpr int kPackWaves = XH_PACK_WAVES;
+constexpr int kPackOcc = kPackWaves / 4;
+
+template <int CTRL>
+__device__ __forceinline__ int dpp_i(int v) {
+  return __builtin_amdgcn_update_dpp(0, v, CTRL, 0xF, 0xF, true);
+}
+template <int CTRL>
+__device__ __forceinline__ double dpp_d(double v) {
+  const int lo = dpp_i<CTRL>(__double2loint(v)), hi = dpp_i<CTRL>(__double2hiint(v));
+  return __hiloint2double(hi, lo);
+}
+template <int L>
+__device__ __forceinline__ int seg_sum_i(int v) {
+  v += dpp_i<0xB1>(v);
+  v += dpp_i<0x4E>(v);
+  if constexpr (L >= 8) v += dpp_i<0x141>(v);
+  if constexpr (L >= 16) v += dpp_i<0x140>(v);
+  return v;
+}
+template <int L>
+__device__ __forceinline__ float seg_min_f(float v) {
+  v = fminf(v, __int_as_float(dpp_i<0xB1>(__float_as_int(v))));
+  v = fminf(v, __int_as_float(dpp_i<0x4E>(__float_as_int(v))));
+  if constexpr (L >= 8) v = fminf(v, __int_as_float(dpp_i<0x141>(__float_as_int(v))));
+  if constexpr (L >= 16) v = fminf(v, __int_as_float(dpp_i<0x140>(__float_as_int(v))));
+  return v;
+}
+template <int L>
+__device__ __forceinline__ double seg_sum_dd(double v) {
+  v += dpp_d<0xB1>(v);
+  v += dpp_d<0x4E>(v);
+  if constexpr (L >= 8) v += dpp_d<0x141>(v);
+  if constexpr (L >= 16) v += dpp_d<0x140>(v);
+  return v;
+}
+template <int L>
+__device__ __forceinline__ double seg_scan_excl(double v, int pos) {
+  double u = dpp_d<0x111>(v);
+  if (pos >= 1) v += u;
+  u = dpp_d<0x112>(v);
+  if (pos >= 2) v += u;
+  if constexpr (L >= 8) {
+    u = dpp_d<0x114>(v);
+    if (pos >= 4) v += u;
+  }
+  if constexpr (L >= 16) {
+    u = dpp_d<0x118>(v);
+    if (pos >= 8) v += u;
+  }
+  u = dpp_d<0x111>(v);
+  return pos >= 1 ? u : 0.0;
+}
+
+template <int W>
+struct alignas(W >= 4 ? 16 : 4 * W) Words {
+  uint32_t w[W];
+};
+
+template <class S, int L>
+__device__ __forceinline__ void pack_step_groups(const RolloutArgs &a, const float *tab,
+                                                 float b3, int g0, int g_end, int gstep) {
+  static_assert(S::B == rp::kBins && S::D == 2 && S::G == 1, "64 bins, 2-D");
+  using P = rp::Pack<L>;
+  constexpr int B = S::B, G = P::kG, BPL = P::kBpl, NW = BPL / 2;
+  const int lane = threadIdx.x & 63;
+  const int pos = P::pos_of(lane), seg0 = lane - pos, bin0 = P::bin0_of(lane);
+  const unsigned long long segmask = ((1ull << L) - 1ull) << seg0;
+  const int N = a.b.N;
+  const int t_last = a.t + (a.nsteps > 1 ? a.nsteps : 1) - 1;
+  for (int g = g0; g < g_end; g += gstep) {
+    const bool act = P::active(g, lane, N);
+    const int env = act ? g * G + P::env_of(lane) : 0;
+    const bool head = act && pos == 0;
+    int bv[BPL][2], iv[2] = {0, 0};
+    uint32_t x = 1u;
+    {
+      const int slot = a.src_slot > 0 ? a.src_slot : a.t;
+      Words<NW> wd;
+      uint32_t iw = 0;
+#pragma unroll
+      for (int k = 0; k < NW; ++k) wd.w[k] = 0;
+      if (act) {
+        wd = *reinterpret_cast<const Words<NW> *>(a.b.bins + ((size_t)slot * N + env) * S::BD +
+                                                  bin0 * 2);
+        iw = *reinterpret_cast<const uint32_t *>(a.b.items + ((size_t)slot * N + env) * 4);
+        x = a.b.rng[env];
+        if (a.src_slot > 0) {
+          *reinterpret_cast<Words<NW> *>(a.b.bins + (size_t)env * S::BD + bin0 * 2) = wd;
+          if (pos == 0) *reinterpret_cast<uint32_t *>(a.b.items + (size_t)env * 4) = iw & 0xffffu;
+        }
+      }
+#pragma unroll
+      for (int r = 0; r < BPL; ++r)
+#pragma unroll
+        for (int d = 0; d < 2; ++d)
+          bv[r][d] = (int)(int8_t)(wd.w[r >> 1] >> (16 * (r & 1) + 8 * d));
+      iv[0] = (int)(int8_t)iw;
+      iv[1] = (int)(int8_t)(iw >> 8);
+    }
+    bool ia = iv[0] == a.env.item_a[0] && iv[1] == a.env.item_a[1];
+    for (int t = a.t; t <= t_last; ++t) {
+      const bool last = t == t_last;
+      float z[BPL], ex[BPL], p[BPL];
+#pragma unroll
+      for (int r = 0; r < BPL; ++r) {
+        const int e = lt::entry(ia ? 0 : 1, bv[r][0], bv[r][1]);
+        z[r] = tab[min((unsigned)e, (unsigned)lt::kEntries - 1u)] + b3;
+        ex[r] = expf(z[r]);
+      }
+      const float sum = seg_sum<L>(rp::lane_tree<BPL>(ex));
+#pragma unroll
+      for (int r = 0; r < BPL; ++r) p[r] = ex[r] / sum;
+      if (act) {
+        if (last && a.logits_out)
+#pragma unroll
+          for (int r = 0; r < BPL; ++r) a.logits_out[(size_t)env * B + bin0 + r] = z[r];
+        if (last && a.probs_out)
+#pragma unroll
+          for (int r = 0; r < BPL; ++r) a.probs_out[(size_t)env * B + bin0 + r] = p[r];
+        if (a.qold_out)
+#pragma unroll
+          for (int r = 0; r < BPL; ++r)
+            a.qold_out[((size_t)t * N + env) * B + bin0 + r] = p[r];
+      }
+
+      const double u = canonical(x);
+      int choice;
+      if (a.forced) {
+        choice = act ? a.forced[(size_t)t * N + env] : 0;
+      } else {
+        double c[BPL];
+#pragma unroll
+        for (int r = 0; r < BPL; ++r) c[r] = r == 0 ? (double)p[0] : c[r - 1] + (double)p[r];
+        const double sd = seg_sum_dd<L>(c[BPL - 1]);
+        const double excl = seg_scan_excl<L>(c[BPL - 1], pos);
+        const double rsd = 1.0 / sd;
+        int cnt = 0;
+        float gap = 1.0f;
+#pragma unroll
+        for (int r = 0; r < BPL; ++r) {
+          double cp = (excl + c[r]) * rsd;
+          if (r == BPL - 1 && pos == L - 1) cp = 1.0;
+          cnt += cp < u ? 1 : 0;
+          gap = fminf(gap, (float)fabs(cp - u));
+        }
+        choice = seg_sum_i<L>(cnt);
+        const bool near = seg_min_f<L>(gap) < 1e-9f;
+        if (__ballot(near) != 0ull) {
+          double s2 = 0.0;
+#pragma unroll 1
+          for (int j = 0; j < L; ++j)
+#pragma unroll
+            for (int r = 0; r < BPL; ++r) s2 += (double)__shfl(p[r], seg0 + j, kWave);
+          double acc = 0.0;
+          int c2 = B - 1;
+#pragma unroll 1
+          for (int j = 0; j < L; ++j)
+#pragma unroll
+            for (int r = 0; r < BPL; ++r) {
+              const int k = j * BPL + r;
+              const double qk = (double)__shfl(p[r], seg0 + j, kWave) / s2;
+              acc = k == 0 ? qk : acc + qk;
+              const double cpk = k == B - 1 ? 1.0 : acc;
+              if (!(cpk < u) && k < c2) c2 = k;
+            }
+          if (near) choice = c2;
+        }
+      }
+      const int cl = choice / BPL, cr = choice % BPL;
+      float ps = p[0];
+#pragma unroll
+      for (int r = 1; r < BPL; ++r) ps = cr == r ? p[r] : ps;
+      const float pold = __shfl(ps, seg0 + cl, kWave);
+
+      const bool owner = cl == pos;
+      bool neg = false;
+#pragma unroll
+      for (int r = 0; r < BPL; ++r)
+#pragma unroll
+        for (int d = 0; d < 2; ++d) {
+          const bool hit = owner && cr == r;
+          bv[r][d] = hit ? bv[r][d] - iv[d] : bv[r][d];
+          neg |= hit && bv[r][d] < 0;
+        }
+      const bool done = (__ballot(neg) & segmask) != 0ull;
+      const bool first = canonical(x) < a.env.p_a;
+      Words<NW> wd;
+#pragma unroll
+      for (int k = 0; k < NW; ++k) wd.w[k] = 0;
+#pragma unroll
+      for (int r = 0; r < BPL; ++r)
+#pragma unroll
+        for (int d = 0; d < 2; ++d) {
+          bv[r][d] = done ? kCapacity : bv[r][d];
+          wd.w[r >> 1] |= ((uint32_t)bv[r][d] & 0xffu) << (16 * (r & 1) + 8 * d);
+        }
+      iv[0] = first ? a.env.item_a[0] : a.env.item_b[0];
+      iv[1] = first ? a.env.item_a[1] : a.env.item_b[1];
+      ia = first;
+      if (act)
+        *reinterpret_cast<Words<NW> *>(a.b.bins + ((size_t)(t + 1) * N + env) * S::BD + bin0 * 2) =
+            wd;
+      if (head) {
+        *reinterpret_cast<uint32_t *>(a.b.items + ((size_t)(t + 1) * N + env) * 4) =
+            ((uint32_t)iv[0] & 0xffu) | (((uint32_t)iv[1] & 0xffu) << 8);
+        a.b.action[(size_t)t * N + env] = choice;
+        a.b.pold[(size_t)t * N + env] = pold;
+        a.b.done[(size_t)t * N + env] = (uint8_t)done;
+      }
+    }
+    if (head) a.b.rng[env] = (t_last == a.b.T - 1) ? mstd_mulmod(x, a.jump_mul) : x;
+  }
+}
+
+template <class S, int L>
+__global__ __launch_bounds__(64 * kPackWaves, kPackOcc) void rollout_pack_kernel(RolloutArgs a) {
+  extern __shared__ __attribute__((aligned(16))) float ldsf[];
+  char *lds = reinterpret_cast<char *>(ldsf);
+  stage_split_rollout<S>(a.params, a.env, lds);
+  __syncthreads();
+  const float b3 = reinterpret_cast<const float *>(lds + RollSplitLds<S>::F)[RollSplitLds<S>::B3];
+  const float *tab = reinterpret_cast<const float *>(lds + RollSplitLds<S>::bytes);
+  build_logit_table<S>(lds, reinterpret_cast<float *>(lds + RollSplitLds<S>::bytes));
+  __syncthreads();
+  const int ngroups = rp::Pack<L>::groups(a.b.N);
+  const int per = (ngroups + (int)gridDim.x - 1) / (int)gridDim.x;
+  const int g_end = min(ngroups, ((int)blockIdx.x + 1) * per);
+  pack_step_groups<S, L>(a, tab, b3, (int)blockIdx.x * per + (int)(threadIdx.x >> 6), g_end,
+                         (int)(blockDim.x >> 6));
+}
+
+template <class S, int L>
+hipError_t launch_pack(const RolloutArgs &a, int cus, hipStream_t s) {
+  constexpr int lds = (int)roll_split_lds<S, true>();
+  static bool attr = false;
+  if (!attr) {
+    (void)hipFuncSetAttribute((const void *)rollout_pack_kernel<S, L>,
+                              hipFuncAttributeMaxDynamicSharedMemorySize, lds);
+    attr = true;
+  }
+  const int ng = rp::Pack<L>::groups(a.b.N);
+  const int wg = (ng + kPackWaves - 1) / kPackWaves;
+  hipLaunchKernelGGL((rollout_pack_kernel<S, L>), dim3(cus < wg ? cus : wg),
+                     dim3(64 * kPackWaves), lds, s, a);
+  return hipGetLastError();
+}
+
+}
+
+int rollout_pack_lanes(int want) {
+  return want == kRollPackLanesAlt ? kRollPackLanesAlt : kRollPackLanes;
+}
+
+hipError_t launch_rollout_pack(const RolloutArgs &a, int lanes, int cus, hipStream_t s) {
+  using S = PShape<64, 2, 128, 128>;
+  if (a.env.B != 64 || a.env.D != 2 || a.e0_mask || a.wide || a.wide_seen)
+    return hipErrorInvalidValue;
+  if (lanes == kRollPackLanes) return launch_pack<S, kRollPackLanes>(a, cus, s);
+  if (lanes == kRollPackLanesAlt) return launch_pack<S, kRollPackLanesAlt>(a, cus, s);
+  return hipErrorInvalidValue;
+}
+
+}
diff --git a/dependence_free_rl_amd/csrc/rollout_pack_layout.h b/dependence_free_rl_amd/csrc/rollout_pack_layout.h
--- /dev/null
+++ b/dependence_free_rl_amd/csrc/rollout_pack_layout.h
@@ -0,0 +1,43 @@
+#ifndef XH_ROLLOUT_PACK_LAYOUT_H_
+#define XH_ROLLOUT_PACK_LAYOUT_H_
+
+#if defined(__HIPCC__)
+#define XH_RP_HD __host__ __device__
+#else
+#define XH_RP_HD
+#endif
+
+namespace xh {
+namespace rp {
+
+constexpr int kWaveLanes = 64;
+constexpr int kBins = 64;
+
+template <int L>
+struct Pack {
+  static_assert(L == 4 || L == 8 || L == 16, "lanes per env: 4, 8 or 16");
+  static constexpr int kL = L;
+  static constexpr int kG = kWaveLanes / L;
+  static constexpr int kBpl = kBins / L;
+  XH_RP_HD static int env_of(int lane) { return lane / L; }
+  XH_RP_HD static int pos_of(int lane) { return lane % L; }
+  XH_RP_HD static int bin0_of(int lane) { return (lane % L) * kBpl; }
+  XH_RP_HD static int lane_of(int e, int bin) { return e * L + bin / kBpl; }
+  XH_RP_HD static int reg_of(int bin) { return bin % kBpl; }
+  XH_RP_HD static int groups(int N) { return (N + kG - 1) / kG; }
+  XH_RP_HD static bool active(int g, int lane, int N) { return g * kG + lane / L < N; }
+};
+
+template <int N>
+XH_RP_HD inline float lane_tree(const float (&v)[N]) {
+  float t[N];
+  for (int i = 0; i < N; ++i) t[i] = v[i];
+  for (int o = 1; o < N; o <<= 1)
+    for (int i = 0; i < N; i += 2 * o) t[i] = t[i] + t[i + o];
+  return t[0];
+}
+
+}
+}
+
+#endif
diff --git a/dependence_free_rl_amd/csrc/trainer_diag.cpp b/dependence_free_rl_amd/csrc/trainer_diag.cpp
--- a/dependence_free_rl_amd/csrc/trainer_diag.cpp
+++ b/dependence_free_rl_amd/csrc/trainer_diag.cpp
@@ -432,7 +432,9 @@
     if (!t || !buf || cap == 0) return fail(XH_ERR_INVALID, "null arg");
     std::string roll = kernel_json(t->last_rollout);
     roll.insert(roll.size() - 1, std::string(", \"logit_table\": ") +
-                                     (t->last_rollout.logit_table ? "true" : "false"));
+                                     (t->last_rollout.logit_table ? "true" : "false") +
+                                     ", \"envs_per_wave\": " +
+                                     std::to_string(t->last_rollout.envs_per_wave));
     const std::string js = "{\"rollout_step\": " + roll +
                            ", \"policy_train\": " + kernel_json(t->last_train) +
                            ", \"value\": \"" +
diff --git a/dependence_free_rl_amd/csrc/xh_kernels.h b/dependence_free_rl_amd/csrc/xh_kernels.h
--- a/dependence_free_rl_amd/csrc/xh_kernels.h
+++ b/dependence_free_rl_amd/csrc/xh_kernels.h
@@ -501,9 +501,13 @@
   const char *name = nullptr;
   int math = kMathF32Mfma;
   bool logit_table = false;
+  int envs_per_wave = 0;
 };
 hipError_t launch_rollout_step(const RolloutArgs &a, int H1, int H2, int grid,
                                hipStream_t s, KernelInfo *info = nullptr);
+constexpr int kRollPackLanes = 8, kRollPackLanesAlt = 16;
+int rollout_pack_lanes(int want);
+hipError_t launch_rollout_pack(const RolloutArgs &a, int lanes, int cus, hipStream_t s);
 hipError_t launch_policy_train(const PolicyTrainArgs &a, int H1, int H2,
                                int grid, hipStream_t s,
                                KernelInfo *info = nullptr);
diff --git a/dependence_free_rl_amd/csrc/xh_roll_split.h b/dependence_free_rl_amd/csrc/xh_roll_split.h
--- /dev/null
+++ b/dependence_free_rl_amd/csrc/xh_roll_split.h
@@ -0,0 +1,324 @@
+#pragma once
+#include "spec8_e0_layout.h"
+#include "xh_device.h"
+#include "xh_kernels.h"
+#include "xh_logit_table.h"
+#include "xh_split.h"
+
+namespace xh {
+
+template <int B_, int D_, int H1_, int H2_>
+struct PShape {
+  static constexpr int B = B_, D = D_, H1 = H1_, H2 = H2_;
+  static constexpr int F0 = 2 * D;
+  static constexpr int S1 = (F0 + 1) / 2;
+  static constexpr int NIT = H1 / 32, NOT = H2 / 32;
+  static constexpr int G = B <= 64 ? 64 / B : 1;
+  static constexpr int HG = B <= 64 ? 1 : B / 64;
+  static constexpr int R = 64 * HG;
+  static constexpr int BD = B * D;
+  static constexpr int W2S = H1 + 4;
+  static constexpr int HS = H1 + 1;
+  static constexpr int AS = H2 + 1;
+  static constexpr int FJ = NOT >= 4 ? 2 : 1;
+  static constexpr int JW = (NOT * NIT + 3) / 4;
+  static constexpr int JH = (2 * NIT + 3) / 4;
+  static constexpr int TOCC = (H1 <= 64 && H2 <= 64 && D == 1) ? 2 : 1;
+  static_assert(B == 8 || B == 16 || B == 32 || B == 64 || B == 128, "B");
+  static_assert(NIT == 1 || NIT == 2 || NIT == 4, "H1 in {32,64,128}");
+  static_assert(NOT == 1 || NOT == 2 || NOT == 4, "H2 in {32,64,128}");
+  static_assert(D >= 1 && D <= 3, "D");
+  static constexpr int r4(int x) { return (x + 3) & ~3; }
+  static constexpr int L_W2 = 0;
+  static constexpr int L_W1 = L_W2 + H2 * W2S;
+  static constexpr int L_B1 = L_W1 + r4(H1 * F0);
+  static constexpr int L_B2 = L_B1 + H1;
+  static constexpr int L_W3 = L_B2 + H2;
+  static constexpr int L_B3 = L_W3 + H2;
+  static constexpr int L_Z = L_B3 + 4;
+  static constexpr int L_ROLLOUT_END = L_Z + NOT * R;
+  static constexpr int L_H1 = L_ROLLOUT_END;
+  static constexpr int L_DA2 = L_H1 + r4(64 * HS);
+  static constexpr int L_TRAIN_END = L_DA2 + r4(64 * AS);
+  static constexpr int TS = 68;
+  static constexpr int L_H1T = L_ROLLOUT_END;
+  static constexpr int L_DAT = L_H1T + H1 * TS;
+  static constexpr int L_B1F = L_DAT + H2 * TS;
+  static constexpr int L_TRAIN8_END = L_B1F + 2 * H1;
+  static constexpr int RED = H1 * F0 + H1 + 2 * H2 + 1;
+  static_assert(4 * RED <= 64 * HS + 64 * AS, "scratch fits");
+};
+
+template <class S>
+__device__ __forceinline__ void stage_params(const float *__restrict__ P,
+                                             float *lds) {
+  const PolicyLayout L{S::F0, S::H1, S::H2};
+  const int tid = threadIdx.x;
+  for (int i = tid; i < S::H2 * S::H1; i += blockDim.x) {
+    const int o = i / S::H1, k = i - o * S::H1;
+    lds[S::L_W2 + o * S::W2S + k] = P[L.oW2() + i];
+  }
+  for (int i = tid; i < S::H1 * S::F0; i += blockDim.x)
+    lds[S::L_W1 + i] = P[L.oW1() + i];
+  for (int i = tid; i < S::H1; i += blockDim.x) lds[S::L_B1 + i] = P[L.ob1() + i];
+  for (int i = tid; i < S::H2; i += blockDim.x) {
+    lds[S::L_B2 + i] = P[L.ob2() + i];
+    lds[S::L_W3 + i] = P[L.ow3() + i];
+  }
+  if (tid == 0) lds[S::L_B3] = P[L.ob3()];
+}
+
+template <class S>
+struct RowRaw {
+  int bv[2][S::D];
+  int iv[2][S::D];
+};
+
+template <class S>
+__device__ __forceinline__ void fetch_rows(const Batch &b, int slot, int e0,
+                                           RowRaw<S> &rr) {
+  const int lr = threadIdx.x & 31;
+#pragma unroll
+  for (int rt = 0; rt < 2; ++rt) {
+    const int r = rt * 32 + lr;
+    const size_t env = (size_t)slot * b.N + e0 + r / S::B;
+    const int8_t *bp = b.bins + env * S::BD + (r % S::B) * S::D;
+    const int8_t *ip = b.items + env * 4;
+#pragma unroll
+    for (int d = 0; d < S::D; ++d) {
+      rr.bv[rt][d] = bp[d];
+      rr.iv[rt][d] = ip[d];
+    }
+  }
+}
+
+template <class S>
+__device__ __forceinline__ float row_feature(const RowRaw<S> &rr, int rt,
+                                             int f) {
+  int v = 0;
+#pragma unroll
+  for (int d = 0; d < S::D; ++d) {
+    if (f == d) v = rr.bv[rt][d];
+    if (f == S::D + d) v = rr.iv[rt][d];
+  }
+  return f < S::F0 ? (float)v / (float)kCapacity : 0.0f;
+}
+
+template <class S>
+struct RollSplitLds {
+  static constexpr int W2 = 0;
+  static constexpr int F = 2 * S::H2 * kImgRow;
+  static constexpr int W1 = 0, B1 = S::H1 * S::F0, B2 = B1 + S::H1, W3 = B2 + S::H2,
+                       B3 = W3 + S::H2, SH = B3 + 1, SC = B3 + 4, B1F = SC + 2 * 16;
+  static constexpr int S1F = (S::D + 1) / 2;
+  static constexpr size_t bytes = F + sizeof(float) * (B1F + 2 * S::H1);
+};
+
+template <class S>
+__device__ __forceinline__ void stage_split_rollout(const float *__restrict__ P,
+                                                    const EnvDesc &env, char *lds) {
+  using L = RollSplitLds<S>;
+  float *lf = reinterpret_cast<float *>(lds + L::F);
+  const PolicyLayout PL{S::F0, S::H1, S::H2};
+  float mw = 0.0f, mh = 0.0f;
+  for (int e = threadIdx.x; e < S::H2 * S::H1; e += blockDim.x)
+    mw = fmaxf(mw, fabsf(P[PL.oW2() + e]));
+  for (int i = threadIdx.x; i < S::H1; i += blockDim.x) {
+    float v = fabsf(P[PL.ob1() + i]);
+    for (int k = 0; k < S::F0; ++k) v += fabsf(P[PL.oW1() + i * S::F0 + k]);
+    mh = fmaxf(mh, v);
+  }
+#pragma unroll
+  for (int o = 1; o < 64; o <<= 1) {
+    mw = fmaxf(mw, __shfl_xor(mw, o, kWave));
+    mh = fmaxf(mh, __shfl_xor(mh, o, kWave));
+  }
+  const int nw = blockDim.x >> 6, wv = threadIdx.x >> 6;
+  if ((threadIdx.x & 63) == 0) {
+    lf[L::SC + wv] = mw;
+    lf[L::SC + 16 + wv] = mh;
+  }
+  __syncthreads();
+  float MW = 0.0f, MH = 0.0f;
+  for (int v = 0; v < nw; ++v) {
+    MW = fmaxf(MW, lf[L::SC + v]);
+    MH = fmaxf(MH, lf[L::SC + 16 + v]);
+  }
+  const float SW = f16_scale_for(MW), SH = f16_scale_for(MH), S2 = SW * SH;
+  for (int e = threadIdx.x; e < S::H2 * S::H1; e += blockDim.x) {
+    const int o = e / S::H1, i = e % S::H1;
+    const int c = (i & ~12) | ((i & 4) << 1) | ((i & 8) >> 1);
+    _Float16 x0, x1;
+    split2h(P[PL.oW2() + e] * SW, x0, x1);
+    const int off = img_off(o, c >> 3) + 2 * (c & 7);
+    *reinterpret_cast<_Float16 *>(lds + L::W2 + off) = x0;
+    *reinterpret_cast<_Float16 *>(lds + L::W2 + S::H2 * kImgRow + off) = x1;
+  }
+  for (int i = threadIdx.x; i < S::H1 * S::F0; i += blockDim.x)
+    lf[L::W1 + i] = P[PL.oW1() + i] * SH;
+  for (int i = threadIdx.x; i < S::H1; i += blockDim.x) {
+    lf[L::B1 + i] = P[PL.ob1() + i] * SH;
+    lf[L::B2 + i] = P[PL.ob2() + i] * S2;
+    lf[L::W3 + i] = P[PL.ow3() + i] * (1.0f / S2);
+    float ba = P[PL.ob1() + i], bb = ba;
+#pragma unroll
+    for (int d = 0; d < S::D; ++d) {
+      const float wv = P[PL.oW1() + i * S::F0 + S::D + d];
+      ba += wv * ((float)env.item_a[d] / (float)kCapacity);
+      bb += wv * ((float)env.item_b[d] / (float)kCapacity);
+    }
+    lf[L::B1F + i] = ba * SH;
+    lf[L::B1F + S::H1 + i] = bb * SH;
+  }
+  if (threadIdx.x == 0) {
+    lf[L::B3] = P[PL.ob3()];
+    lf[L::SH] = SH;
+  }
+}
+
+template <class S, bool E0 = false>
+__device__ __forceinline__ void wave_logits_split(const char *lds,
+                                                  const RowRaw<S> &cur,
+                                                  const float *const (&b1r)[2],
+                                                  float (&zl)[2],
+                                                  unsigned *mbits = nullptr) {
+  using L = RollSplitLds<S>;
+  const float *lf = reinterpret_cast<const float *>(lds + L::F);
+  const int lane = threadIdx.x & 63, lr = lane & 31, h = lane >> 5;
+  const char *w2i[2] = {lds + L::W2, lds + L::W2 + S::H2 * kImgRow};
+#pragma unroll
+  for (int rt = 0; rt < 2; ++rt) {
+    float xb[L::S1F];
+#pragma unroll
+    for (int s1 = 0; s1 < L::S1F; ++s1) {
+      const int f = 2 * s1 + h;
+      xb[s1] = f < S::D ? row_feature<S>(cur, rt, f) : 0.0f;
+    }
+    f32x16s pre[S::NOT];
+#pragma unroll
+    for (int ot = 0; ot < S::NOT; ++ot)
+#pragma unroll
+      for (int q = 0; q < 4; ++q) {
+        const float4 bb = *reinterpret_cast<const float4 *>(lf + L::B2 + ot * 32 + 8 * q + 4 * h);
+        pre[ot][4 * q + 0] = bb.x;
+        pre[ot][4 * q + 1] = bb.y;
+        pre[ot][4 * q + 2] = bb.z;
+        pre[ot][4 * q + 3] = bb.w;
+      }
+#pragma unroll
+    for (int it = 0; it < S::NIT; ++it) {
+      f32x16 t1;
+#pragma unroll
+      for (int q = 0; q < 4; ++q) {
+        const float4 bb = *reinterpret_cast<const float4 *>(b1r[rt] + it * 32 + 8 * q + 4 * h);
+        t1[4 * q + 0] = bb.x;
+        t1[4 * q + 1] = bb.y;
+        t1[4 * q + 2] = bb.z;
+        t1[4 * q + 3] = bb.w;
+      }
+#pragma unroll
+      for (int s1 = 0; s1 < L::S1F; ++s1) {
+        const int k = 2 * s1 + h;
+        const float wa = k < S::D ? lf[L::W1 + (it * 32 + lr) * S::F0 + k] : 0.0f;
+        t1 = mfma32(wa, xb[s1], t1);
+      }
+      f16x8 bfr[2][2];
+      {
+        typedef unsigned u32x4_t __attribute__((ext_vector_type(4)));
+        u32x4_t hb[2], lb[2];
+#pragma unroll
+        for (int jj = 0; jj < 8; ++jj) {
+          unsigned h2, l2;
+          split2h_x2(relu(t1[2 * jj]), relu(t1[2 * jj + 1]), h2, l2);
+          hb[jj >> 2][jj & 3] = h2;
+          lb[jj >> 2][jj & 3] = l2;
+        }
+#pragma unroll
+        for (int s = 0; s < 2; ++s) {
+          bfr[s][0] = __builtin_bit_cast(f16x8, hb[s]);
+          bfr[s][1] = __builtin_bit_cast(f16x8, lb[s]);
+        }
+      }
+#pragma unroll
+      for (int ot = 0; ot < S::NOT; ++ot) {
+        const int rb = row_base(ot * 32 + lr, h);
+#pragma unroll
+        for (int s = 0; s < 2; ++s) {
+          f16x8 af[2];
+#pragma unroll
+          for (int p = 0; p < 2; ++p)
+            af[p] = __builtin_bit_cast(f16x8, ld_row(w2i[p], rb, 2 * it + s));
+          pre[ot] = mfma_f16(af[1], bfr[s][0], pre[ot]);
+          pre[ot] = mfma_f16(af[0], bfr[s][1], pre[ot]);
+          pre[ot] = mfma_f16(af[0], bfr[s][0], pre[ot]);
+        }
+        __builtin_amdgcn_sched_barrier(0);
+      }
+    }
+    float z = 0.0f;
+#pragma unroll
+    for (int ot = 0; ot < S::NOT; ++ot) {
+      float zp = 0.0f;
+#pragma unroll
+      for (int q = 0; q < 4; ++q) {
+        const float4 ww = *reinterpret_cast<const float4 *>(lf + L::W3 + ot * 32 + 8 * q + 4 * h);
+        const float wq[4] = {ww.x, ww.y, ww.z, ww.w};
+#pragma unroll
+        for (int u = 0; u < 4; ++u) zp = fmaf(relu(pre[ot][4 * q + u]), wq[u], zp);
+      }
+      z += zp + __shfl_xor(zp, 32, kWave);
+    }
+    zl[rt] = z;
+    if constexpr (E0) {
+#pragma unroll
+      for (int ot = 0; ot < S::NOT; ++ot) {
+        unsigned wd = rt == 0 ? 0u : mbits[ot];
+#pragma unroll
+        for (int e = 0; e < 16; ++e) {
+          int m;
+          asm("v_med3_i32 %0, %1, 0, 1" : "=v"(m) : "v"(__float_as_int(pre[ot][e])));
+          wd |= (unsigned)m << sp8::e0_bit(rt, e);
+        }
+        mbits[ot] = wd;
+      }
+    }
+  }
+}
+
+template <class S>
+__device__ __forceinline__ void build_logit_table(const char *lds, float *out) {
+  static_assert(S::B == 64 && S::D == 2 && S::G == 1 && lt::kCap == kCapacity,
+                "the logit table: 64 bins, 2-D");
+  const float *lfr = reinterpret_cast<const float *>(lds + RollSplitLds<S>::F);
+  const float *const b1r[2] = {lfr + RollSplitLds<S>::B1F,
+                               lfr + RollSplitLds<S>::B1F + S::H1};
+  const int lane = threadIdx.x & 63, w = threadIdx.x >> 6, lr = lane & 31;
+  const int nw = blockDim.x >> 6;
+#pragma unroll 1
+  for (int c = w; c < lt::kCalls; c += nw) {
+    const int sn = lt::enum_state(c, lr);
+    const int s = sn < lt::kStates ? sn : lt::kStates - 1;
+    int b0, b1;
+    lt::state_bins(s, b0, b1);
+    RowRaw<S> cur;
+#pragma unroll
+    for (int rt = 0; rt < 2; ++rt) {
+      cur.bv[rt][0] = b0;
+      cur.bv[rt][1] = b1;
+      cur.iv[rt][0] = cur.iv[rt][1] = 0;
+    }
+    float zl[2];
+    wave_logits_split<S>(lds, cur, b1r, zl);
+    if (lane < 32 && sn < lt::kStates) {
+      out[lt::entry(0, b0, b1)] = zl[0];
+      out[lt::entry(1, b0, b1)] = zl[1];
+    }
+  }
+}
+
+template <class S, bool TAB>
+constexpr size_t roll_split_lds() {
+  return RollSplitLds<S>::bytes + (TAB ? sizeof(float) * lt::kEntries : 0);
+}
+
+}
```
